# PengjieRen/CaSE_RG

Hardware: AMD Instinct MI355X
Metric: train tokens/sec (query+passage) CaSE model (higher is better)
Workload: dtype bf16; 1 GPU; CaSE train step fwd+bwd+allreduce+clip+Adam+EMA, d_model=512, 6 encoder layers, 10 passages x 384 tok, query 64, answer 40, vocab 30522, per-GPU batch 32, dropout on; global_batch=32, parallelism=dp1

## Files before the change

### case_rg_amd/CaSE/Model.py

```python
import torch
import torch.nn as nn

from .. import config, ops
from ..common.Constants import BOS_WORD, EOS_WORD, UNK_WORD
from ..common.Interaction import Interaction
from ..common.TransformerSeqEncoderDecoder import PointerDecoderCore, TransformerSeqEncoder, no_repeat_ngram_param, sampling_params
from ..common.Utils import to_sentence
from ..common.heads import block_stack, generation_nll, passage_bce, run_block_pair, run_blocks
from ..evaluation.rouge_ids import consensus_answers


class CaSETransformerSeqDecoder(PointerDecoderCore):

    def __init__(self, num_memories, num_layers, nhead, tgt_vocab_size, hidden_size, emb_matrix=None):
        super().__init__()
        H = hidden_size
        self._build(num_memories, num_layers, nhead, tgt_vocab_size, H, 2 * H, emb_matrix=emb_matrix)
        self.norm1 = nn.LayerNorm(H)
        self.norm2 = nn.LayerNorm(H)
        self.gen = nn.Sequential(nn.Linear(3 * H, H), nn.Dropout(0.1), nn.Linear(H, tgt_vocab_size, bias=False), nn.Softmax(dim=-1))
        self.mix = nn.Linear(3 * H, num_memories + 1)

    def extend(self, dec_outputs, gen_outputs, memory_weights, source_map):
        H = self.hidden_size
        d1, d2 = self._mix(dec_outputs[..., :H], [dec_outputs[..., H:2 * H], dec_outputs[..., 2 * H:]], gen_outputs,
                           memory_weights, source_map)
        return (d1, d2) if self.training else d1 + d2

    def _feature(self, answer_rep, T):
        feat = ops.layer_norm(answer_rep, self.norm2.weight, self.norm2.bias, self.norm2.eps)
        return ops.dropout(feat.unsqueeze(1).expand(-1, T, -1).contiguous(), 0.1, self.training)

    def _head_parts(self, dec_in, x, feat):
        dec_out = ops.layer_norm(x, self.norm1.weight, self.norm1.bias, self.norm1.eps)
        return dec_out, torch.cat([dec_in, dec_out, feat], dim=-1)

    train_returns_pair = True

    @property
    def gen_dropout(self):
        return self.gen[1].p

    def forward(self, encode_memories, BOS, UNK, source_map, groundtruth_index=None, additional_decoder_feature=None,
                encode_weights=None, encode_masks=None, init_decoder_state=None, max_target_length=None, beam_width=None, sampling=None,
                score_index=None, no_repeat_ngram=0):
        return self._run(encode_memories, encode_masks, encode_weights, source_map, BOS, groundtruth_index, max_target_length, beam_width, sampling,
                         score_index, feature_of=lambda T: self._feature(additional_decoder_feature, T), no_repeat_ngram=no_repeat_ngram)


class RelevantPassageSelection(nn.Module):

    def __init__(self, hidden_size, num_heads, query_encoder, passage_encoder):
        super().__init__()
        self.hidden_size = hidden_size
        self.query_encoder = query_encoder
        self.passage_encoder = passage_encoder
        self.num_heads = num_heads
        self.interaction = Interaction(hidden_size)
        self.query_blocks = block_stack(num_heads, hidden_size, 2)
        self.passage_blocks = block_stack(num_heads, hidden_size, 4)
        self.scorer = nn.Linear(hidden_size, 1)

    def action(self, query, passage, encode_query, encode_passage):
        eq, ep = encode_query[0][:, :, -1], encode_passage[0][:, :, -1]
        passage_mask, query_mask = passage.ne(0), query.ne(0)
        g_pq, g_qp = self.interaction(eq, ep, query_mask, passage_mask)
        query_reps, passage_reps = run_block_pair(self.query_blocks, g_pq, query_mask, self.passage_blocks, g_qp, passage_mask)
        cls = passage_reps[:, :, 0].contiguous()
        score = ops.linear(cls, self.scorer.weight, self.scorer.bias, out_dtype=torch.float32).squeeze(-1)
        return score, (query_reps, query_reps[:, :, 0]), (passage_reps, passage_reps[:, :, 0])


class SupportingTokenIdentification(nn.Module):

    def __init__(self, max_span_size, hidden_size, num_heads, query_encoder, passage_encoder, passage_selection):
        super().__init__()
        self.hidden_size = hidden_size
        self.num_heads = num_heads
        self.query_encoder = query_encoder
        self.passage_encoder = passage_encoder
        self.max_span_size = max_span_size
        self.passage_selection = passage_selection
        self.interaction = Interaction(hidden_size)
        self.query_blocks = block_stack(num_heads, hidden_size, 1)
        self.passage_blocks = block_stack(num_heads, hidden_size, 2)
        self.norm1 = nn.LayerNorm(hidden_size)
        self.norm2 = nn.LayerNorm(hidden_size)
        self.scorer = nn.Linear(hidden_size, 1)

    def action(self, query, passage, encode_query, encode_passage, passage_selection_result):
        passage_mask, query_mask = passage.ne(0), query.ne(0)
        _, query_rep, passage_rep = passage_selection_result
        g_pq, g_qp = self.interaction(query_rep[0], passage_rep[0], query_mask, passage_mask)
        query_reps, passage_reps = run_block_pair(self.query_blocks, g_pq, query_mask, self.passage_blocks, g_qp, passage_mask)
        token_score = ops.linear(passage_reps, self.scorer.weight, self.scorer.bias, out_dtype=torch.float32).squeeze(-1)
        token_score = token_score.masked_fill(~passage_mask, -1e6).clamp(min=-1e6, max=1e6)
        query_reps = ops.layer_norm(query_rep[0], self.norm1.weight, self.norm1.bias, self.norm1.eps, add=query_reps)
        passage_reps = ops.layer_norm(passage_rep[0], self.norm2.weight, self.norm2.bias, self.norm2.eps, add=passage_reps)
        return token_score, (query_reps, query_reps[:, :, 0]), (passage_reps, passage_reps[:, :, 0])


class ResponseGeneration(nn.Module):

    def __init__(self, BOS, UNK, vocab_size, hidden_size, num_heads, query_encoder, passage_encoder, passage_selection,
                 span_extraction, decoder):
        super().__init__()
        self.hidden_size = hidden_size
        self.vocab_size = vocab_size
        self.num_heads = num_heads
        self.query_encoder = query_encoder
        self.passage_encoder = passage_encoder
        self.passage_selection = passage_selection
        self.span_extraction = span_extraction
        self.BOS = BOS
        self.UNK = UNK
        self.decoder = decoder

    def action(self, query, passage, source_map, encode_query, encode_passage, passage_selection_result,
               span_extraction_result, output=None, max_target_length=None, beam_width=None, sampling=None, score_index=None, no_repeat_ngram=0):
        B = query.size(0)
        passage_score = passage_selection_result[0]
        token_score, query_rep, passage_rep = span_extraction_result
        H = passage_rep[0].size(-1)
        prior = (torch.sigmoid(passage_score).unsqueeze(-1) * torch.sigmoid(token_score)).reshape(B, -1)
        prior = prior / (1e-8 + prior.sum(dim=-1, keepdim=True))
        mem = passage_rep[0].reshape(B, -1, H)
        answer_rep = ops.bmm(ops.cast_to(prior.unsqueeze(1), mem.dtype), mem, b_is_kn=True).squeeze(1)
        prior_p = prior.reshape_as(token_score)
        prior_q = torch.ones(B, 1, query_rep[0].size(2), device=prior.device)
        return self.decoder([query_rep[0], passage_rep[0]], self.BOS, self.UNK, source_map,
                            additional_decoder_feature=answer_rep, groundtruth_index=output,
                            max_target_length=max_target_length, encode_masks=[query.ne(0), passage.ne(0)],
                            encode_weights=[prior_q, prior_p], beam_width=beam_width, sampling=sampling, score_index=score_index,
                            no_repeat_ngram=no_repeat_ngram)


class CaSE(nn.Module):
    def __init__(self, max_span_size, max_target_length, id2vocab, vocab2id, hidden_size, enc_layers=3, dec_layers=4, heads=8, early_stop=False):
        super().__init__()
        V = len(vocab2id)
        self.UNK = vocab2id[UNK_WORD]
        self.max_target_length = max_target_length
        self.query_encoder = TransformerSeqEncoder(enc_layers, heads, V, hidden_size)
        self.passage_encoder = self.query_encoder
        self.passage_selection = RelevantPassageSelection(hidden_size, heads, self.query_encoder, self.passage_encoder)
        self.span_extraction = SupportingTokenIdentification(max_span_size, hidden_size, heads, self.query_encoder,
                                                             self.passage_encoder, self.passage_selection)
        self.response_generation = ResponseGeneration(vocab2id[BOS_WORD], vocab2id[UNK_WORD], V, hidden_size, heads,
                                                      self.query_encoder, self.passage_encoder, self.passage_selection,
                                                      self.span_extraction,
                                                      CaSETransformerSeqDecoder(2, dec_layers, heads, V, hidden_size))
        self.id2vocab = id2vocab
        self.vocab_size = len(id2vocab)
        self.vocab2id = vocab2id
        self.beam_width = 4
        self.sampling = dict(num_samples=1, temperature=1.0, top_k=0, top_p=1.0, seed=None)
        self.consensus_samples = 8
        self.no_repeat_ngram = 0
        self.response_generation.decoder.beam_eos_id = vocab2id[EOS_WORD]
        if early_stop:
            self.response_generation.decoder.eos_id = vocab2id[EOS_WORD]

    def to_sentence(self, data, batch_indices):
        return to_sentence(batch_indices, self.id2vocab)

    def _encode_select_extract(self, data):
        if self.query_encoder is self.passage_encoder:
            eq, ep = self.query_encoder.forward_many([data['query'], data['passage']])
        else:
            eq, ep = self.query_encoder(data['query']), self.passage_encoder(data['passage'])
        ps = self.passage_selection.action(data['query'], data['passage'], encode_query=eq, encode_passage=ep)
        se = self.span_extraction.action(data['query'], data['passage'], encode_query=eq, encode_passage=ep,
                                         passage_selection_result=ps)
        return eq, ep, ps, se

    def do_train(self, data):
        eq, ep, ps, se = self._encode_select_extract(data)
        loss_ps = passage_bce(ps[0], data['passage_label'])
        valid = data['passage'].ne(0).float()
        bce = torch.nn.functional.binary_cross_entropy_with_logits(se[0], data['token_label'].detach(), reduction='none')
        loss_se = (valid * bce * data['token_weight'].detach()).sum() / valid.sum()
        rg = self.response_generation.action(data['query'], data['passage'], data['source_map'], encode_query=eq,
                                             encode_passage=ep, passage_selection_result=ps, span_extraction_result=se,
                                             output=data['response'])
        dist1, dist2 = rg[2]
        return [loss_ps, loss_se, generation_nll(ops.add(dist1, dist2), data['response'])]

    def _respond(self, data, **mode):
        eq, ep, ps, se = self._encode_select_extract(data)
        rg = self.response_generation.action(data['query'], data['passage'], data['source_map'], encode_query=eq,
                                             encode_passage=ep, passage_selection_result=ps, span_extraction_result=se,
                                             output=None, **mode)
        return rg, ps[0]

    def _ngram(self, no_repeat_ngram):
        return no_repeat_ngram_param(self.no_repeat_ngram if no_repeat_ngram is None else no_repeat_ngram, self.max_target_length)

    def do_test(self, data, no_repeat_ngram=None):
        rg, rank = self._respond(data, max_target_length=self.max_target_length, no_repeat_ngram=self._ngram(no_repeat_ngram))
        return {'answer': rg[3], 'rank': rank}

    do_infer = do_test

    def do_beam(self, data, width=None, no_repeat_ngram=None):
        rg, rank = self._respond(data, max_target_length=self.max_target_length, beam_width=self.beam_width if width is None else width,
                                 no_repeat_ngram=self._ngram(no_repeat_ngram))
        return {'answer': rg[3], 'rank': rank, 'beam_score': rg[5][:, 0], 'beam_answers': rg[4], 'beam_scores': rg[5]}

    def do_sample(self, data, num_samples=1, temperature=1.0, top_k=0, top_p=1.0, seed=None, uniforms=None, no_repeat_ngram=None):
        sampling = sampling_params(self.vocab2id, num_samples, temperature, top_k, top_p, seed, uniforms)
        rg, rank = self._respond(data, max_target_length=self.max_target_length, sampling=sampling, no_repeat_ngram=self._ngram(no_repeat_ngram))
        return {'answer': rg[3], 'rank': rank, 'samples': rg[4], 'sample_probs': rg[5], 'sample_scores': rg[6]}

    def do_consensus(self, data, pool="sample", candidates=None, valid=None, weights=None, no_repeat_ngram=None, **sampling):
        return consensus_answers(self, data, lambda d: self._encode_select_extract(d)[2][0], pool, candidates, valid, weights,
                                 no_repeat_ngram=no_repeat_ngram, **sampling)

    def do_score(self, data, answers=None):
        if self.training:
            raise ValueError("do_score runs in eval mode: call model.eval() first")
        out, rank = self._respond(data, score_index=data['response'] if answers is None else answers)
        out['rank'] = rank
        return out

    def forward(self, data, method='mle_train'):
        if method == 'train':
            return self.do_train(data)
        elif method == 'test':
            return self.do_test(data)
        elif method == 'beam':
            return self.do_beam(data)
        elif method == 'sample':
            return self.do_sample(data, **self.sampling)
        elif method == 'score':
            return self.do_score(data)
        elif method == 'consensus':
            return self.do_consensus(data)
```

### case_rg_amd/Masque/Model.py

```python
import torch
import torch.nn as nn

from .. import ops
from ..common.Constants import BOS_WORD, EOS_WORD, UNK_WORD
from ..common.Interaction import Interaction
from ..common.TransformerSeqEncoderDecoder import PointerDecoderCore, TransformerSeqEncoder, no_repeat_ngram_param, sampling_params
from ..common.Utils import to_sentence
from ..common.heads import block_stack, generation_nll, passage_bce, run_block_pair
from ..evaluation.rouge_ids import consensus_answers


class MasqueTransformerSeqDecoder(PointerDecoderCore):

    def __init__(self, num_memories, num_layers, nhead, tgt_vocab_size, hidden_size, emb_matrix=None):
        super().__init__()
        H = hidden_size
        self._build(num_memories, num_layers, nhead, tgt_vocab_size, H, H, emb_matrix=emb_matrix)
        self.norm = nn.LayerNorm(H)
        self.gen = nn.Sequential(nn.Linear(2 * H, H), nn.Linear(H, tgt_vocab_size, bias=False), nn.Softmax(dim=-1))
        self.mix = nn.Linear(3 * H, num_memories + 1)

    def extend(self, dec_outputs, gen_outputs, memory_weights, source_map):
        H = self.hidden_size
        d1, d2 = self._mix(dec_outputs[..., :H], [dec_outputs[..., H:2 * H], dec_outputs[..., 2 * H:]], gen_outputs,
                           memory_weights, source_map)
        return d1 + d2

    def _head_parts(self, dec_in, x, feat):
        dec_out = ops.layer_norm(x, self.norm.weight, self.norm.bias, self.norm.eps)
        return dec_out, torch.cat([dec_in, dec_out], dim=-1)

    def forward(self, encode_memories, BOS, UNK, source_map, encode_masks=None, encode_weights=None,
                groundtruth_index=None, init_decoder_state=None, max_target_length=None, beam_width=None, sampling=None, score_index=None,
                no_repeat_ngram=0):
        return self._run(encode_memories, encode_masks, encode_weights, source_map, BOS, groundtruth_index, max_target_length, beam_width, sampling,
                         score_index, no_repeat_ngram=no_repeat_ngram)


class PassageSelection(nn.Module):

    def __init__(self, hidden_size, num_heads, query_encoder, passage_encoder):
        super().__init__()
        self.hidden_size = hidden_size
        self.query_encoder = query_encoder
        self.passage_encoder = passage_encoder
        self.num_heads = num_heads
        self.interaction = Interaction(hidden_size)
        self.query_blocks = block_stack(num_heads, hidden_size, 2)
        self.passage_blocks = block_stack(num_heads, hidden_size, 4)
        self.scorer = nn.Linear(hidden_size, 1)

    def action(self, query, passage, encode_query=None, encode_passage=None):
        if encode_query is None:
            encode_query = self.query_encoder(query)[0][:, :, -1]
        if encode_passage is None:
            encode_passage = self.passage_encoder(passage)[0][:, :, -1]
        passage_mask, query_mask = passage.ne(0), query.ne(0)
        g_pq, g_qp = self.interaction(encode_query, encode_passage, query_mask, passage_mask)
        query_reps, passage_reps = run_block_pair(self.query_blocks, g_pq, query_mask, self.passage_blocks, g_qp, passage_mask)
        cls = passage_reps[:, :, 0].contiguous()
        score = ops.linear(cls, self.scorer.weight, self.scorer.bias, out_dtype=torch.float32).squeeze(-1)
        return score, query_reps, passage_reps


class ResponseGeneration(nn.Module):

    def __init__(self, BOS, UNK, vocab_size, hidden_size, num_heads, query_encoder, passage_encoder, passage_selection, decoder):
        super().__init__()
        self.hidden_size = hidden_size
        self.vocab_size = vocab_size
        self.num_heads = num_heads
        self.query_encoder = query_encoder
        self.passage_encoder = passage_encoder
        self.passage_selection = passage_selection
        self.BOS = BOS
        self.UNK = UNK
        self.decoder = decoder

    def action(self, query, passage, source_map, encode_query=None, encode_passage=None, passage_selection_result=None,
               output=None, max_target_length=None, beam_width=None, sampling=None, score_index=None, no_repeat_ngram=0):
        if encode_query is None:
            encode_query = self.query_encoder(query)[0][:, :, -1]
        if encode_passage is None:
            encode_passage = self.passage_encoder(passage)[0][:, :, -1]
        if passage_selection_result is None:
            passage_selection_result = self.passage_selection.action(query, passage, encode_query=encode_query,
                                                                     encode_passage=encode_passage)
        passage_score, query_rep, passage_rep = passage_selection_result
        B = query.size(0)
        prior_q = torch.ones(B, 1, query_rep.size(2), device=passage_score.device)
        prior_p = torch.sigmoid(passage_score).unsqueeze(-1).expand(-1, -1, passage_rep.size(2))
        return self.decoder([query_rep, passage_rep], self.BOS, self.UNK, source_map, groundtruth_index=output,
                            max_target_length=max_target_length, encode_masks=[query.ne(0), passage.ne(0)],
                            encode_weights=[prior_q, prior_p], beam_width=beam_width, sampling=sampling, score_index=score_index,
                            no_repeat_ngram=no_repeat_ngram)


class Masque(nn.Module):
    def __init__(self, max_target_length, id2vocab, vocab2id, hidden_size, enc_layers=3, dec_layers=4, heads=8, early_stop=False):
        super().__init__()
        V = len(vocab2id)
        self.UNK = vocab2id[UNK_WORD]
        self.max_target_length = max_target_length
        self.query_encoder = TransformerSeqEncoder(enc_layers, heads, V, hidden_size)
        self.passage_encoder = self.query_encoder
        self.passage_selection = PassageSelection(hidden_size, heads, self.query_encoder, self.passage_encoder)
        self.response_generation = ResponseGeneration(vocab2id[BOS_WORD], vocab2id[UNK_WORD], V, hidden_size, heads,
                                                      self.query_encoder, self.passage_encoder, self.passage_selection,
                                                      MasqueTransformerSeqDecoder(2, dec_layers, heads, V, hidden_size))
        self.id2vocab = id2vocab
        self.vocab_size = len(id2vocab)
        self.vocab2id = vocab2id
        self.beam_width = 4
        self.sampling = dict(num_samples=1, temperature=1.0, top_k=0, top_p=1.0, seed=None)
        self.consensus_samples = 8
        self.no_repeat_ngram = 0
        self.response_generation.decoder.beam_eos_id = vocab2id[EOS_WORD]
        if early_stop:
            self.response_generation.decoder.eos_id = vocab2id[EOS_WORD]

    def to_sentence(self, data, batch_indices):
        return to_sentence(batch_indices, self.id2vocab)

    def _encode_select(self, data):
        if self.query_encoder is self.passage_encoder:
            oq, op = self.query_encoder.forward_many([data['query'], data['passage']])
            eq, ep = oq[0][:, :, -1], op[0][:, :, -1]
        else:
            eq = self.query_encoder(data['query'])[0][:, :, -1]
            ep = self.passage_encoder(data['passage'])[0][:, :, -1]
        return eq, ep, self.passage_selection.action(data['query'], data['passage'], encode_query=eq, encode_passage=ep)

    def do_train(self, data):
        eq, ep, ps = self._encode_select(data)
        rg = self.response_generation.action(data['query'], data['passage'], data['source_map'], encode_query=eq,
                                             encode_passage=ep, passage_selection_result=ps, output=data['response'])
        return [0.25 * passage_bce(ps[0], data['passage_label']), generation_nll(rg[2], data['response'])]

    def do_ps_train(self, data):
        _, _, ps = self._encode_select(data)
        return [passage_bce(ps[0], data['passage_label'])]

    def _respond(self, data, **mode):
        eq, ep, ps = self._encode_select(data)
        rg = self.response_generation.action(data['query'], data['passage'], data['source_map'], encode_query=eq,
                                             encode_passage=ep, passage_selection_result=ps, output=None, **mode)
        return rg, ps[0]

    def _ngram(self, no_repeat_ngram):
        return no_repeat_ngram_param(self.no_repeat_ngram if no_repeat_ngram is None else no_repeat_ngram, self.max_target_length)

    def do_test(self, data, no_repeat_ngram=None):
        rg, rank = self._respond(data, max_target_length=self.max_target_length, no_repeat_ngram=self._ngram(no_repeat_ngram))
        return {'answer': rg[3], 'rank': rank}

    do_infer = do_test

    def do_beam(self, data, width=None, no_repeat_ngram=None):
        rg, rank = self._respond(data, max_target_length=self.max_target_length, beam_width=self.beam_width if width is None else width,
                                 no_repeat_ngram=self._ngram(no_repeat_ngram))
        return {'answer': rg[3], 'rank': rank, 'beam_score': rg[5][:, 0], 'beam_answers': rg[4], 'beam_scores': rg[5]}

    def do_sample(self, data, num_samples=1, temperature=1.0, top_k=0, top_p=1.0, seed=None, uniforms=None, no_repeat_ngram=None):
        sampling = sampling_params(self.vocab2id, num_samples, temperature, top_k, top_p, seed, uniforms)
        rg, rank = self._respond(data, max_target_length=self.max_target_length, sampling=sampling, no_repeat_ngram=self._ngram(no_repeat_ngram))
        return {'answer': rg[3], 'rank': rank, 'samples': rg[4], 'sample_probs': rg[5], 'sample_scores': rg[6]}

    def do_consensus(self, data, pool="sample", candidates=None, valid=None, weights=None, no_repeat_ngram=None, **sampling):
        return consensus_answers(self, data, lambda d: self._encode_select(d)[2][0], pool, candidates, valid, weights,
                                 no_repeat_ngram=no_repeat_ngram, **sampling)

    def do_score(self, data, answers=None):
        if self.training:
            raise ValueError("do_score runs in eval mode: call model.eval() first")
        out, rank = self._respond(data, score_index=data['response'] if answers is None else answers)
        out['rank'] = rank
        return out

    def forward(self, data, method='mle_train'):
        if method == 'train':
            return self.do_train(data)
        elif method == 'ps_train':
            return self.do_ps_train(data)
        elif method == 'test':
            return self.do_test(data)
        elif method == 'beam':
            return self.do_beam(data)
        elif method == 'sample':
            return self.do_sample(data, **self.sampling)
        elif method == 'score':
            return self.do_score(data)
        elif method == 'consensus':
            return self.do_consensus(data)
```

### case_rg_amd/_abi.py

```python
import ctypes as C
import os

import torch

_HERE = os.path.dirname(os.path.abspath(__file__))
LIB_PATH = os.environ.get("CASE_HIP_LIB") or os.path.join(_HERE, "csrc", "libcase_hip.so")

ABI_VERSION = 600
F32, BF16 = 0, 1
WS_ATTENTION_SPLITKV, WS_ATTENTION_BWD, WS_OPTIM_SUMSQ, WS_ENCODER_CHAIN_PACK, WS_GEMM_DW_SLABS = 1, 2, 3, 4, 5
(FEAT_GEMM_256, FEAT_GEMM_SMALL, FEAT_ENCODER_CHAIN, FEAT_ATTN_SCORES, FEAT_ATTN_DECODE, FEAT_OPTIM, FEAT_ATTN_RESIDENT, FEAT_RESERVED_CUS,
 FEAT_GEMM_DW_SLABS, FEAT_DECODER_CHAIN, FEAT_ATTN_DECODE_MQA, FEAT_POINTER_DECODE, FEAT_POINTER_HEAD, FEAT_GEMM_LN, FEAT_STEP_STATE,
 FEAT_INTERACTION, FEAT_ATTN_DECODE_APPEND, FEAT_LINEAR_SKINNY, FEAT_BEAM_DECODE, FEAT_SAMPLE_DECODE, FEAT_POINTER_SCORE, FEAT_CONSENSUS, FEAT_NGRAM_BAN) = (1 << i for i in range(23))
EPI_BIAS_COL, EPI_BIAS_ROW, EPI_GELU, EPI_RELU = 1, 2, 4, 8
EPI_RESIDUAL, EPI_MUL_DGELU, EPI_MUL_DRELU, EPI_ATOMIC, EPI_DROPOUT = 16, 32, 64, 128, 256

i32, i64, u64, f32, f64, ptr = C.c_int32, C.c_int64, C.c_uint64, C.c_float, C.c_double, C.c_void_p


class GemmDesc(C.Structure):
    _fields_ = [(n, i64) for n in ("M", "N", "K", "lda", "ldb", "ldc", "ld_aux", "batch1", "batch2",
                                   "sa1", "sa2", "sb1", "sb2", "sc1", "sc2", "saux1", "saux2")] + \
               [(n, i32) for n in ("a_kmajor", "b_kmajor", "in_dtype", "out_dtype", "epilogue", "split_k", "tile")] + \
               [("alpha", f32), ("drop_p", f32), ("seed", u64), ("offset", u64), ("state", ptr)]


class StepState(C.Structure):
    _fields_ = [("rng_base", u64), ("step_size", f32), ("bc2_sqrt", f32), ("lr", f32), ("step", i32), ("reserved", u64 * 5)]


class EncoderChainDesc(C.Structure):
    _fields_ = [("rows", i64), ("width", i32), ("variant", i32), ("eps_ln2", f32), ("eps_ln1_next", f32)]


class SoftmaxDesc(C.Structure):
    _fields_ = [("outer", i64), ("inner", i64), ("R", i64), ("C", i64), ("causal", i32), ("in_dtype", i32),
                ("out_dtype", i32), ("drop_p", f32), ("seed", u64), ("offset", u64), ("state", ptr)]


class AttnDesc(C.Structure):
    _fields_ = [(n, i64) for n in ("N", "heads", "Lq", "Lk", "head_dim", "ldq", "ldk", "ldv", "sq", "sk", "sv", "ldo", "so")] + \
               [("causal", i32), ("scale", f32), ("drop_p", f32), ("seed", u64), ("offset", u64), ("state", ptr)]


class InteractionDesc(C.Structure):
    _fields_ = [(n, i64) for n in ("n", "Lp", "Lq", "H", "eq_div")] + [("dtype", i32)]


class AttnProductDesc(C.Structure):
    _fields_ = [(n, i64) for n in ("N", "heads", "M", "Kc", "head_dim", "lda", "sa_seq", "sa_head", "ldb", "sb_seq", "sb_head",
                                   "ldc", "sc_seq", "sc_head")] + [("a_transposed", i32), ("alpha", f32)]


SIGNATURES = {
    "case_gemm": [C.POINTER(GemmDesc), ptr, ptr, ptr, ptr, ptr, ptr, ptr, ptr],
    "case_gemm_dw_bias": [C.POINTER(GemmDesc), ptr, ptr, ptr, ptr, ptr],
    "case_gemm_dw_slabs": [C.POINTER(GemmDesc), ptr, ptr, ptr, ptr, ptr, i64, ptr],
    "case_embed_pos_fwd": [ptr, ptr, ptr, ptr, i64, i64, i64, i64, f32, f32, u64, u64, ptr, i32, ptr],
    "case_embed_pos_bwd": [ptr, ptr, ptr, i64, i64, i64, f32, f32, u64, u64, ptr, i32, ptr],
    "case_scale_add_rows": [ptr, ptr, ptr, i64, i64, i64, f32, i32, ptr],
    "case_layernorm_fwd": [ptr, ptr, ptr, ptr, ptr, ptr, ptr, i64, i64, f32, i32, ptr],
    "case_layernorm_bwd": [ptr, ptr, ptr, ptr, ptr, ptr, ptr, ptr, ptr, ptr, i64, i64, i32, ptr],
    "case_layernorm_bwd_dropout": [ptr, ptr, ptr, ptr, ptr, ptr, ptr, ptr, ptr, i64, i64, f32, u64, u64, ptr, i32, ptr],
    "case_layernorm_bwd_concat5": [ptr] * 15 + [i64, i64, i32, ptr],
    "case_softmax_fwd": [C.POINTER(SoftmaxDesc), ptr, ptr, ptr, ptr, ptr, ptr],
    "case_softmax_bwd": [C.POINTER(SoftmaxDesc), ptr, ptr, ptr, ptr],
    "case_attention_supported": [i64],
    "case_attention_fwd": [C.POINTER(AttnDesc), ptr, ptr, ptr, ptr, ptr, ptr, ptr],
    "case_attention_splitkv_workspace": [C.POINTER(AttnDesc), i32, C.POINTER(i64)],
    "case_attention_fwd_splitkv": [C.POINTER(AttnDesc), ptr, ptr, ptr, ptr, ptr, ptr, ptr, i64, i32, ptr],
    "case_attention_bwd_supported": [i64],
    "case_attention_decode_supported": [i64],
    "case_attention_decode": [C.POINTER(AttnDesc), ptr, ptr, ptr, ptr, ptr, ptr],
    "case_attention_decode_append": [C.POINTER(AttnDesc), ptr, ptr, ptr, ptr, ptr, i64, i64, ptr, ptr, ptr],
    "case_attention_bwd": [C.POINTER(AttnDesc), ptr, ptr, ptr, ptr, ptr, ptr, ptr, ptr, ptr, ptr, ptr, ptr],
    "case_attention_scores_supported": [C.POINTER(AttnDesc)],
    "case_attention_scores_fwd": [C.POINTER(AttnDesc), ptr, ptr, ptr, ptr, ptr, ptr],
    "case_attention_scores_bwd": [C.POINTER(AttnDesc), ptr, ptr, ptr, ptr, ptr],
    "case_attention_product_supported": [C.POINTER(AttnProductDesc)],
    "case_attention_product": [C.POINTER(AttnProductDesc), ptr, ptr, ptr, ptr],
    "case_add": [ptr, ptr, ptr, i64, i32, ptr],
    "case_add_n": [C.POINTER(ptr), i32, ptr, i64, i32, ptr],
    "case_dropout": [ptr, ptr, i64, f32, u64, u64, ptr, i32, ptr],
    "case_mask_rows": [ptr, ptr, ptr, i64, i64, i32, ptr],
    "case_colsum": [ptr, ptr, i64, i64, i32, ptr],
    "case_cast": [ptr, ptr, i64, i32, i32, ptr],
    "case_scale_cols": [ptr, ptr, ptr, i64, i64, i32, ptr],
    "case_scale_cols_bwd": [ptr, ptr, ptr, ptr, ptr, i64, i64, i32, ptr],
    "case_rowdot_fwd": [ptr, ptr, ptr, ptr, i64, i64, i32, ptr],
    "case_linear_skinny": [ptr, ptr, i32, ptr, ptr, ptr, i64, i32, i32, ptr],
    "case_rowdot_bwd": [ptr, ptr, ptr, ptr, ptr, ptr, i64, i64, i32, ptr],
    "case_masked_mean_fwd": [ptr, ptr, ptr, i64, i64, i64, i32, ptr],
    "case_masked_mean_bwd": [ptr, ptr, ptr, i64, i64, i64, i32, ptr],
    "case_highway_gate_fwd": [ptr, ptr, i64, i64, i32, ptr],
    "case_highway_gate_bwd": [ptr, ptr, ptr, i64, i64, i32, ptr],
    "case_concat5_fwd": [ptr, ptr, ptr, ptr, ptr, i64, i64, i32, ptr],
    "case_concat5_bwd": [ptr, ptr, ptr, ptr, ptr, ptr, ptr, ptr, i64, i64, i32, ptr],
    "case_max_over_p_fwd": [ptr, ptr, ptr, i64, i64, i64, i32, ptr],
    "case_max_over_p_bwd": [ptr, ptr, ptr, i64, i64, i64, i32, ptr],
    "case_additive_scores_fwd": [ptr, ptr, ptr, ptr, i64, i64, i64, i64, i32, ptr],
    "case_additive_scores_bwd": [ptr, ptr, ptr, ptr, ptr, ptr, ptr, i64, i64, i64, i64, i32, ptr],
    "case_copy_scatter_fwd": [ptr, ptr, ptr, i64, i64, i64, i64, ptr],
    "case_copy_scatter_bwd": [ptr, ptr, ptr, i64, i64, i64, i64, ptr],
    "case_source_sort": [ptr, ptr, i64, i64, i64, ptr],
    "case_copy_scatter_sorted_fwd": [ptr, ptr, ptr, i64, i64, i64, i64, ptr],
    "case_nll_gather_fwd": [ptr, ptr, ptr, i64, i64, ptr],
    "case_nll_gather_bwd": [ptr, ptr, ptr, ptr, i64, i64, ptr],
    "case_row_argmax": [ptr, ptr, ptr, i64, i64, i64, ptr],
    "case_sentence_compact": [ptr, ptr, ptr, i64, i64, i64, i64, i64, ptr],
    "case_encoder_chain_pack": [ptr, ptr, ptr, ptr, ptr, ptr],
    "case_encoder_chain": [C.POINTER(EncoderChainDesc)] + [ptr] * 14,
    "case_set_reserved_cus": [i32],
    "case_attention_decode_mqa": [ptr, ptr, ptr, ptr, i64, i64, i64, i32, ptr, i64, ptr],
    "case_additive_key_exp": [ptr, ptr, i64, ptr],
    "case_pointer_attend_decode": [ptr] * 11 + [i64, i64, i64, ptr],
    "case_pointer_head_decode": [ptr] * 5 + [i32] + [ptr] * 4 + [i64, i64, i64, ptr],
    "case_pointer_head_beam": [ptr] * 5 + [i32] + [ptr] * 4 + [i64, i64, i64, i32, ptr],
    "case_pointer_head_sample": [ptr] * 5 + [i32] + [ptr] * 7 + [i64, i64, i64, f32, i32, f32, u64, u64, ptr, i64, i64, i64, i32, i32, ptr],
    "case_pointer_head_score": [ptr] * 3 + [i64, ptr, ptr, i32, ptr, i64, ptr, ptr, i64, i64, i64, ptr],
    "case_beam_advance": [ptr] * 12 + [i64, i64, i64, i32, i64, ptr],
    "case_pointer_head_decode_ban": [ptr] * 5 + [i32] + [ptr] * 4 + [i64, i64, i64, ptr, i64, i64, i32, i64, ptr],
    "case_pointer_head_beam_ban": [ptr] * 5 + [i32] + [ptr] * 4 + [i64, i64, i64, i32, ptr, i64, i64, i32, i64, ptr],
    "case_pointer_head_sample_ban": [ptr] * 5 + [i32] + [ptr] * 7 + [i64, i64, i64, f32, i32, f32, u64, u64, ptr, i64, i64, i64, i32, i32,
                                     ptr, i64, i64, i32, ptr],
    "case_beam_advance_ban": [ptr] * 12 + [i64, i64, i64, i32, i64, ptr, ptr, i64, ptr],
    "case_ngram_ban": [ptr, ptr, ptr, i64, i64, i64, i64, i32, i64, ptr],
    "case_remove_duplicate_ids": [ptr, ptr, i64, i64, i32, i64, ptr],
    "case_beam_gather": [ptr, ptr, i32, ptr, ptr, ptr, i64, i32, i64, i64, i64, ptr],
    "case_beam_backtrack": [ptr] * 8 + [i64, i32, i64, ptr],
    "case_lcs_pairs": [ptr] * 6 + [i64, i64, i64, i64, i64, ptr],
    "case_consensus_pick": [ptr] * 7 + [i64, i64, i64, ptr],
    "case_gemm_ln": [C.POINTER(GemmDesc), ptr, ptr, ptr, f32, ptr, ptr, ptr, ptr, ptr, ptr],
    "case_optim_sumsq": [ptr, ptr, i64, ptr, ptr, ptr],
    "case_optim_adam_ema": [ptr, ptr, i64, ptr, f32, f64, f64, f64, f64, ptr, ptr],
    "case_step_advance": [ptr, u64, f64, f64, ptr],
    "case_interaction_supported": [C.POINTER(InteractionDesc)],
    "case_interaction_fwd": [C.POINTER(InteractionDesc), ptr, ptr, ptr, ptr, ptr, ptr, ptr, ptr, ptr, ptr],
}


def _load():
    if not os.path.exists(LIB_PATH):
        raise ImportError(
            "case_rg_amd: %s is missing. Build it with `python -c 'import __graft_entry__ as g; g.build()'` "
            "(or `make -C case_rg_amd/csrc`). There is no CPU or eager fallback." % LIB_PATH)
    lib = C.CDLL(LIB_PATH)
    lib.case_version.restype = C.c_int
    if lib.case_version() != ABI_VERSION:
        raise ImportError("case_rg_amd: %s is ABI generation %d, this package binds %d -- rebuild it (make -C case_rg_amd/csrc)"
                          % (LIB_PATH, lib.case_version(), ABI_VERSION))
    for name, args in SIGNATURES.items():
        fn = getattr(lib, name)
        fn.argtypes = args
        fn.restype = C.c_int
    lib.case_optim_chunk_elems.restype = C.c_int
    lib.case_optim_chunk_elems.argtypes = []
    lib.case_encoder_chain_packed_bytes.restype = C.c_int64
    lib.case_encoder_chain_packed_bytes.argtypes = []
    lib.case_attention_bwd_scratch_floats.restype = C.c_int64
    lib.case_attention_bwd_scratch_floats.argtypes = [C.POINTER(AttnDesc)]
    lib.case_attention_decode_mqa_workspace.restype = C.c_int64
    lib.case_attention_decode_mqa_workspace.argtypes = [i64, i64, i32]
    lib.case_attention_decode_mqa_splits.restype = C.c_int32
    lib.case_attention_decode_mqa_splits.argtypes = [i64, i64]
    lib.case_abi_features.restype = C.c_uint32
    lib.case_abi_features.argtypes = []
    lib.case_get_reserved_cus.restype = C.c_int
    lib.case_get_reserved_cus.argtypes = []
    lib.case_sizeof_opt_tensor.restype = C.c_int
    lib.case_sizeof_opt_tensor.argtypes = []
    lib.case_sizeof_step_state.restype = C.c_int
    lib.case_sizeof_step_state.argtypes = []
    if lib.case_sizeof_step_state() != C.sizeof(StepState):
        raise ImportError("case_rg_amd: CaseStepState is %d bytes in %s, %d in this binding" % (lib.case_sizeof_step_state(), LIB_PATH, C.sizeof(StepState)))
    lib.case_gemm_dw_slab_bytes.restype = C.c_int64
    lib.case_gemm_dw_slab_bytes.argtypes = [C.POINTER(GemmDesc)]
    lib.case_workspace_bytes.restype = C.c_int64
    lib.case_workspace_bytes.argtypes = [i32, ptr, i64]
    lib.case_gemm_tile_for.restype = C.c_int
    lib.case_gemm_tile_for.argtypes = [C.POINTER(GemmDesc), ptr, ptr, ptr, ptr, ptr, ptr]
    lib.case_last_error.restype = C.c_char_p
    return lib


lib = _load()


def check(code, what):
    if code != 0:
        raise RuntimeError("%s failed (%d): %s" % (what, code, lib.case_last_error().decode()))


def call(name, *args):
    check(getattr(lib, name)(*args), name)
```

### case_rg_amd/common/TransformerSeqEncoderDecoder.py

```python
import operator
import os

import torch
import torch.nn as nn

from .. import config, ops
from .BilinearAttention import BilinearAttention
from .PositionalEmbedding import PositionalEmbedding
from .TransformerDecoder import TransformerDecoder, TransformerDecoderLayer
from .TransformerEncoder import TransformerEncoder, TransformerEncoderLayer
from .Utils import generate_square_subsequent_mask

MERGED_ENCODE = os.environ.get("CASE_MERGED_ENCODE", "1") != "0"
QUERY_SPLIT = os.environ.get("CASE_QUERY_SPLIT", "1") != "0"


def _embedding(vocab, width, max_len=1000, emb_matrix=None):
    if emb_matrix is not None:
        vocab, width = emb_matrix.shape
    table = nn.Embedding(vocab, width, padding_idx=0)
    if emb_matrix is not None:
        table.load_state_dict({"weight": emb_matrix})
        table.weight.requires_grad = False
    return nn.Sequential(table, PositionalEmbedding(width, dropout=0.1, max_len=max_len))
# ... 248 lines not shown
                            eu=self.attns[i].project_keys_exp(m) if fused else None))
        return out

    def _run_prefix(self, dec_ids, mems, valid, weights, feature):
        dec_in = _embed(self.embedding, dec_ids, self.training)
        tgt_valid = dec_ids.ne(0)
        x = dec_in
        ctxs, copies = [], []
        for i, mem in enumerate(mems):
            x = self.decs[i].forward_batch_first(x, mem, tgt_valid, valid[i], causal=True)
            q = x if feature is None else torch.cat([x, feature], dim=-1)
            ctx, p = self.attns[i].attend(q, mem, mem, row_valid=tgt_valid, col_valid=valid[i])
            ctxs.append(ctx)
            if weights is not None:
                p = weights[i].unsqueeze(1) * p
                p = p / (1e-8 + p.sum(dim=-1, keepdim=True))
            copies.append(p)
        return dec_in, x, ctxs, copies

    def _check_length(self, T):
        if T > self.embedding[1].pe.size(0):
            raise RuntimeError("max_target_length %d exceeds max_len %d" % (T, self.embedding[1].pe.size(0)))

    def _cache_setup(self, mems, max_target_length, feat):
        B, dev = mems[0].shape[0], mems[0].device
        inference = not self.training and not torch.is_grad_enabled()
        cache = self._memory_cache(mems, absorb=inference)
        self_kvs = [dec.new_self_cache(B, max_target_length, mems[0]) for dec in self.decs]
        hist_valid = torch.zeros(B, max_target_length, dtype=torch.bool, device=dev)
        self._check_length(max_target_length)
        splits = [self.attns[i].split_query(feat, self.hidden_size) if (QUERY_SPLIT and inference and feat is not None and cache[i]["eu"] is not None) else None
                  for i in range(len(mems))]
        return inference, cache, self_kvs, hist_valid, splits

    def _cached_layers(self, t, ids, mems, valid, weights, feat, cache, splits, self_kvs, hist_valid):
        table, pos = self.embedding[0].weight, self.embedding[1]
        tok_valid = ids.ne(0)
        hist_valid[:, t] = tok_valid[:, 0]
        dec_in = ops.embed_pos(ids, table, pos.pe[t:t + 1])
        x = dec_in
        ctxs, copies = [], []
        for i, mem in enumerate(mems):
            x = self.decs[i].step(x, t, self_kvs[i], hist_valid, cache[i]["kvs"], valid[i])
            q = x if (feat is None or splits[i] is not None) else torch.cat([x, feat], dim=-1)
            if cache[i]["eu"] is not None:
                ctx, p = self.attns[i].attend_decode(q, mem, tok_valid, valid[i], cache[i]["eu"], None if weights is None else weights[i],
                                                     split=splits[i])
            else:
                ctx, p = self.attns[i].attend(q, mem, mem, row_valid=tok_valid, col_valid=valid[i], uh=cache[i]["uh"])
                if weights is not None:
                    p = weights[i].unsqueeze(1) * p
                    p = p / (1e-8 + p.sum(dim=-1, keepdim=True))
            ctxs.append(ctx)
            copies.append(p)
        return dec_in, x, ctxs, copies

    @staticmethod
    def _per_item(n, mems, valid, weights, source_map, feat, keys=True, unit_too=False):
        if n == 1 and not unit_too:
            return mems, valid, weights, source_map, feat
        mems = [m.repeat_interleave(n, dim=0) for m in mems]
        valid = [v.repeat_interleave(n, dim=0) for v in valid]
        weights = None if weights is None else [w.repeat_interleave(n, dim=0) for w in weights]
        if keys:
            source_map = source_map.expand(n) if isinstance(source_map, ops.SortedSource) else source_map.repeat_interleave(n, dim=0)
        return mems, valid, weights, source_map, None if feat is None else feat.repeat_interleave(n, dim=0)

    def _decode(self, mode, mems, valid, weights, source_map, feat, BOS, max_target_length):
        R, dev, T = mems[0].shape[0], mems[0].device, max_target_length
        inference, cache, self_kvs, hist_valid, splits = self._cache_setup(mems, T, feat)
        ids = self._bos(R, BOS, dev)
        capturing = torch.cuda.is_current_stream_capturing()
        fused_head = inference and ops.pointer_head_supported(source_map, self.tgt_vocab_size, len(mems))
        mode.start(capturing, self_kvs, hist_valid)
        for t in range(T):
            dec_in, x, ctxs, copies = self._cached_layers(t, ids, mems, valid, weights, feat, cache, splits, self_kvs, hist_valid)
            if fused_head:
                dec_out, gen_in = self._head_parts(dec_in, x, feat)
                logits, mix_logits = self._head_logits(dec_out, gen_in, ctxs)
                ids = mode.fused_step(t, logits, mix_logits, source_map, [c.reshape(R, -1) for c in copies])
            else:
                dec_out, gen, dist = self._head(dec_in, x, ctxs, copies, feat, source_map)
                ids = mode.unfused_step(t, gen, dist)
            steps = t + 1
            if steps == T:
                break
            self_kvs, hist_valid = mode.after_step(t, self_kvs, hist_valid)
            if not capturing and steps % self.eos_check_every == 0 and mode.all_finished():
                break
        setattr(self, mode.counter, steps)
        return mode.result(dec_out)

    def _score(self, mems, valid, weights, source_map, BOS, answers, pad=0, feature_of=None):
        if self.training:
            raise ValueError("scoring runs in eval mode: call model.eval() first")
        if answers.dim() == 2:
            answers = answers.unsqueeze(1)
        if answers.dim() != 3 or answers.dtype != torch.int64 or answers.size(0) != mems[0].shape[0]:
            raise ValueError("scoring: answers must be int64 [B, T] or [B, N, T] with the batch's B")
        B, N, T = answers.shape
        dev, V, H = mems[0].device, self.tgt_vocab_size, self.hidden_size
        self._check_length(T)
        feat = None if feature_of is None else feature_of(T)
        mems, valid, weights, source_map, feat = self._per_item(N, mems, valid, weights, source_map, feat, keys=False)
        R = B * N
        tgt = answers.reshape(R, T).to(dev)
        dec_ids = torch.cat([self._bos(R, BOS, dev), tgt[:, :-1]], dim=-1)
        dec_in, x, ctxs, copies = self._run_prefix(dec_ids, mems, valid, weights, feat)
        rows, per = R * T, N * T
        dec_in, x = dec_in.reshape(rows, 1, H), x.reshape(rows, 1, H)
        feat = None if feat is None else feat.reshape(rows, 1, -1)
        ctxs = [c.reshape(rows, 1, -1) for c in ctxs]
        copies = [c.reshape(rows, -1) for c in copies]
        flat = tgt.reshape(rows)
        sorted_src = isinstance(source_map, ops.SortedSource)
        fused = sorted_src and ops.pointer_score_supported(source_map, len(mems))
        limit = max(1, int(self.score_chunk_rows))
        if per <= limit:
            step = limit // per * per
            chunks = [(r0, min(r0 + step, rows)) for r0 in range(0, rows, step)]
        else:
            chunks = [(b * per + o, min(b * per + o + limit, (b + 1) * per)) for b in range(B) for o in range(0, per, limit)]
        probs, ptrs = [], []
        for r0, r1 in chunks:
            n = r1 - r0
            dec_out, gen_in = self._head_parts(dec_in[r0:r1], x[r0:r1], None if feat is None else feat[r0:r1])
            cx, cp, y = [c[r0:r1] for c in ctxs], [c[r0:r1] for c in copies], flat[r0:r1]
            b0, b1 = r0 // per, (r1 + per - 1) // per
            if fused:
                logits, mix_logits = self._head_logits(dec_out, gen_in, cx)
                p, c = ops.pointer_head_score(logits, mix_logits, source_map.select(slice(b0, b1)), n // (b1 - b0), cp, y, pad)
            else:
                item = torch.arange(r0, r1, device=dev) // per
                src = source_map.select(item) if sorted_src else source_map.index_select(0, item)
                gen = self._generate(gen_in, 0.0)
                d1, d2 = self._mix(dec_out, cx, gen, [c.unsqueeze(1) for c in cp], src)
                inside = (y >= 0) & (y < V)
                at = y.clamp(0, V - 1).reshape(n, 1, 1)
                c = d2.gather(-1, at).reshape(n)
                p = d1.gather(-1, at).reshape(n) + c
                skip = y.eq(pad) if pad >= 0 else torch.zeros_like(inside)
                p = torch.where(skip, torch.ones_like(p), torch.where(inside, p, torch.zeros_like(p)))
                c = torch.where(skip | ~inside, torch.zeros_like(c), c)
            probs.append(p)
            ptrs.append(c)
        p, c = torch.cat(probs).view(B, N, T), torch.cat(ptrs).view(B, N, T)
        scored = (answers.to(dev).ne(pad) if pad >= 0 else torch.ones_like(answers, dtype=torch.bool, device=dev))
        count = scored.sum()
        scores = (-torch.log(p.clamp_min(1e-30)) * scored).sum(dim=-1) / scored.sum(dim=-1).clamp_min(1)
        loss = ((-torch.log(p + 1e-8) * scored).sum() / count.clamp_min(1)).reshape(1)
        return dict(token_probs=p, copy_probs=c, scores=scores, loss=loss, tokens=count)

    def _run(self, encode_memories, encode_masks, encode_weights, source_map, BOS, groundtruth_index, max_target_length, beam_width, sampling,
             score_index, feature_of=None, no_repeat_ngram=0):
        B, dev = source_map.size(0), encode_memories[0].device
        source_map = self._sorted(source_map)
        mems = [m.reshape(B, -1, self.hidden_size) for m in encode_memories]
        valid = [m.reshape(B, -1).contiguous() for m in encode_masks]
        weights = None if encode_weights is None else [w.reshape(B, -1) for w in encode_weights]
        if score_index is not None:
            return self._score(mems, valid, weights, source_map, BOS, score_index, feature_of=feature_of)
        T = groundtruth_index.size(1) if max_target_length is None else max_target_length
        if self.training and groundtruth_index is not None:
            dec_ids = torch.cat([self._bos(B, BOS, dev), groundtruth_index[:, :-1]], dim=-1)
            feat = None if feature_of is None else feature_of(dec_ids.size(1))
            dec_out, gen, dist = self._head(*self._run_prefix(dec_ids, mems, valid, weights, feat), feat, source_map)
            return dec_out, gen, dist, groundtruth_index
        if self.training:
            return None
        feat = None if feature_of is None else feature_of(1)
        ngram = no_repeat_ngram_param(no_repeat_ngram, T)
        if ngram and not ops.ngram_ban_supported():
            raise RuntimeError("no_repeat_ngram: this build of the library lacks the n-gram ban (CASE_FEAT_NGRAM_BAN)")
        if beam_width:
            W = int(beam_width)
            if not ops.beam_supported(W):
                raise RuntimeError("beam search: width %d is outside what the beam kernels are built for (1 .. 8)" % W)
            mode, n = _BeamMode(self, B, W, T, dev, ngram), W
        elif sampling:
            if not ops.sample_supported(self.tgt_vocab_size):
                raise RuntimeError("sampled decoding: the vocabulary (%d) is beyond what the sampling kernel holds in LDS (V <= 36000)"
                                   % self.tgt_vocab_size)
            mode, n = _SampleMode(B, T, dev, sampling, ngram), int(sampling["num_samples"])
        else:
            mode, n = _GreedyMode(self, B, T, dev, ngram), 1
        return self._decode(mode, *self._per_item(n, mems, valid, weights, source_map, feat, unit_too=bool(beam_width)), BOS, T)

    def _head_logits(self, dec_out, gen_in, ctxs):
        B, V = dec_out.shape[0], self.tgt_vocab_size
        h = ops.linear(gen_in, self.gen[0].weight, self.gen[0].bias)
        logits = ops.linear(h, self.gen[-2].weight, None, out_dtype=torch.float32)
        parts = [dec_out] + ctxs
        if ops.linear_skinny_supported(parts, self.mix.weight):
            mix_logits = ops.linear_skinny(parts, self.mix.weight, self.mix.bias)
        else:
            mix_logits = ops.linear(torch.cat(parts, dim=-1), self.mix.weight, self.mix.bias, out_dtype=torch.float32)
        return logits.reshape(B, V), mix_logits.reshape(B, -1)

    def _head(self, dec_in, x, ctxs, copies, feat, source_map):
        dec_out, gen_in = self._head_parts(dec_in, x, feat)
        gen = self._generate(gen_in, self.gen_dropout)
        d1, d2 = self._mix(dec_out, ctxs, gen, copies, source_map)
        return dec_out, gen, ((d1, d2) if self.training and self.train_returns_pair else ops.add(d1, d2))

    def _generate(self, gen_in, hidden_drop):
        h = ops.linear(gen_in, self.gen[0].weight, self.gen[0].bias, p_drop=config.drop_p(hidden_drop, self.training))
        logits = ops.linear(h, self.gen[-2].weight, None, out_dtype=torch.float32)
        return ops.masked_softmax(logits)

    def _mix(self, dec_out, ctxs, gen, copies, source_map):
        mix_in = torch.cat([dec_out] + ctxs, dim=-1)
        pm = ops.masked_softmax(ops.linear(mix_in, self.mix.weight, self.mix.bias, out_dtype=torch.float32))
        dist1 = pm[:, :, 0:1] * gen
        ptr = torch.cat([pm[:, :, k + 1:k + 2] * c for k, c in enumerate(copies)], dim=-1)
        return dist1, self._scatter(ptr, source_map, gen.shape[-1])

    @staticmethod
    def _scatter(ptr, source_map, V):
        if isinstance(source_map, ops.SortedSource) or (source_map.dtype == torch.int64 and source_map.dim() == 2):
            return ops.copy_scatter(source_map, ptr, V)
        return ops.copy_scatter(source_map.argmax(dim=-1), ptr * source_map.sum(dim=-1).unsqueeze(1), V)

    @staticmethod
    def _bos(batch_size, BOS, device):
        return torch.full((batch_size, 1), BOS, dtype=torch.long, device=device)


class TransformerSeqDecoder(PointerDecoderCore):

    def __init__(self, num_memories, num_layers, nhead, tgt_vocab_size, hidden_size, emb_matrix=None):
        super().__init__()
        H = hidden_size
        self._build(num_memories, num_layers, nhead, tgt_vocab_size, H, H, emb_matrix=emb_matrix, max_len=100 if emb_matrix is not None else 1000)
        self.norm = nn.LayerNorm(H)
        self.gen = nn.Sequential(nn.Linear(2 * H, H), nn.Linear(H, tgt_vocab_size, bias=False), nn.Softmax(dim=-1))
        self.mix = nn.Linear(H + num_memories * H, num_memories + 1)

    def _head_parts(self, dec_in, x, feat):
        dec_out = ops.layer_norm(x, self.norm.weight, self.norm.bias, self.norm.eps)
        return dec_out, torch.cat([dec_in, dec_out], dim=-1)

    def forward(self, encode_memories, BOS, UNK, source_maps, encode_masks=None, encode_weights=None,
                groundtruth_index=None, init_decoder_state=None, max_target_length=None, beam_width=None, sampling=None, score_index=None,
                no_repeat_ngram=0):
        if isinstance(source_maps, (list, tuple)):
            source_maps = torch.cat(source_maps, dim=-2 if source_maps[0].dim() == 3 else -1)
        return self._run(encode_memories, encode_masks, encode_weights, source_maps, BOS, groundtruth_index, max_target_length, beam_width, sampling,
                         score_index, no_repeat_ngram=no_repeat_ngram)
```

### case_rg_amd/common/heads.py

```python
import os

import torch
import torch.distributed as dist
import torch.nn as nn
import torch.nn.functional as F

from .. import ops
from .TransformerBlock import TransformerBlock


def block_stack(num_heads, hidden_size, extra):
    return nn.ModuleList([TransformerBlock(num_heads, 5 * hidden_size, hidden_size)] +
                         [TransformerBlock(num_heads, hidden_size, hidden_size) for _ in range(extra)])


def run_blocks(blocks, reps, mask):
    for block in blocks:
        reps = block(reps, mask)
    return reps


SIDE_STREAM = os.environ.get("CASE_SIDE_STREAM", "1") != "0"
SIDE_STREAM_INFERENCE = os.environ.get("CASE_SIDE_STREAM_INFERENCE", "0") == "1"
SIDE_STREAM_NOT_UNDER_DP = os.environ.get("CASE_SIDE_STREAM_UNDER_DP", "0") != "1"
SIDE_STREAM_MIN_ELEMS = 100_000_000
_side = {}


def run_block_pair(query_blocks, g_pq, query_mask, passage_blocks, g_qp, passage_mask):
    if not (SIDE_STREAM and g_pq.is_cuda and g_qp.numel() >= SIDE_STREAM_MIN_ELEMS and (torch.is_grad_enabled() or SIDE_STREAM_INFERENCE)
            and not torch.cuda.is_current_stream_capturing() and not (SIDE_STREAM_NOT_UNDER_DP and dist.is_available() and dist.is_initialized())):
        return run_blocks(query_blocks, g_pq, query_mask), run_blocks(passage_blocks, g_qp, passage_mask)
    cur = torch.cuda.current_stream()
    side = _side.get(g_pq.device)
    if side is None:
        side = _side[g_pq.device] = torch.cuda.Stream(device=g_pq.device)
    ops.AUX_STREAMS[side.cuda_stream] = side
    ops.AUX_STREAMS[cur.cuda_stream] = cur
    side.wait_stream(cur)
    with torch.cuda.stream(side):
        g_pq.record_stream(side)
        if torch.is_tensor(query_mask):
            query_mask.record_stream(side)
        query_reps = run_blocks(query_blocks, g_pq, query_mask)
    passage_reps = run_blocks(passage_blocks, g_qp, passage_mask)
    cur.wait_stream(side)
    query_reps.record_stream(cur)
    return query_reps, passage_reps


def passage_bce(passage_score, passage_label):
    target = torch.zeros_like(passage_score).scatter_(1, passage_label.unsqueeze(-1), 1.0)
    return F.binary_cross_entropy_with_logits(passage_score.float(), target.float()).unsqueeze(0)


def generation_nll(dist, response):
    V = dist.size(-1)
    rows = ops.nll_rows(dist.reshape(-1, V), response.reshape(-1))
    count = response.ne(0).sum().clamp(min=1)
    return (rows.sum() / count).unsqueeze(0)
```

### case_rg_amd/csrc/api.hip

```cpp
#include <stdarg.h>
#include <stdio.h>
#include <stdlib.h>

#include "common.h"

static thread_local char g_err[512] = "";

int case_set_error(int code, const char* fmt, ...) {
  va_list ap;
  va_start(ap, fmt);
  vsnprintf(g_err, sizeof(g_err), fmt, ap);
  va_end(ap);
  return code;
}

int case_check_launch(const char* what) {
  const hipError_t e = hipGetLastError();
  if (e == hipSuccess) return CASE_OK;
  return case_set_error(CASE_E_LAUNCH, "%s: %s", what, hipGetErrorString(e));
}

extern "C" int case_version(void) { return CASE_ABI_VERSION; }
extern "C" uint32_t case_abi_features(void) {
  return CASE_FEAT_GEMM_256 | CASE_FEAT_GEMM_SMALL | CASE_FEAT_ENCODER_CHAIN | CASE_FEAT_ATTN_SCORES | CASE_FEAT_ATTN_DECODE | CASE_FEAT_OPTIM |
         CASE_FEAT_ATTN_RESIDENT | CASE_FEAT_RESERVED_CUS | CASE_FEAT_GEMM_DW_SLABS | CASE_FEAT_ATTN_DECODE_MQA | CASE_FEAT_POINTER_DECODE | CASE_FEAT_POINTER_HEAD | CASE_FEAT_GEMM_LN | CASE_FEAT_STEP_STATE | CASE_FEAT_INTERACTION | CASE_FEAT_ATTN_DECODE_APPEND | CASE_FEAT_LINEAR_SKINNY |
         CASE_FEAT_BEAM_DECODE | CASE_FEAT_SAMPLE_DECODE | CASE_FEAT_POINTER_SCORE | CASE_FEAT_CONSENSUS | CASE_FEAT_NGRAM_BAN;
}
extern "C" const char* case_last_error(void) { return g_err; }

static int g_reserved_cus = [] {
  const char* e = getenv("CASE_RESERVE_CUS");
  return e ? atoi(e) : 0;
}();
extern "C" int case_set_reserved_cus(int n) {
  if (n < 0 || n > 128) return case_set_error(CASE_E_ARG, "case_set_reserved_cus: %d out of range (0 .. 128)", n);
  g_reserved_cus = n;
  return CASE_OK;
}
extern "C" int case_get_reserved_cus(void) { return g_reserved_cus; }
int case_device_cus() {
  static int cus = 0;
  if (!cus) {
    int dev = 0, n = 0;
    (void)hipGetDevice(&dev);
    (void)hipDeviceGetAttribute(&n, hipDeviceAttributeMultiprocessorCount, dev);
    cus = n > 0 ? n : 256;
  }
  return cus;
}
int case_persistent_cus() {
  int c = case_device_cus() - g_reserved_cus;
  c = c / 8 * 8;
  return c > 8 ? c : 8;
}
extern "C" int case_sizeof_opt_tensor(void) { return (int)sizeof(CaseOptTensor); }
```

### case_rg_amd/csrc/attn_pointer.hip

```cpp
#include "common.h"

namespace {

template <bool FAST>
__device__ __forceinline__ float tanh_t(float x) {
  if constexpr (FAST) {
    const float e = __expf(2.f * x);
    return 1.f - __fdividef(2.f, e + 1.f);
  } else {
    return tanhf(x);
  }
}

constexpr float TANH_PRESCALE = 2.8853900817779268f;
constexpr float EXP2_CLAMP = 62.f;
__device__ __forceinline__ float exp2_factor(float xs) { return __builtin_amdgcn_exp2f(fminf(fmaxf(xs, -EXP2_CLAMP), EXP2_CLAMP)); }
__device__ __forceinline__ float half_sigmoid_prod(float ew, float eu) { return __builtin_amdgcn_rcpf(fmaf(ew, eu, 1.f)); }

constexpr int AJ = 64;
constexpr int AH = 64;
constexpr int ATW = 8;

template <typename T, bool FAST>
__global__ __launch_bounds__(256) void additive_fwd_kernel(const float* __restrict__ wq, const T* __restrict__ uh,
// ... 800 lines not shown
  return x;
}

template <bool BAN>
__global__ __launch_bounds__(PH_THREADS) void pointer_head_sample_kernel(const HeadArgs a, const SampleArgs s, const BanArgs nb) {
  extern __shared__ __attribute__((aligned(16))) float ph_smem[];
  float* row = ph_smem;
  uint32_t* tk = reinterpret_cast<uint32_t*>(ph_smem + ((a.V + 3) & ~(int64_t)3));
  float* tv = reinterpret_cast<float*>(tk + PH_THREADS + 4);
  float* red = tv + PH_THREADS;
  unsigned long long* hist = reinterpret_cast<unsigned long long*>(tk);
  __shared__ unsigned long long sel[3];
  __shared__ uint32_t wcnt[SM_WAVES];
  __shared__ float wsum[SM_WAVES];
  __shared__ int wmin[SM_WAVES], wmax[SM_WAVES];
  __shared__ int tie_id;
  const int64_t b = blockIdx.x;
  const int V = (int)a.V, tid = threadIdx.x, lane = tid & 63, wave = tid >> 6;
  if (a.logits) {
    pointer_head_build_row(a, row, tk, tv, red, b);
  } else {
    for (int i = tid; i < V; i += PH_THREADS) row[i] = s.dist_in[b * a.V + i];
    __syncthreads();
  }
  if constexpr (BAN) {
    if (!s.ended[b]) ngram_ban_row(row, a.V, nb.hist + b * nb.Tmax, nb.t, nb.n, s.eos, reinterpret_cast<int*>(tv));
  }
  float pmax = 0.f;
  for (int i = tid; i < V; i += PH_THREADS) {
    const float x = row[i];
    if (a.dist) a.dist[b * a.V + i] = x;
    pmax = fmaxf(pmax, x);
  }
  pmax = block_max(pmax, red);

  SampleView v;
  v.row = row;
  const int chunk = (((V + SM_WAVES - 1) / SM_WAVES) + 255) & ~255;
  v.w0 = min(V, wave * chunk);
  v.w1 = min(V, v.w0 + chunk);
  v.lane = lane;
  v.unit = s.temperature == 1.f;
  v.inv_tau = 1.f / s.temperature;
  v.l2max = v.unit ? 0.f : __builtin_amdgcn_logf(pmax);
  {
    int e = 0;
    frexpf(v.unit ? pmax : 1.f, &e);
    v.scale = ldexpf(1.f, min(40 - e, 120));
  }
  v.cbits = 0;
  v.cid = V - 1;

  if (s.top_k > 0 && s.top_k < V) {
    const uint32_t bits = sample_radix<false>(v, hist, sel, (unsigned long long)s.top_k, 0.0);
    const unsigned long long r = sel[1] - sel[0];
    const int id = sample_nth_tie(v, bits, r, wcnt, &tie_id, V);
    v.cbits = bits;
    v.cid = id;
  }
  if (s.top_p < 1.f) {
    const uint32_t bits = sample_radix<true>(v, hist, sel, 0ull, (double)s.top_p);
    const unsigned long long m = (unsigned long long)(__uint_as_float(bits) * v.scale), lack = sel[1] - sel[0];
    const unsigned long long r = m > 0 ? (lack + m - 1) / m : 1ull;
    const int id = sample_nth_tie(v, bits, r < 1 ? 1ull : r, wcnt, &tie_id, V);
    v.cbits = bits;
    v.cid = id;
  }

  float carry = 0.f;
  for (int base = v.w0; base < v.w1; base += 256) {
    float x[4];
    v.quad(base, x);
    const float mine = ((x[0] + x[1]) + x[2]) + x[3];
    const float inc = sample_scan64(mine, lane);
    float before = __shfl_up(inc, 1, 64);
    if (lane == 0) before = 0.f;
    carry += __shfl(before + mine, 63, 64);
  }
  if (lane == 0) wsum[wave] = carry;
  __syncthreads();
  float off = 0.f, Z = 0.f;
  for (int w = 0; w < SM_WAVES; ++w) {
    if (w == wave) off = Z;
    Z += wsum[w];
  }
  const float u = s.uniforms ? s.uniforms[b] : rng_uniform24(s.seed, rng_base_of(s.state) + s.offset + (uint64_t)b);
  const float thr = u * Z;
  int mn = 0x7fffffff, mx = -1;
  carry = 0.f;
  for (int base = v.w0; base < v.w1; base += 256) {
    float x[4];
    v.quad(base, x);
    const float mine = ((x[0] + x[1]) + x[2]) + x[3];
    const float inc = sample_scan64(mine, lane);
    float before = __shfl_up(inc, 1, 64);
    if (lane == 0) before = 0.f;
    float run = 0.f;
#pragma unroll
    for (int e = 0; e < 4; ++e) {
      run = e == 0 ? x[0] : run + x[e];
      const int i = base + 4 * lane + e;
      if (x[e] > 0.f) {
        mx = i;
        if (off + (carry + (before + run)) > thr && i < mn) mn = i;
      }
    }
    carry += __shfl(before + mine, 63, 64);
  }
#pragma unroll
  for (int o = 32; o > 0; o >>= 1) {
    mn = min(mn, __shfl_xor(mn, o, 64));
    mx = max(mx, __shfl_xor(mx, o, 64));
  }
  if (lane == 0) {
    wmin[wave] = mn;
    wmax[wave] = mx;
  }
  __syncthreads();
  if (tid == 0) {
    for (int w = 0; w < SM_WAVES; ++w) {
      mn = min(mn, wmin[w]);
      mx = max(mx, wmax[w]);
    }
    const int x = mn < V ? mn : (mx >= 0 ? mx : 0);
    const bool e = s.ended[b] != 0, this_end = (int64_t)x == s.eos;
    int64_t emit;
    if (s.first) emit = this_end ? s.unk : (int64_t)x;
    else if (s.last) emit = e ? s.pad : s.eos;
    else emit = e ? s.pad : (int64_t)x;
    s.ids[b] = emit;
    if constexpr (BAN) nb.hist[b * nb.Tmax + nb.t] = (int32_t)emit;
    s.prob[b] = e ? 1.f : row[x];
    s.ended[b] = (uint8_t)(e || this_end);
  }
}

__global__ __launch_bounds__(64) void ngram_ban_kernel(float* __restrict__ dist, const uint8_t* __restrict__ ended, const int64_t V, const BanArgs nb) {
  __shared__ int stage[NB_MAX_T];
  const int64_t b = blockIdx.x;
  if (ended && ended[b]) return;
  ngram_ban_row(dist + b * V, V, nb.hist + b * nb.Tmax, nb.t, nb.n, nb.eos, stage);
}

constexpr int PS_THREADS = 256;
struct ScoreArgs {
  const float* logits;
  const float* mix_logits;
  const uint32_t* keys;
  const float* copy[PH_MAX_MEM];
  int64_t len[PH_MAX_MEM];
  const int64_t* targets;
  float* prob;
  float* ptr;
  int64_t V, S, rows_per_source, pad;
  int nmem;
};

typedef float ps_f32x4 __attribute__((ext_vector_type(4)));
#ifndef CASE_STREAM_DEFAULT_POLICY
#define PS_LOAD1(P) __builtin_nontemporal_load(P)
#define PS_LOAD4(P) __builtin_nontemporal_load(reinterpret_cast<const ps_f32x4*>(P))
#else
#define PS_LOAD1(P) (*(P))
#define PS_LOAD4(P) (*reinterpret_cast<const ps_f32x4*>(P))
#endif

__device__ __forceinline__ void ps_merge(float& m, float& s, const float om, const float os) {
  const float M = fmaxf(m, om);
  const float ref = M == -INFINITY ? 0.f : M;
  s = s * __expf(m - ref) + os * __expf(om - ref);
  m = M;
}

__global__ __launch_bounds__(PS_THREADS) void pointer_head_score_kernel(const ScoreArgs a) {
  __shared__ float red_m[PS_THREADS / 64], red_s[PS_THREADS / 64];
  const int64_t r = blockIdx.x, V = a.V;
  const int tid = threadIdx.x, lane = tid & 63;
  const int64_t y = a.targets[r];
  const bool is_pad = a.pad >= 0 && y == a.pad;
  if (is_pad || y < 0 || y >= V) {
    if (tid == 0) {
      a.prob[r] = is_pad ? 1.f : 0.f;
      if (a.ptr) a.ptr[r] = 0.f;
    }
    return;
  }
  const float* lg = a.logits + r * V;
  int64_t head = (int64_t)(((16u - (uint32_t)(reinterpret_cast<uintptr_t>(lg) & 15u)) & 15u) >> 2);
  if (head > V) head = V;
  const int64_t n4 = (V - head) >> 2, tail = head + 4 * n4;
  float m = -INFINITY, s = 0.f;
  if (tid < head) ps_merge(m, s, PS_LOAD1(lg + tid), 1.f);
  const float* body = lg + head;
#pragma unroll 2
  for (int64_t i = tid; i < n4; i += PS_THREADS) {
    const ps_f32x4 x = PS_LOAD4(body + 4 * i);
    const float m4 = fmaxf(fmaxf(x[0], x[1]), fmaxf(x[2], x[3]));
    if (m4 > m) {
      s *= __expf(m - m4);
      m = m4;
    }
    s += (__expf(x[0] - m) + __expf(x[1] - m)) + (__expf(x[2] - m) + __expf(x[3] - m));
  }
  if (tail + tid < V) ps_merge(m, s, PS_LOAD1(lg + tail + tid), 1.f);
#pragma unroll
  for (int o = 32; o > 0; o >>= 1) {
    const float om = __shfl_xor(m, o, 64), os = __shfl_xor(s, o, 64);
    ps_merge(m, s, om, os);
  }
  if (lane == 0) {
    red_m[tid >> 6] = m;
    red_s[tid >> 6] = s;
  }
  __syncthreads();
  if (tid >= 64) return;
  m = red_m[0];
  s = red_s[0];
#pragma unroll
  for (int w = 1; w < PS_THREADS / 64; ++w) ps_merge(m, s, red_m[w], red_s[w]);
  const float gen_y = __expf(lg[y] - m) / s;
  float pm[1 + PH_MAX_MEM];
  {
    float mm = -INFINITY, ss = 0.f;
#pragma unroll
    for (int k = 0; k <= PH_MAX_MEM; ++k) pm[k] = k <= a.nmem ? a.mix_logits[r * (a.nmem + 1) + k] : -INFINITY;
#pragma unroll
    for (int k = 0; k <= PH_MAX_MEM; ++k) mm = fmaxf(mm, pm[k]);
#pragma unroll
    for (int k = 0; k <= PH_MAX_MEM; ++k) {
      pm[k] = __expf(pm[k] - mm);
      ss += pm[k];
    }
#pragma unroll
    for (int k = 0; k <= PH_MAX_MEM; ++k) pm[k] /= ss;
  }
  const uint32_t* keys = a.keys + (r / a.rows_per_source) * a.S;
  const uint32_t want = (uint32_t)y << 15;
  int64_t lo = 0, hi = a.S;
  while (lo < hi) {
    const int64_t mid = (lo + hi) >> 1;
    if (keys[mid] < want) lo = mid + 1;
    else hi = mid;
  }
  float acc = 0.f;
  for (int64_t i = lo + lane; i < a.S; i += 64) {
    const uint32_t key = keys[i];
    if (key == 0xFFFFFFFFu || (key >> 15) != (uint32_t)y) break;
    int64_t pos = key & 0x7FFFu;
    bool done = false;
#pragma unroll
    for (int k = 0; k < PH_MAX_MEM; ++k) {
      if (k < a.nmem && !done) {
        if (pos < a.len[k]) {
          acc += pm[k + 1] * a.copy[k][r * a.len[k] + pos];
          done = true;
        }
        pos -= a.len[k];
      }
    }
  }
  acc = wave_sum(acc);
  if (lane == 0) {
    a.prob[r] = pm[0] * gen_y + acc;
    if (a.ptr) a.ptr[r] = acc;
  }
}

__global__ void copy_scatter_fwd_kernel(const int64_t* __restrict__ src, const float* __restrict__ w,
                                        float* __restrict__ dist, int64_t B, int64_t Tn, int64_t S, int64_t V) {
  const int64_t n = B * Tn * S;
  for (int64_t i = (int64_t)blockIdx.x * blockDim.x + threadIdx.x; i < n; i += (int64_t)gridDim.x * blockDim.x) {
    const int64_t sidx = i % S, bt = i / S, b = bt / Tn;
    const int64_t tok = src[b * S + sidx];
    const float val = w[i];
    if (tok >= 0 && tok < V && val != 0.f) atomicAdd(dist + bt * V + tok, val);
  }
}

__global__ void copy_scatter_bwd_kernel(const int64_t* __restrict__ src, const float* __restrict__ d_dist,
                                        float* __restrict__ d_w, int64_t B, int64_t Tn, int64_t S, int64_t V) {
  const int64_t n = B * Tn * S;
  for (int64_t i = (int64_t)blockIdx.x * blockDim.x + threadIdx.x; i < n; i += (int64_t)gridDim.x * blockDim.x) {
    const int64_t sidx = i % S, bt = i / S, b = bt / Tn;
    const int64_t tok = src[b * S + sidx];
    d_w[i] = (tok >= 0 && tok < V) ? d_dist[bt * V + tok] : 0.f;
  }
}

__global__ __launch_bounds__(1024) void source_sort_kernel(const int64_t* __restrict__ src, uint32_t* __restrict__ keys, int64_t S,
                                                            int64_t V, int n) {
  extern __shared__ uint32_t sk[];
  const int64_t b = blockIdx.x;
  for (int i = threadIdx.x; i < n; i += 1024) {
    uint32_t k = 0xFFFFFFFFu;
    if (i < S) {
      const int64_t tok = src[b * S + i];
      if (tok >= 0 && tok < V) k = ((uint32_t)tok << 15) | (uint32_t)i;
    }
    sk[i] = k;
  }
  __syncthreads();
  for (int k = 2; k <= n; k <<= 1) {
    for (int j = k >> 1; j > 0; j >>= 1) {
      for (int i = threadIdx.x; i < n; i += 1024) {
        const int p = i ^ j;
        if (p > i) {
          const uint32_t x = sk[i], y = sk[p];
          if ((x > y) == ((i & k) == 0)) {
            sk[i] = y;
            sk[p] = x;
          }
        }
      }
      __syncthreads();
    }
  }
  for (int i = threadIdx.x; i < S; i += 1024) keys[b * S + i] = sk[i];
}

__global__ __launch_bounds__(256) void copy_scatter_sorted_kernel(const uint32_t* __restrict__ keys, const float* __restrict__ w,
                                                                  float* __restrict__ dist, int64_t Tn, int64_t S, int64_t V) {
  __shared__ uint32_t tk[257];
  __shared__ float tv[256];
  const int64_t bt = blockIdx.x, b = bt / Tn;
  const uint32_t* k = keys + b * S;
  const float* wr = w + bt * S;
  float* d = dist + bt * V;
  for (int64_t base = 0; base < S; base += 256) {
    const int64_t i = base + threadIdx.x;
    const uint32_t key = i < S ? k[i] : 0xFFFFFFFFu;
    const bool valid = key != 0xFFFFFFFFu;
    tk[threadIdx.x] = valid ? (key >> 15) : 0xFFFFFFFFu;
    tv[threadIdx.x] = valid ? wr[key & 0x7FFFu] : 0.f;
    if (threadIdx.x == 0) tk[256] = 0xFFFFFFFEu;
    __syncthreads();
    const uint32_t tok = tk[threadIdx.x];
    if (valid && tok != tk[threadIdx.x + 1]) {
      int j = threadIdx.x;
      while (j > 0 && tk[j - 1] == tok) --j;
      float sum = 0.f;
      for (; j <= (int)threadIdx.x; ++j) sum += tv[j];
      if (sum != 0.f) d[tok] += sum;
    }
    __threadfence_block();
    __syncthreads();
  }
}

__global__ void nll_fwd_kernel(const float* __restrict__ dist, const int64_t* __restrict__ target,
                               float* __restrict__ per_row, int64_t rows, int64_t V) {
  for (int64_t r = (int64_t)blockIdx.x * blockDim.x + threadIdx.x; r < rows; r += (int64_t)gridDim.x * blockDim.x) {
    const int64_t y = target[r];
    per_row[r] = (y > 0 && y < V) ? -logf(dist[r * V + y] + 1e-8f) : 0.f;
  }
}

__global__ void nll_bwd_kernel(const float* __restrict__ dist, const int64_t* __restrict__ target,
                               const float* __restrict__ g_row, float* __restrict__ d_dist, int64_t rows, int64_t V) {
  for (int64_t r = (int64_t)blockIdx.x * blockDim.x + threadIdx.x; r < rows; r += (int64_t)gridDim.x * blockDim.x) {
    const int64_t y = target[r];
    if (y > 0 && y < V) d_dist[r * V + y] = -g_row[r] / (dist[r * V + y] + 1e-8f);
  }
}

__global__ __launch_bounds__(256) void row_argmax_kernel(const float* __restrict__ x, int64_t* __restrict__ idx,
                                                         float* __restrict__ val, int64_t rows, int64_t cols, int64_t ld) {
  __shared__ float sv[4];
  __shared__ int64_t si[4];
  for (int64_t r = blockIdx.x; r < rows; r += gridDim.x) {
    float best = -INFINITY;
    int64_t bi = cols;
    for (int64_t c = threadIdx.x; c < cols; c += 256) {
      const float vv = x[r * ld + c];
      if (vv > best || (vv == best && c < bi)) {
        best = vv;
        bi = c;
      }
    }
#pragma unroll
    for (int o = 32; o > 0; o >>= 1) {
      const float ob = __shfl_xor(best, o, 64);
      const int64_t oi = __shfl_xor(bi, o, 64);
      if (ob > best || (ob == best && oi < bi)) {
        best = ob;
        bi = oi;
      }
    }
    __syncthreads();
    if ((threadIdx.x & 63) == 0) {
      sv[threadIdx.x >> 6] = best;
      si[threadIdx.x >> 6] = bi;
    }
    __syncthreads();
    if (threadIdx.x == 0) {
      for (int w = 1; w < 4; ++w)
        if (sv[w] > best || (sv[w] == best && si[w] < bi)) {
          best = sv[w];
          bi = si[w];
        }
      idx[r] = bi < cols ? bi : 0;
      if (val) val[r] = best;
    }
  }
}

}

extern "C" int case_additive_scores_fwd(const float* wq, const void* uh, const float* v, float* s, int64_t B, int64_t T,
                                        int64_t S, int64_t H, int32_t dtype, case_stream_t stream) {
  CASE_REQUIRE(wq && uh && v && s && B > 0 && T > 0 && S > 0 && H > 0 && B < 65536, "case_additive_scores_fwd: bad argument");
  hipStream_t st = (hipStream_t)stream;
  const int ev = dtype == CASE_F32 ? 4 : 8;
  if (T <= 2 && H % ev == 0 && H <= 2 * 64 * ev && (uintptr_t)uh % 16 == 0) {
    const dim3 g((unsigned)((S + 15) / 16 < 64 ? (S + 15) / 16 : 64), (unsigned)B);
    const bool one = H <= 64 * ev;
#define ROWWISE(TY, FAST, TT, NCH) hipLaunchKernelGGL((additive_fwd_rowwise_kernel<TY, FAST, TT, NCH>), g, dim3(256), 0, st, wq, (const TY*)uh, v, s, T, S, H)
    if (dtype == CASE_F32) {
// ... 140 lines not shown
  a.ids = ids;
  a.top = top;
  static bool attr = false;
  rc = pointer_head_reserve(reinterpret_cast<const void*>(&pointer_head_decode_kernel<BAN>), attr, who);
  if (rc != CASE_OK) return rc;
  hipLaunchKernelGGL(pointer_head_decode_kernel<BAN>, dim3((unsigned)B), dim3(PH_THREADS), pointer_head_lds(V), (hipStream_t)stream, a, nb);
  return case_check_launch(who);
}

extern "C" int case_pointer_head_decode(const float* logits, const float* mix_logits, const uint32_t* keys, const float* const* copies,
                                        const int64_t* lens, int32_t nmem, float* gen, float* dist, int64_t* ids, float* top, int64_t B, int64_t V,
                                        int64_t S, case_stream_t stream) {
  return pointer_head_decode_launch<false>("case_pointer_head_decode", logits, mix_logits, keys, copies, lens, nmem, gen, dist, ids, top, B, V, S,
                                           BanArgs(), stream);
}

extern "C" int case_pointer_head_decode_ban(const float* logits, const float* mix_logits, const uint32_t* keys, const float* const* copies,
                                            const int64_t* lens, int32_t nmem, float* gen, float* dist, int64_t* ids, float* top, int64_t B,
                                            int64_t V, int64_t S, int32_t* hist, int64_t Tmax, int64_t t, int32_t n, int64_t eos,
                                            case_stream_t stream) {
  BanArgs nb;
  const int rc = pointer_head_ban(nb, "case_pointer_head_decode_ban", hist, Tmax, t, n, eos);
  if (rc != CASE_OK) return rc;
  return pointer_head_decode_launch<true>("case_pointer_head_decode_ban", logits, mix_logits, keys, copies, lens, nmem, gen, dist, ids, top, B, V, S,
                                          nb, stream);
}

template <bool BAN>
static int pointer_head_beam_launch(const char* who, const float* logits, const float* mix_logits, const uint32_t* keys, const float* const* copies,
                                    const int64_t* lens, int32_t nmem, float* gen, float* dist, float* cand_p, int64_t* cand_id, int64_t R, int64_t V,
                                    int64_t S, int32_t W, const BanArgs& nb, case_stream_t stream) {
  CASE_REQUIRE(cand_p && cand_id, "%s: bad argument", who);
  if (W < 1 || W > PH_MAX_W || W > V) return case_set_error(CASE_E_UNSUPPORTED, "%s: width %d outside 1 .. min(%d, V)", who, W, PH_MAX_W);
  HeadArgs a;
  int rc = pointer_head_args(a, who, logits, mix_logits, keys, copies, lens, nmem, gen, dist, R, V, S);
  if (rc != CASE_OK) return rc;
  static bool attr = false;
  rc = pointer_head_reserve(reinterpret_cast<const void*>(&pointer_head_beam_kernel<BAN>), attr, who);
  if (rc != CASE_OK) return rc;
  hipLaunchKernelGGL(pointer_head_beam_kernel<BAN>, dim3((unsigned)R), dim3(PH_THREADS), pointer_head_lds(V), (hipStream_t)stream, a, cand_p, cand_id,
                     (int)W, nb);
  return case_check_launch(who);
}

extern "C" int case_pointer_head_beam(const float* logits, const float* mix_logits, const uint32_t* keys, const float* const* copies,
                                      const int64_t* lens, int32_t nmem, float* gen, float* dist, float* cand_p, int64_t* cand_id, int64_t R,
                                      int64_t V, int64_t S, int32_t W, case_stream_t stream) {
  return pointer_head_beam_launch<false>("case_pointer_head_beam", logits, mix_logits, keys, copies, lens, nmem, gen, dist, cand_p, cand_id, R, V, S, W,
                                         BanArgs(), stream);
}

extern "C" int case_pointer_head_beam_ban(const float* logits, const float* mix_logits, const uint32_t* keys, const float* const* copies,
                                          const int64_t* lens, int32_t nmem, float* gen, float* dist, float* cand_p, int64_t* cand_id, int64_t R,
                                          int64_t V, int64_t S, int32_t W, const int32_t* hist, int64_t Tmax, int64_t t, int32_t n, int64_t eos,
                                          case_stream_t stream) {
  BanArgs nb;
  const int rc = pointer_head_ban(nb, "case_pointer_head_beam_ban", hist, Tmax, t, n, eos);
  if (rc != CASE_OK) return rc;
  return pointer_head_beam_launch<true>("case_pointer_head_beam_ban", logits, mix_logits, keys, copies, lens, nmem, gen, dist, cand_p, cand_id, R, V, S,
                                        W, nb, stream);
}

template <bool BAN>
static int pointer_head_sample_launch(const char* who, const float* logits, const float* mix_logits, const uint32_t* keys, const float* const* copies,
                                      const int64_t* lens, int32_t nmem, const float* dist_in, float* gen, float* dist, int64_t* ids, float* prob,
                                      uint8_t* ended, const float* uniforms, int64_t R, int64_t V, int64_t S, float temperature, int32_t top_k,
                                      float top_p, uint64_t seed, uint64_t offset, const CaseStepState* state, int64_t eos, int64_t unk, int64_t pad,
                                      int32_t first, int32_t last, const BanArgs& nb, case_stream_t stream) {
  CASE_REQUIRE(ids && prob && ended && R > 0 && V > 0 && R < (1ll << 31), "%s: bad argument", who);
  CASE_REQUIRE(temperature > 0.f && top_k >= 0 && top_p > 0.f && top_p <= 1.f, "%s: temperature must be > 0, top_k >= 0 and top_p in (0, 1]", who);
  CASE_REQUIRE((logits != nullptr) != (dist_in != nullptr), "%s: give either the logits or a ready distribution", who);
  HeadArgs a;
  if (logits) {
    const int rc = pointer_head_args(a, who, logits, mix_logits, keys, copies, lens, nmem, gen, dist, R, V, S);
    if (rc != CASE_OK) return rc;
  } else {
    if (V > PH_MAX_V) return case_set_error(CASE_E_UNSUPPORTED, "%s: built for V <= %lld", who, (long long)PH_MAX_V);
    a = HeadArgs();
    a.dist = dist;
    a.V = V;
  }
  SampleArgs s;
  s.dist_in = dist_in;
  s.uniforms = uniforms;
  s.state = state;
  s.seed = seed;
  s.offset = offset;
  s.ended = ended;
  s.ids = ids;
  s.prob = prob;
  s.eos = eos;
  s.unk = unk;
  s.pad = pad;
  s.temperature = temperature;
  s.top_p = top_p;
  s.top_k = top_k;
  s.first = first;
  s.last = last;
  static bool attr = false;
  const int rc = pointer_head_reserve(reinterpret_cast<const void*>(&pointer_head_sample_kernel<BAN>), attr, who);
  if (rc != CASE_OK) return rc;
  hipLaunchKernelGGL(pointer_head_sample_kernel<BAN>, dim3((unsigned)R), dim3(PH_THREADS), pointer_head_lds(V), (hipStream_t)stream, a, s, nb);
  return case_check_launch(who);
}

extern "C" int case_pointer_head_sample(const float* logits, const float* mix_logits, const uint32_t* keys, const float* const* copies,
                                        const int64_t* lens, int32_t nmem, const float* dist_in, float* gen, float* dist, int64_t* ids, float* prob,
                                        uint8_t* ended, const float* uniforms, int64_t R, int64_t V, int64_t S, float temperature, int32_t top_k,
                                        float top_p, uint64_t seed, uint64_t offset, const CaseStepState* state, int64_t eos, int64_t unk,
                                        int64_t pad, int32_t first, int32_t last, case_stream_t stream) {
  return pointer_head_sample_launch<false>("case_pointer_head_sample", logits, mix_logits, keys, copies, lens, nmem, dist_in, gen, dist, ids, prob,
                                           ended, uniforms, R, V, S, temperature, top_k, top_p, seed, offset, state, eos, unk, pad, first, last,
                                           BanArgs(), stream);
}

extern "C" int case_pointer_head_sample_ban(const float* logits, const float* mix_logits, const uint32_t* keys, const float* const* copies,
                                            const int64_t* lens, int32_t nmem, const float* dist_in, float* gen, float* dist, int64_t* ids,
                                            float* prob, uint8_t* ended, const float* uniforms, int64_t R, int64_t V, int64_t S, float temperature,
                                            int32_t top_k, float top_p, uint64_t seed, uint64_t offset, const CaseStepState* state, int64_t eos,
                                            int64_t unk, int64_t pad, int32_t first, int32_t last, int32_t* hist, int64_t Tmax, int64_t t, int32_t n,
                                            case_stream_t stream) {
  BanArgs nb;
  const int rc = pointer_head_ban(nb, "case_pointer_head_sample_ban", hist, Tmax, t, n, eos);
  if (rc != CASE_OK) return rc;
  return pointer_head_sample_launch<true>("case_pointer_head_sample_ban", logits, mix_logits, keys, copies, lens, nmem, dist_in, gen, dist, ids, prob,
                                          ended, uniforms, R, V, S, temperature, top_k, top_p, seed, offset, state, eos, unk, pad, first, last, nb,
                                          stream);
}

extern "C" int case_ngram_ban(float* dist, const int32_t* hist, const uint8_t* ended, int64_t R, int64_t V, int64_t Tmax, int64_t t, int32_t n,
                              int64_t eos, case_stream_t stream) {
  CASE_REQUIRE(dist && R > 0 && R < (1ll << 31) && V > 0, "case_ngram_ban: bad argument");
  BanArgs nb;
  const int rc = pointer_head_ban(nb, "case_ngram_ban", hist, Tmax, t, n, eos);
  if (rc != CASE_OK) return rc;
  hipLaunchKernelGGL(ngram_ban_kernel, dim3((unsigned)R), dim3(64), 0, (hipStream_t)stream, dist, ended, V, nb);
  return case_check_launch("case_ngram_ban");
}

extern "C" int case_pointer_head_score(const float* logits, const float* mix_logits, const uint32_t* keys, int64_t rows_per_source,
                                       const float* const* copies, const int64_t* lens, int32_t nmem, const int64_t* targets, int64_t pad,
                                       float* prob, float* copy, int64_t R, int64_t V, int64_t S, case_stream_t stream) {
  CASE_REQUIRE(targets && prob, "case_pointer_head_score: bad argument");
  CASE_REQUIRE(rows_per_source >= 1 && R % rows_per_source == 0, "case_pointer_head_score: %lld rows are no multiple of rows_per_source %lld",
               (long long)R, (long long)rows_per_source);
  ScoreArgs a;
  const int rc = pointer_head_fill(a, "case_pointer_head_score", logits, mix_logits, keys, copies, lens, nmem, R, V, S, PS_MAX_V, "");
  if (rc != CASE_OK) return rc;
  a.targets = targets;
  a.prob = prob;
  a.ptr = copy;
  a.rows_per_source = rows_per_source;
  a.pad = pad;
  hipLaunchKernelGGL(pointer_head_score_kernel, dim3((unsigned)R), dim3(PS_THREADS), 0, (hipStream_t)stream, a);
  return case_check_launch("case_pointer_head_score");
}

extern "C" int case_copy_scatter_fwd(const int64_t* src, const float* w, float* dist, int64_t B, int64_t T, int64_t S,
                                     int64_t V, case_stream_t stream) {
  CASE_REQUIRE(src && w && dist && B > 0 && T > 0 && S > 0 && V > 0, "case_copy_scatter_fwd: bad argument");
  hipLaunchKernelGGL(copy_scatter_fwd_kernel, dim3(grid_for(B * T * S, 256, 2)), dim3(256), 0, (hipStream_t)stream, src, w,
                     dist, B, T, S, V);
  return case_check_launch("case_copy_scatter_fwd");
}

extern "C" int case_copy_scatter_bwd(const int64_t* src, const float* d_dist, float* d_w, int64_t B, int64_t T, int64_t S,
                                     int64_t V, case_stream_t stream) {
  CASE_REQUIRE(src && d_dist && d_w && B > 0 && T > 0 && S > 0 && V > 0, "case_copy_scatter_bwd: bad argument");
  hipLaunchKernelGGL(copy_scatter_bwd_kernel, dim3(grid_for(B * T * S, 256, 2)), dim3(256), 0, (hipStream_t)stream, src,
                     d_dist, d_w, B, T, S, V);
  return case_check_launch("case_copy_scatter_bwd");
}

extern "C" int case_source_sort(const int64_t* src, uint32_t* keys, int64_t B, int64_t S, int64_t V, case_stream_t stream) {
  CASE_REQUIRE(src && keys && B > 0 && S > 0 && V > 0, "case_source_sort: bad argument");
  CASE_REQUIRE(S <= 32768 && V <= 131071, "case_source_sort: S <= 32768 and V <= 131071 (token << 15 | position must fit 32 bits)");
  int n = 2;
  while (n < S) n <<= 1;
  if (n > 16384 && hipFuncSetAttribute((const void*)source_sort_kernel, hipFuncAttributeMaxDynamicSharedMemorySize, 32768 * 4) != hipSuccess)
    return case_set_error(CASE_E_LAUNCH, "case_source_sort: cannot reserve 128 KiB of LDS");
  hipLaunchKernelGGL(source_sort_kernel, dim3((unsigned)B), dim3(1024), (size_t)n * 4, (hipStream_t)stream, src, keys, S, V, n);
  return case_check_launch("case_source_sort");
}

extern "C" int case_copy_scatter_sorted_fwd(const uint32_t* keys, const float* w, float* dist, int64_t B, int64_t T, int64_t S,
                                            int64_t V, case_stream_t stream) {
  CASE_REQUIRE(keys && w && dist && B > 0 && T > 0 && S > 0 && V > 0 && B * T < (1ll << 31), "case_copy_scatter_sorted_fwd: bad argument");
  CASE_REQUIRE(S <= 32768 && V <= 131071, "case_copy_scatter_sorted_fwd: S <= 32768 and V <= 131071");
  hipLaunchKernelGGL(copy_scatter_sorted_kernel, dim3((unsigned)(B * T)), dim3(256), 0, (hipStream_t)stream, keys, w, dist, T, S, V);
  return case_check_launch("case_copy_scatter_sorted_fwd");
}

extern "C" int case_nll_gather_fwd(const float* dist, const int64_t* target, float* per_row, int64_t rows, int64_t V,
                                   case_stream_t stream) {
  CASE_REQUIRE(dist && target && per_row && rows > 0 && V > 0, "case_nll_gather_fwd: bad argument");
  hipLaunchKernelGGL(nll_fwd_kernel, dim3(grid_for(rows, 256)), dim3(256), 0, (hipStream_t)stream, dist, target, per_row, rows, V);
  return case_check_launch("case_nll_gather_fwd");
}

extern "C" int case_nll_gather_bwd(const float* dist, const int64_t* target, const float* g_row, float* d_dist,
                                   int64_t rows, int64_t V, case_stream_t stream) {
  CASE_REQUIRE(dist && target && g_row && d_dist && rows > 0 && V > 0, "case_nll_gather_bwd: bad argument");
  hipLaunchKernelGGL(nll_bwd_kernel, dim3(grid_for(rows, 256)), dim3(256), 0, (hipStream_t)stream, dist, target, g_row, d_dist, rows, V);
  return case_check_launch("case_nll_gather_bwd");
}

namespace {
__global__ void sentence_compact_kernel(const int64_t* __restrict__ ids, int64_t* __restrict__ out, int32_t* __restrict__ len,
                                        int64_t B, int64_t T, int64_t bos, int64_t pad, int64_t eos) {
  const int64_t b = (int64_t)blockIdx.x * blockDim.x + threadIdx.x;
  if (b >= B) return;
  int n = 0;
  bool open = true;
  for (int64_t t = 0; t < T; ++t) {
    const int64_t id = ids[b * T + t];
    if (open && id == eos) open = false;
    if (open && id != bos && id != pad) out[b * T + n++] = id;
  }
  len[b] = n;
  for (int64_t t = n; t < T; ++t) out[b * T + t] = pad;
}

constexpr int RD_MAX_T = 256;
__global__ __launch_bounds__(64) void remove_duplicate_kernel(int64_t* __restrict__ out, int32_t* __restrict__ len, const int64_t T, const int n,
                                                              const int64_t pad) {
  __shared__ int64_t tok[RD_MAX_T];
  const int64_t b = blockIdx.x;
  const int lane = threadIdx.x;
  int64_t* row = out + b * T;
  int L = len[b];
  L = L < 0 ? 0 : (L > (int)T ? (int)T : L);
  const int L0 = L;
  for (int i = lane; i < L0; i += 64) tok[i] = row[i];
  __syncthreads();
  int first[4];
#pragma unroll
  for (int e = 0; e < 4; ++e) {
    const int p = 4 * lane + e;
    first[e] = p;
    if (p < L0) {
      const int64_t mine = tok[p];
      for (int q = 0; q < p; ++q)
        if (tok[q] == mine) {
          first[e] = q;
          break;
        }
    }
  }
  while (L > n) {
    int s[4];
#pragma unroll
    for (int e = 3; e >= 0; --e) {
      const int p = 4 * lane + e;
      const int x = p < L ? first[e] : -1;
      s[e] = e == 3 ? x : max(x, s[e + 1]);
    }
    int tot = s[0];
#pragma unroll
    for (int o = 1; o < 64; o <<= 1) {
      const int other = __shfl_down(tot, o, 64);
      if (lane + o < 64) tot = max(tot, other);
    }
    int after = __shfl_down(tot, 1, 64);
    if (lane == 63) after = -1;
    int best = 0;
#pragma unroll
    for (int e = 0; e < 4; ++e) {
      const int i = 4 * lane + e;
      if (i >= 1 && i <= L - n && max(s[e], after) < i) best = i;
    }
#pragma unroll
    for (int o = 32; o > 0; o >>= 1) best = max(best, __shfl_xor(best, o, 64));
    if (best < 1) break;
    L = best;
  }
  for (int i = L + lane; i < L0; i += 64) row[i] = pad;
  if (lane == 0) len[b] = L;
}
}

extern "C" int case_sentence_compact(const int64_t* ids, int64_t* out, int32_t* len, int64_t B, int64_t T, int64_t bos, int64_t pad,
                                     int64_t eos, case_stream_t stream) {
  CASE_REQUIRE(ids && out && len && B > 0 && T > 0, "case_sentence_compact: bad argument");
  hipLaunchKernelGGL(sentence_compact_kernel, dim3((unsigned)((B + 63) / 64)), dim3(64), 0, (hipStream_t)stream, ids, out, len, B, T, bos,
                     pad, eos);
  return case_check_launch("case_sentence_compact");
}

extern "C" int case_remove_duplicate_ids(int64_t* out, int32_t* len, int64_t B, int64_t T, int32_t n, int64_t pad, case_stream_t stream) {
  CASE_REQUIRE(out && len && B > 0 && B < (1ll << 31) && T > 0 && n >= 1, "case_remove_duplicate_ids: bad argument");
  if (T > RD_MAX_T) return case_set_error(CASE_E_UNSUPPORTED, "case_remove_duplicate_ids: rows of up to %d positions (got %lld)", RD_MAX_T, (long long)T);
  hipLaunchKernelGGL(remove_duplicate_kernel, dim3((unsigned)B), dim3(64), 0, (hipStream_t)stream, out, len, T, (int)n, pad);
  return case_check_launch("case_remove_duplicate_ids");
}

extern "C" int case_row_argmax(const float* x, int64_t* idx, float* val, int64_t rows, int64_t cols, int64_t ld,
                               case_stream_t stream) {
  CASE_REQUIRE(x && idx && rows > 0 && cols > 0 && ld >= cols, "case_row_argmax: bad argument");
  hipLaunchKernelGGL(row_argmax_kernel, dim3(grid_for(rows, 1)), dim3(256), 0, (hipStream_t)stream, x, idx, val, rows, cols, ld);
  return case_check_launch("case_row_argmax");
}
```

### case_rg_amd/ops.py

```python
import math
import ctypes as C
import os

import torch
from torch.autograd import Function

from . import _abi as A
from . import config, paramcache

_DT = {torch.float32: A.F32, torch.bfloat16: A.BF16}


def _code(t):
    try:
        return _DT[t.dtype]
    except KeyError:
        raise TypeError("case_rg_amd: unsupported activation dtype %s" % t.dtype)


_raw_stream, _cur_device = getattr(torch._C, "_cuda_getCurrentRawStream", None), getattr(torch._C, "_cuda_getDevice", None)


def _stream():
    if _raw_stream is not None and _cur_device is not None:
        return _raw_stream(_cur_device())
    return torch.cuda.current_stream().cuda_stream


def _ptr(t, offset_elems=0):
    if t is None:
        return None
    if not t.is_cuda:
        raise RuntimeError("case_rg_amd ops run on the GPU only (got a %s tensor); there is no CPU path" % t.device)
    return t.data_ptr() + offset_elems * t.element_size()


def _drop4(drop):
    if drop is None:
        return 0.0, 0, 0, None
    return tuple(drop) if len(drop) == 4 else tuple(drop) + (None,)


def _u8(mask):
    if mask is None:
        return None
    m = mask.contiguous()
    return m.view(torch.uint8) if m.dtype == torch.bool else m


def invalidate_param_cache():
    paramcache.rewritten()


def cast_param(p, dtype):
    if p.dtype == dtype:
        return p.detach().contiguous()
    base = getattr(p, "_base", None)
    owner = p if isinstance(p, torch.nn.Parameter) else (base if isinstance(base, torch.nn.Parameter) else None)
    if owner is None:
        return cast(p.detach(), dtype)
    owners, tag = (owner,), paramcache.cast_tag(p, dtype)
    hit = paramcache.peek(owners, tag)
    if hit is not None:
        return hit
    if owner is not p and p.is_contiguous() and owner.is_contiguous():
        whole = paramcache.peek(owners, paramcache.cast_tag(owner, dtype))
        if whole is not None:
            return whole.as_strided(p.shape, p.stride(), p.storage_offset() - owner.storage_offset())
    return paramcache.derived(owners, tag, lambda: cast(p.detach(), dtype))


def cast(x, dtype):
    if x.dtype == dtype:
        return x
    x = x.contiguous()
    out = torch.empty(x.shape, dtype=dtype, device=x.device)
    A.call("case_cast", _ptr(x), _ptr(out), x.numel(), _code(x), _DT[dtype], _stream())
    return out


ENCODER_CHAIN = "auto"


def encoder_chain_supported(x, width, ffn_width, needs_grad):
    return (ENCODER_CHAIN == "auto" and x.is_cuda and x.dtype == torch.bfloat16 and width == 512 and ffn_width == 512
            and not needs_grad)


def _chain_pack(mats):
    def build():
        low = [None if m is None else cast_param(m, torch.bfloat16) for m in mats]
        packed = torch.empty(A.lib.case_encoder_chain_packed_bytes() // 2, dtype=torch.bfloat16, device=next(m for m in mats if m is not None).device)
        A.call("case_encoder_chain_pack", _ptr(low[0]), _ptr(low[1]), _ptr(low[2]), _ptr(low[3]), _ptr(packed), _stream())
        return packed

    return paramcache.derived(mats, "chain", build)


def encoder_chain(variant, x_in, resid, layer, next_layer):
    M = x_in.shape[0] * x_in.shape[1]
    dev = x_in.device
    f32 = lambda p: None if p is None else p.detach()
    lay = None if variant == "head" else layer
    nxt = None if variant == "tail" else next_layer
    packed = _chain_pack((None if lay is None else lay.self_attn.out_proj.weight, None if lay is None else lay.linear1.weight,
                          None if lay is None else lay.linear2.weight, None if nxt is None else nxt.self_attn.in_proj_weight))
    d = A.EncoderChainDesc()
    d.rows, d.width, d.variant = M, 512, {"full": 0, "tail": 1, "head": 2}[variant]
    d.eps_ln2 = 0.0 if lay is None else lay.norm2.eps
    d.eps_ln1_next = 0.0 if nxt is None else nxt.norm1.eps
    s_out = torch.empty(x_in.shape, dtype=torch.bfloat16, device=dev)
    qkv = None if nxt is None else torch.empty(x_in.shape[0], x_in.shape[1], 1536, dtype=torch.bfloat16, device=dev)
    x_in = x_in if x_in.is_contiguous() else x_in.contiguous()
    if resid is not None and not resid.is_contiguous():
        resid = resid.contiguous()
    A.call("case_encoder_chain", d, _ptr(x_in), _ptr(resid), _ptr(packed),
           _ptr(None if lay is None else f32(lay.self_attn.out_proj.bias)), _ptr(None if lay is None else f32(lay.linear1.bias)),
           _ptr(None if lay is None else f32(lay.linear2.bias)), _ptr(None if nxt is None else f32(nxt.self_attn.in_proj_bias)),
           _ptr(None if lay is None else f32(lay.norm2.weight)), _ptr(None if lay is None else f32(lay.norm2.bias)),
           _ptr(None if nxt is None else f32(nxt.norm1.weight)), _ptr(None if nxt is None else f32(nxt.norm1.bias)),
           _ptr(s_out), _ptr(qkv), _stream())
    return s_out, qkv


GEMM_TILE = 0
AUX_STREAMS = {}


TILE_TRACE = None
DECODE_MIN_PAIRS = 192
FUSE_BIAS_GRAD = True


def gemm(a, b, c, M, N, K, lda, ldb, ldc, *, a_off=0, b_off=0, c_off=0, a_kmajor=False, b_kmajor=False,
         batch1=1, batch2=1, sa=(0, 0), sb=(0, 0), sc=(0, 0), alpha=1.0, epilogue=0, bias_col=None, bias_row=None,
         aux=None, aux_out=None, ld_aux=0, saux=(0, 0), split_k=1, drop=None, rowsum_out=None):
    d = A.GemmDesc()
    d.M, d.N, d.K, d.lda, d.ldb, d.ldc, d.ld_aux = M, N, K, lda, ldb, ldc, ld_aux
    d.batch1, d.batch2 = batch1, batch2
    d.sa1, d.sa2 = sa
    d.sb1, d.sb2 = sb
    d.sc1, d.sc2 = sc
    d.saux1, d.saux2 = saux
    d.a_kmajor, d.b_kmajor = int(a_kmajor), int(b_kmajor)
    d.in_dtype, d.out_dtype = _code(a), _code(c)
    d.tile = GEMM_TILE
    if b.dtype != a.dtype:
        raise TypeError("gemm operands differ in dtype: %s vs %s" % (a.dtype, b.dtype))
    for name, t in (("aux", aux), ("aux_out", aux_out)):
        if t is not None and t.dtype != a.dtype:
            raise TypeError("gemm %s must have the operand dtype %s, got %s" % (name, a.dtype, t.dtype))
    for name, t in (("bias_col", bias_col), ("bias_row", bias_row)):
        if t is not None and t.dtype != torch.float32:
            raise TypeError("gemm %s must be float32, got %s" % (name, t.dtype))
    if drop is not None and drop[0] > 0.0:
        epilogue |= A.EPI_DROPOUT
        d.drop_p, d.seed, d.offset, d.state = _drop4(drop)
    d.epilogue, d.split_k, d.alpha = epilogue, split_k, alpha
    if TILE_TRACE is not None:
        TILE_TRACE.append(A.lib.case_gemm_tile_for(d, _ptr(a, a_off), _ptr(b, b_off), _ptr(c, c_off), _ptr(bias_col), _ptr(aux),
                                                   _ptr(aux_out)))
    if rowsum_out is not None:
        if not (a_kmajor and epilogue == A.EPI_ATOMIC and lda == M and batch1 * batch2 == 1 and a_off == 0):
            raise ValueError("rowsum_out needs an unbatched k-major contiguous A and the bare ATOMIC epilogue")
        if FUSE_BIAS_GRAD and a.dtype == torch.bfloat16 and A.lib.case_gemm_tile_for(d, _ptr(a), _ptr(b, b_off), _ptr(c, c_off), None, None, None) == 256:
            if not _dw_slabs(d, a, b, b_off, c, c_off, rowsum_out):
                A.call("case_gemm_dw_bias", d, _ptr(a), _ptr(b, b_off), _ptr(c, c_off), _ptr(rowsum_out), _stream())
            return c
        A.call("case_colsum", _ptr(a), _ptr(rowsum_out), K, M, _code(a), _stream())
    elif (epilogue == A.EPI_ATOMIC and split_k >= DW_SLAB_MIN_SPLIT and a.dtype == torch.bfloat16 and batch1 * batch2 == 1 and a_off == 0
          and A.lib.case_gemm_tile_for(d, _ptr(a), _ptr(b, b_off), _ptr(c, c_off), None, None, None) == 256 and _dw_slabs(d, a, b, b_off, c, c_off, None)):
        return c
    A.call("case_gemm", d, _ptr(a, a_off), _ptr(b, b_off), _ptr(c, c_off), _ptr(bias_col), _ptr(bias_row), _ptr(aux),
           _ptr(aux_out), _stream())
    return c


DW_SLAB_MIN_SPLIT = int(os.environ.get("CASE_DW_SLAB_MIN_SPLIT", "8"))
DW_SLAB_MAX_BYTES = 256 << 20


def _dw_slabs(d, a, b, b_off, c, c_off, rowsum_out):
    if DW_SLAB_MIN_SPLIT <= 0 or d.split_k < DW_SLAB_MIN_SPLIT or d.ldc != d.N:
        return False
    need = A.lib.case_gemm_dw_slab_bytes(d)
    if need <= 0 or need > DW_SLAB_MAX_BYTES:
        return False
    ws = torch.empty(need, dtype=torch.uint8, device=c.device)
    A.call("case_gemm_dw_slabs", d, _ptr(a), _ptr(b, b_off), _ptr(c, c_off), _ptr(rowsum_out), _ptr(ws), need, _stream())
    return True


def _split_for(out_rows, out_cols, k_len, elem_bytes):
    k_tiles = max(1, (k_len * elem_bytes + 127) // 128)
    tiles256 = (out_rows // 256) * (out_cols // 256)
    if (elem_bytes == 2 and out_rows % 256 == 0 and out_cols % 256 == 0 and k_len % 64 == 0 and k_tiles >= 64
            and tiles256 * min(64, k_tiles // 8) >= 230):
        tiles = tiles256
        cus = max(8, (256 - int(A.lib.case_get_reserved_cus())) // 8 * 8)
        best, best_score = 1, -1.0
        for split in range(1, 65):
            if split > 1 and k_tiles // split < 8:
                break
            wgs = tiles * split
            eff = wgs / float(((wgs + cus - 1) // cus) * cus)
            score = eff - (0.012 if tiles >= 64 else 0.004) * split - (0.5 if wgs < 0.9 * cus else 0.0)
            if score > best_score:
                best, best_score = split, score
        return best
    tiles = ((out_rows + 127) // 128) * ((out_cols + 127) // 128)
    if elem_bytes == 2 and out_rows % 64 == 0 and out_cols % 64 == 0 and k_len % 64 == 0 and tiles < 128:
        t64 = (out_rows // 64) * (out_cols // 64)
        need = (k_tiles + 9) // 10
        want = max(need, (256 + t64 - 1) // t64)
        split = min(want, k_tiles, max(need, 512 // t64))
        if (k_tiles + split - 1) // split <= 10 and t64 * split <= 512:
            return max(1, split)
    min_k_tiles = 8 if tiles >= 128 else 2
    best, best_eff = 1, 0.0
    for split in range(1, 65):
        if split > 1 and k_tiles // split < min_k_tiles:
            break
# ... 1441 lines not shown

LINEAR_SKINNY = os.environ.get("CASE_LINEAR_SKINNY", "auto")


def linear_skinny_supported(xs, w):
    return (LINEAR_SKINNY != "off" and 1 <= len(xs) <= 4 and 1 <= w.shape[0] <= 8 and not torch.is_grad_enabled()
            and all(x.is_cuda and x.dtype == xs[0].dtype and x.shape[:-1] == xs[0].shape[:-1] for x in xs)
            and xs[0].dtype in (torch.float32, torch.bfloat16) and sum(x.shape[-1] for x in xs) == w.shape[1]
            and bool(A.lib.case_abi_features() & A.FEAT_LINEAR_SKINNY))


def linear_skinny(xs, w, b=None):
    xs = [x if x.is_contiguous() else x.contiguous() for x in xs]
    n = len(xs)
    rows = xs[0].numel() // xs[0].shape[-1]
    ptrs = (C.c_void_p * n)(*[x.data_ptr() for x in xs])
    widths = (C.c_int64 * n)(*[x.shape[-1] for x in xs])
    w32 = w.detach().float().contiguous()
    b32 = None if b is None else b.detach().float().contiguous()
    y = torch.empty(*xs[0].shape[:-1], w.shape[0], dtype=torch.float32, device=xs[0].device)
    A.call("case_linear_skinny", C.cast(ptrs, C.c_void_p), C.cast(widths, C.c_void_p), n, _ptr(w32), _ptr(b32), _ptr(y), rows, w.shape[0], _code(xs[0]),
           _stream())
    return y


def _head_operands(logits, mix_logits, source_map, copies):
    logits = logits if logits.is_contiguous() else logits.contiguous()
    mix_logits = mix_logits.float().contiguous()
    cs = [c.float().contiguous() for c in copies]
    n = len(cs)
    ptrs = (C.c_void_p * n)(*[c.data_ptr() for c in cs])
    lens = (C.c_int64 * n)(*[c.shape[-1] for c in cs])
    return logits, mix_logits, cs, C.cast(ptrs, C.c_void_p), C.cast(lens, C.c_void_p), n, source_map.keys.shape[1]


def _ban_operands(ban, rows, who):
    hist, t, n, eos = ban
    if hist.dtype != torch.int32 or hist.dim() != 2 or hist.shape[0] != rows or not hist.is_contiguous():
        raise TypeError("%s: the history must be a contiguous int32 [%d, Tmax]" % (who, rows))
    if int(n) < 1 or not 0 <= int(t) < hist.shape[1] or int(t) > NGRAM_MAX_T:
        raise ValueError("%s: n >= 1 and 0 <= t < min(Tmax, %d + 1) (got n %r, t %r, Tmax %d)" % (who, NGRAM_MAX_T, n, t, hist.shape[1]))
    return _ptr(hist), hist.shape[1], int(t), int(n), -1 if eos is None else int(eos)


def pointer_head_decode(logits, mix_logits, source_map, copies, want_gen=True, want_dist=True, ban=None):
    B, V = logits.shape
    logits, mix_logits, cs, ptrs, lens, n, S = _head_operands(logits, mix_logits, source_map, copies)
    gen = torch.empty(B, V, dtype=torch.float32, device=logits.device) if want_gen else None
    dist = torch.empty(B, V, dtype=torch.float32, device=logits.device) if want_dist else None
    ids = torch.empty(B, dtype=torch.int64, device=logits.device)
    head = (_ptr(logits), _ptr(mix_logits), _ptr(source_map.keys), ptrs, lens, n, _ptr(gen), _ptr(dist), _ptr(ids), None, B, V, S)
    if ban is None:
        A.call("case_pointer_head_decode", *head, _stream())
    else:
        A.call("case_pointer_head_decode_ban", *head, *_ban_operands(ban, B, "pointer_head_decode"), _stream())
    return gen, dist, ids


def beam_supported(width):
    return 1 <= width <= 8 and bool(A.lib.case_abi_features() & A.FEAT_BEAM_DECODE)


def pointer_head_topk(logits, mix_logits, source_map, copies, width, want_gen=False, want_dist=False, ban=None):
    R, V = logits.shape
    logits, mix_logits, cs, ptrs, lens, n, S = _head_operands(logits, mix_logits, source_map, copies)
    gen = torch.empty(R, V, dtype=torch.float32, device=logits.device) if want_gen else None
    dist = torch.empty(R, V, dtype=torch.float32, device=logits.device) if want_dist else None
    cand_p = torch.empty(R, width, dtype=torch.float32, device=logits.device)
    cand_id = torch.empty(R, width, dtype=torch.int64, device=logits.device)
    head = (_ptr(logits), _ptr(mix_logits), _ptr(source_map.keys), ptrs, lens, n, _ptr(gen), _ptr(dist), _ptr(cand_p), _ptr(cand_id), R, V, S, width)
    if ban is None:
        A.call("case_pointer_head_beam", *head, _stream())
    else:
        A.call("case_pointer_head_beam_ban", *head, *_ban_operands(ban, R, "pointer_head_topk"), _stream())
    return gen, dist, cand_p, cand_id


def sample_supported(V):
    return V <= 36000 and bool(A.lib.case_abi_features() & A.FEAT_SAMPLE_DECODE)


def pointer_head_sample(logits, mix_logits, source_map, copies, ended, t_first, t_last, eos, unk, pad, temperature, top_k, top_p, rng=None,
                        uniforms=None, dist_in=None, want_gen=False, want_dist=False, ban=None):
    if not (float(temperature) > 0.0) or int(top_k) < 0 or not (0.0 < float(top_p) <= 1.0):
        raise ValueError("pointer_head_sample: temperature must be > 0, top_k >= 0 and top_p in (0, 1]")
    if (logits is None) == (dist_in is None):
        raise ValueError("pointer_head_sample: give either the logits or dist_in")
    if uniforms is None and rng is None:
        raise ValueError("pointer_head_sample: give rng=(seed, offset, state) or uniforms")
    src = dist_in if logits is None else logits
    if src.dtype != torch.float32 or src.dim() != 2:
        raise TypeError("pointer_head_sample: the row source must be f32 [R, V]")
    R, V = src.shape
    dev = src.device
    src = src if src.is_contiguous() else src.contiguous()
    if ended.dtype != torch.uint8 or tuple(ended.shape) != (R,) or not ended.is_contiguous():
        raise TypeError("pointer_head_sample: ended must be a contiguous uint8 [R]")
    if uniforms is not None:
        if uniforms.dtype != torch.float32 or tuple(uniforms.shape) != (R,):
            raise TypeError("pointer_head_sample: uniforms must be f32 [R]")
        uniforms = uniforms if uniforms.is_contiguous() else uniforms.contiguous()
    seed, offset, state = rng if rng is not None else (0, 0, None)
    gen = torch.empty(R, V, dtype=torch.float32, device=dev) if (want_gen and logits is not None) else None
    dist = torch.empty(R, V, dtype=torch.float32, device=dev) if want_dist else None
    ids = torch.empty(R, dtype=torch.int64, device=dev)
    prob = torch.empty(R, dtype=torch.float32, device=dev)
    tail = (_ptr(gen), _ptr(dist), _ptr(ids), _ptr(prob), _ptr(ended), _ptr(uniforms), R, V)
    draw = (float(temperature), min(int(top_k), 2 ** 31 - 1), float(top_p), int(seed), int(offset), state, int(eos), int(unk), int(pad),
            int(bool(t_first)), int(bool(t_last)))
    if ban is None:
        entry, draw = "case_pointer_head_sample", draw + (_stream(),)
    else:
        entry, draw = "case_pointer_head_sample_ban", draw + _ban_operands(tuple(ban) + (None,), R, "pointer_head_sample")[:4] + (_stream(),)
    if logits is None:
        A.call(entry, None, None, None, None, None, 0, _ptr(src), *tail, 0, *draw)
    else:
        src, mix_logits, cs, ptrs, lens, n, S = _head_operands(src, mix_logits, source_map, copies)
        A.call(entry, _ptr(src), _ptr(mix_logits), _ptr(source_map.keys), ptrs, lens, n, None, *tail, S, *draw)
    return gen, dist, ids, prob


POINTER_SCORE = os.environ.get("CASE_POINTER_SCORE", "auto")


def pointer_score_supported(source_map, nmem):
    return (POINTER_SCORE != "off" and isinstance(source_map, SortedSource) and 1 <= nmem <= 4
            and not torch.is_grad_enabled()
            and bool(A.lib.case_abi_features() & A.FEAT_POINTER_SCORE))


def pointer_head_score(logits, mix_logits, source_map, rows_per_source, copies, targets, pad=0):
    if logits.dtype != torch.float32 or logits.dim() != 2:
        raise TypeError("pointer_head_score: logits must be f32 [R, V]")
    R, V = logits.shape
    rows_per_source = int(rows_per_source)
    keys = source_map.keys
    if rows_per_source < 1 or R % rows_per_source or keys.shape[0] * rows_per_source != R:
        raise ValueError("pointer_head_score: %d rows, %d key rows, rows_per_source %d" % (R, keys.shape[0], rows_per_source))
    if targets.dtype != torch.int64 or targets.numel() != R:
        raise TypeError("pointer_head_score: targets must be int64 [R]")
    if tuple(mix_logits.shape) != (R, len(copies) + 1):
        raise ValueError("pointer_head_score: mix_logits must be [R, 1 + nmem]")
    if any(c.dim() != 2 or c.shape[0] != R for c in copies):
        raise ValueError("pointer_head_score: every copies[k] must be [R, len_k]")
    logits, mix_logits, cs, ptrs, lens, n, S = _head_operands(logits, mix_logits, source_map, copies)
    targets = targets.reshape(R).contiguous()
    prob = torch.empty(R, dtype=torch.float32, device=logits.device)
    copy = torch.empty(R, dtype=torch.float32, device=logits.device)
    A.call("case_pointer_head_score", _ptr(logits), _ptr(mix_logits), _ptr(keys), rows_per_source, ptrs, lens, n, _ptr(targets), int(pad), _ptr(prob),
           _ptr(copy), R, V, S, _stream())
    return prob, copy


NGRAM_MAX_T = 256


def ngram_ban_supported():
    return bool(A.lib.case_abi_features() & A.FEAT_NGRAM_BAN)


def ngram_ban_(dist, hist, t, n, eos=None, ended=None):
    if dist.dtype != torch.float32 or dist.dim() != 2 or not dist.is_contiguous():
        raise TypeError("ngram_ban_: dist must be a contiguous f32 [R, V]")
    R, V = dist.shape
    if ended is not None and (ended.dtype != torch.uint8 or tuple(ended.shape) != (R,) or not ended.is_contiguous()):
        raise TypeError("ngram_ban_: ended must be a contiguous uint8 [R]")
    hp, Tmax, t, n, eos = _ban_operands((hist, t, n, eos), R, "ngram_ban_")
    A.call("case_ngram_ban", _ptr(dist), hp, _ptr(ended), R, V, Tmax, t, n, eos, _stream())
    return dist


def remove_duplicate_ids(out, len, n=3, pad=0):
    if out.dtype != torch.int64 or out.dim() != 2 or not out.is_contiguous():
        raise TypeError("remove_duplicate_ids: out must be a contiguous int64 [B, T]")
    B, T = out.shape
    if len.dtype != torch.int32 or tuple(len.shape) != (B,) or not len.is_contiguous():
        raise TypeError("remove_duplicate_ids: len must be a contiguous int32 [B]")
    if int(n) != n or n < 1:
        raise ValueError("remove_duplicate_ids: n must be an integer >= 1, not %r" % (n,))
    if T > NGRAM_MAX_T:
        raise ValueError("remove_duplicate_ids: rows of up to %d positions (got %d)" % (NGRAM_MAX_T, T))
    A.call("case_remove_duplicate_ids", _ptr(out), _ptr(len), B, T, int(n), int(pad), _stream())
    return out, len


class BeamState(object):

    def __init__(self, B, W, T, device, flat=False):
        self.B, self.W, self.T = B, W, T
        self.flat = torch.zeros(2, B, W, T, dtype=torch.int32, device=device) if flat else None
        self.alive = torch.zeros(B, W, dtype=torch.uint8, device=device)
        self.alive[:, 0] = 1
        self.cum = torch.zeros(B, W, dtype=torch.float32, device=device)
        self.len = torch.ones(B, W, dtype=torch.int32, device=device)
        self.parent = torch.zeros(B, W, dtype=torch.int32, device=device)
        self.token = torch.zeros(B, W, dtype=torch.int64, device=device)
        self.hist_parent = torch.zeros(T, B, W, dtype=torch.int32, device=device)
        self.hist_token = torch.zeros(T, B, W, dtype=torch.int64, device=device)
        self.fin_key = torch.full((B, W), float("inf"), dtype=torch.float32, device=device)
        self.fin_step = torch.full((B, W), -1, dtype=torch.int32, device=device)
        self.fin_slot = torch.zeros(B, W, dtype=torch.int32, device=device)


    def flat_rows(self, t):
        return self.flat[t % 2].view(self.B * self.W, self.T)


def beam_advance(state, cand_p, cand_id, t, eos):
    B, W = state.B, state.W
    if tuple(cand_p.shape) != (B * W, W) or tuple(cand_id.shape) != (B * W, W) or cand_p.dtype != torch.float32 or cand_id.dtype != torch.int64:
        raise TypeError("beam_advance: candidates must be f32 / int64 [B * W, W]")
    cand_p = cand_p if cand_p.is_contiguous() else cand_p.contiguous()
    cand_id = cand_id if cand_id.is_contiguous() else cand_id.contiguous()
    args = (_ptr(cand_p), _ptr(cand_id), _ptr(state.alive), _ptr(state.cum), _ptr(state.len), _ptr(state.parent), _ptr(state.token),
            _ptr(state.hist_parent), _ptr(state.hist_token), _ptr(state.fin_key), _ptr(state.fin_step), _ptr(state.fin_slot), t, state.T, B, W,
            -1 if eos is None else eos)
    if state.flat is None:
        A.call("case_beam_advance", *args, _stream())
    else:
        A.call("case_beam_advance_ban", *args, _ptr(state.flat[t % 2]), _ptr(state.flat[(t + 1) % 2]), state.T, _stream())


def beam_gather(src, dst, parent, t, valid_src=None, valid_dst=None):
    B, W = parent.shape
    n = len(src)
    first = src[0]
    for s, d in zip(src, dst):
        if not (s.is_contiguous() and d.is_contiguous() and s.shape == first.shape == d.shape and s.dtype == first.dtype == d.dtype
                and s.shape[0] == B * W):
            raise TypeError("beam_gather: every cache must be a contiguous [B * W, Tmax, 2E] tensor of one shape and dtype")
    if parent.dtype != torch.int32 or not parent.is_contiguous():
        raise TypeError("beam_gather: parent must be a contiguous int32 [B, W]")
    sp = (C.c_void_p * n)(*[x.data_ptr() for x in src])
    dp = (C.c_void_p * n)(*[x.data_ptr() for x in dst])
    Tmax = first.shape[1]
    A.call("case_beam_gather", C.cast(sp, C.c_void_p), C.cast(dp, C.c_void_p), n, _ptr(parent), _ptr(_u8(valid_src)), _ptr(_u8(valid_dst)), B, W, Tmax,
           first.shape[2] * first.element_size(), t, _stream())


def beam_backtrack(state):
    B, W, T = state.B, state.W, state.T
    dev = state.fin_key.device
    answer = torch.empty(B, T, dtype=torch.int64, device=dev)
    beam_answers = torch.empty(B, W, T, dtype=torch.int64, device=dev)
    beam_scores = torch.empty(B, W, dtype=torch.float32, device=dev)
    A.call("case_beam_backtrack", _ptr(state.hist_parent), _ptr(state.hist_token), _ptr(state.fin_key), _ptr(state.fin_step), _ptr(state.fin_slot),
           _ptr(answer), _ptr(beam_answers), _ptr(beam_scores), B, W, T, _stream())
    return answer, beam_answers, beam_scores


class SortedSource(object):
    MAX_S, MAX_V = 32768, 131071

    def __init__(self, ids, V):
        self.ids = ids.contiguous()
        self.V = V
        B, S = self.ids.shape
        self.keys = torch.empty(B, S, dtype=torch.int32, device=ids.device)
        A.call("case_source_sort", _ptr(self.ids), _ptr(self.keys), B, S, V, _stream())

    def expand(self, width):
        out = object.__new__(SortedSource)
        out.ids, out.V, out.keys = self.ids.repeat_interleave(width, dim=0), self.V, self.keys.repeat_interleave(width, dim=0)
        return out

    def select(self, rows):
        out = object.__new__(SortedSource)
        if isinstance(rows, slice):
            out.ids, out.V, out.keys = self.ids[rows], self.V, self.keys[rows]
        else:
            out.ids, out.V, out.keys = self.ids.index_select(0, rows), self.V, self.keys.index_select(0, rows)
        return out

    @classmethod
    def fits(cls, ids, V):
        return ids.dtype == torch.int64 and ids.dim() == 2 and ids.size(1) <= cls.MAX_S and V <= cls.MAX_V


class CopyScatterFn(Function):
    @staticmethod
    def forward(ctx, src_ids, w, V, base, keys=None):
        B, T, S = w.shape
        w = w.float().contiguous()
        dist = torch.zeros(B, T, V, dtype=torch.float32, device=w.device) if base is None else base.float().clone()
        if keys is not None:
            A.call("case_copy_scatter_sorted_fwd", _ptr(keys), _ptr(w), _ptr(dist), B, T, S, V, _stream())
        else:
            A.call("case_copy_scatter_fwd", _ptr(src_ids), _ptr(w), _ptr(dist), B, T, S, V, _stream())
        ctx.save_for_backward(src_ids)
        ctx.meta = (B, T, S, V, base is not None)
        return dist

    @staticmethod
    def backward(ctx, g):
        (src_ids,) = ctx.saved_tensors
        B, T, S, V, has_base = ctx.meta
        g = g.float().contiguous()
        d_w = torch.empty(B, T, S, dtype=torch.float32, device=g.device)
        A.call("case_copy_scatter_bwd", _ptr(src_ids), _ptr(g), _ptr(d_w), B, T, S, V, _stream())
        return None, d_w, None, (g if has_base else None), None


def copy_scatter(src_ids, w, V, base=None):
    if isinstance(src_ids, SortedSource):
        if src_ids.V != V:
            raise ValueError("source map was sorted for a vocabulary of %d, scatter asks for %d" % (src_ids.V, V))
# ... 93 lines not shown
```

### case_rg_amd/optim.py

```python
import ctypes as C
import math

import torch

from . import _abi as A
from . import ops, paramcache


class _Entry(C.Structure):
    _fields_ = [("p", C.c_void_p), ("g", C.c_void_p), ("m", C.c_void_p), ("v", C.c_void_p), ("shadow", C.c_void_p),
                ("p_bf16", C.c_void_p), ("numel", C.c_int64), ("step_size", C.c_float), ("bc2_sqrt", C.c_float)]


if C.sizeof(_Entry) != A.lib.case_sizeof_opt_tensor():
    raise ImportError("case_rg_amd.optim: CaseOptTensor is %d bytes in libcase_hip.so, %d here" % (A.lib.case_sizeof_opt_tensor(), C.sizeof(_Entry)))


class FusedAdam(torch.optim.Optimizer):
    def __init__(self, params, lr=1e-3, betas=(0.9, 0.999), eps=1e-8, low_precision=None):
        if lr < 0.0 or eps < 0.0 or not 0.0 <= betas[0] < 1.0 or not 0.0 <= betas[1] < 1.0:
            raise ValueError("invalid Adam hyper-parameters")
        super().__init__(params, dict(lr=lr, betas=betas, eps=eps))
        self.low_precision = low_precision
        self._chunks = {}
        self._table = None
        self._stage = []
        self._stage_next = 0
        self._low = {}
        self._norm_ws = None
        self._graph_stage = None
        self._graph_keep = []
        self.generation = 0
        self.last_stepped = []

    def load_state_dict(self, state_dict):
        super().load_state_dict(state_dict)
        self.generation += 1

    def next_step_number(self):
        steps = [int(st["step"]) for st in self.state.values() if "step" in st]
        return 1 + (max(steps) if steps else 0)

    def stage_step(self, state):
        g0 = self.param_groups[0]
        if any(g["lr"] != g0["lr"] or g["betas"] != g0["betas"] for g in self.param_groups):
            raise RuntimeError("FusedAdam: the device-resident step state carries ONE learning rate / beta pair; the groups differ")
        state.stage_adam(g0["lr"], g0["betas"][0], g0["betas"][1], self.next_step_number())

    def prepare_capture(self):
        n = max(4096, 0 if self._table is None else self._table.numel())
        self._graph_stage = torch.empty(n, dtype=torch.uint8).pin_memory()
        self._graph_keep.append(self._graph_stage)
        self.refresh_low_copies()
        paramcache.rewritten(keep=self.low_copies())

    def low_copies(self):
        for group in self.param_groups:
            for p in group["params"]:
                if id(p) in self._low:
                    yield p, self._low[id(p)]

    def refresh_low_copies(self):
        for p, lp in self.low_copies():
            A.call("case_cast", p.data_ptr(), lp.data_ptr(), p.numel(), A.F32, ops._DT[lp.dtype], ops._stream())
            paramcache.install((p,), paramcache.cast_tag(p, lp.dtype), lp)

    def advance_host_steps(self, params):
        for p in params:
            self.state[p]["step"] = int(self.state[p]["step"]) + 1

    def _chunk_list(self, numels, device):
        key = (tuple(numels), str(device))
        if key not in self._chunks:
            per = A.lib.case_optim_chunk_elems()
            pairs = [(i, c) for i, n in enumerate(numels) for c in range((n + per - 1) // per)]
            self._chunks = {key: torch.tensor(pairs, dtype=torch.int32).to(device)}
        return self._chunks[key]

    @torch.no_grad()
    def step(self, closure=None, clip_norm=None, ema=None, state=None):
        capturing = torch.cuda.is_current_stream_capturing()
        if capturing and (state is None or self._graph_stage is None):
            raise RuntimeError("FusedAdam.step() under stream capture needs prepare_capture() and a device-resident step state")
        self.last_stepped = []
        loss = None
        if closure is not None:
            with torch.enable_grad():
                loss = closure()
        shadow_of = {}
        if ema is not None:
            names = {id(p): n for n, p in ema.model.named_parameters()}
            shadow_of = {pid: ema.shadow[n] for pid, n in names.items() if n in ema.shadow}
        rows, runs, fresh, stepped = [], [], [], []
        dev = None
        for group in self.param_groups:
            params = [p for p in group["params"] if p.grad is not None]
            idle = [p for p in group["params"] if p.grad is None and p.requires_grad and id(p) in shadow_of]
            if not params and not idle:
                continue
            if not (params or idle)[0].is_cuda:
                raise RuntimeError("case_rg_amd.optim.FusedAdam runs on the GPU only; there is no CPU path")
            if dev is None:
                dev = (params or idle)[0].device
            elif (params or idle)[0].device != dev:
                raise RuntimeError("FusedAdam: every parameter group must live on one device")
            beta1, beta2 = group["betas"]
            lr = float(group["lr"])
            first = len(rows)
            dev_state = state
            for p in params:
                if p.dtype != torch.float32 or p.grad.dtype != torch.float32 or not p.is_contiguous():
                    raise TypeError("FusedAdam expects contiguous float32 parameters and gradients")
                st = self.state[p]
                if not st:
                    st["step"] = 0
                    st["exp_avg"] = torch.zeros_like(p, memory_format=torch.preserve_format)
                    st["exp_avg_sq"] = torch.zeros_like(p, memory_format=torch.preserve_format)
                step = st["step"] = int(st["step"]) + 1
                if state is not None and (step != state.staged_step or lr != state.staged_lr):
                    if capturing:
                        raise RuntimeError("FusedAdam: a captured step needs every updated parameter at the same step count (got %d, state %d)"
                                           % (step, state.staged_step))
                    dev_state = None
                g = p.grad if p.grad.is_contiguous() else p.grad.contiguous()
                sh = shadow_of.get(id(p))
                lp = None
                if self.low_precision is not None and p.dim() > 1:
                    lp = self._low.get(id(p))
                    if lp is None or lp.shape != p.shape or lp.device != dev:
                        lp = self._low[id(p)] = torch.empty(p.shape, dtype=self.low_precision, device=dev)
                    fresh.append((p, lp))
                rows.append((_Entry(p.data_ptr(), g.data_ptr(), st["exp_avg"].data_ptr(), st["exp_avg_sq"].data_ptr(),
                                           0 if sh is None else sh.data_ptr(), 0 if lp is None else lp.data_ptr(), p.numel(),
                                           lr / (1.0 - beta1 ** step), math.sqrt(1.0 - beta2 ** step)), p.numel()))
                st["_g"] = g
            for p in idle:
                rows.append((_Entry(p.data_ptr(), 0, 0, 0, shadow_of[id(p)].data_ptr(), 0, p.numel(), 0.0, 1.0), p.numel()))
            runs.append((first, len(rows), beta1, beta2, group["eps"], dev_state))
            stepped += params
        if not rows:
            return loss
        entries = (_Entry * len(rows))(*[e for e, _ in rows])
        raw = bytes(entries)
        if capturing:
            if self._table is None or self._table.numel() < len(raw) or self._table.device != dev or len(raw) > self._graph_stage.numel():
                raise RuntimeError("FusedAdam: run the step eagerly once before capturing it (the entry table is sized by the first step)")
            self._graph_stage[:len(raw)].copy_(torch.frombuffer(bytearray(raw), dtype=torch.uint8))
            self._table[:len(raw)].copy_(self._graph_stage[:len(raw)], non_blocking=True)
        else:
            if self._table is None or self._table.numel() < len(raw) or self._table.device != dev:
                self._table = torch.empty(max(len(raw), 4096), dtype=torch.uint8, device=dev)
                self._stage = [(torch.empty(self._table.numel(), dtype=torch.uint8).pin_memory(), None) for _ in range(3)]
            stage, ev = self._stage[self._stage_next]
            if ev is not None:
                ev.synchronize()
            stage[:len(raw)].copy_(torch.frombuffer(bytearray(raw), dtype=torch.uint8))
            self._table[:len(raw)].copy_(stage[:len(raw)], non_blocking=True)
            ev = torch.cuda.Event()
            ev.record()
            self._stage[self._stage_next] = (stage, ev)
            self._stage_next = (self._stage_next + 1) % len(self._stage)
        table = self._table
        chunks = self._chunk_list([n for _, n in rows], dev)
        per = A.lib.case_optim_chunk_elems()
        chunk_at = [0]
        for _, n in rows:
            chunk_at.append(chunk_at[-1] + (n + per - 1) // per)
        stream = torch.cuda.current_stream().cuda_stream
        sumsq = None
        if clip_norm is not None:
            if self._norm_ws is None or self._norm_ws.numel() != chunks.shape[0] + 1 or self._norm_ws.device != dev:
                self._norm_ws = torch.empty(chunks.shape[0] + 1, dtype=torch.float32, device=dev)
            sumsq = self._norm_ws
            A.call("case_optim_sumsq", table.data_ptr(), chunks.data_ptr(), chunks.shape[0], sumsq.data_ptr() + 4, sumsq.data_ptr(),
                   stream)
        for first, end, beta1, beta2, eps, dev_state in runs:
            c0, c1 = chunk_at[first], chunk_at[end]
            A.call("case_optim_adam_ema", table.data_ptr(), chunks.data_ptr() + c0 * chunks.stride(0) * chunks.element_size(), c1 - c0,
                   None if sumsq is None else sumsq.data_ptr(), float(clip_norm or 0.0), beta1, beta2, eps,
                   0.0 if ema is None else 1.0 - ema.decay, None if dev_state is None else dev_state.address, stream)
        if capturing:
            self._graph_keep += [table, chunks, sumsq]
        self.last_stepped = stepped
        for p in stepped:
            self.state[p].pop("_g", None)
        paramcache.rewritten(keep=fresh)
        return loss
```

### case_rg_amd/paramcache.py

```python
import weakref

_entries = {}
EPOCH = 0
_nobody = lambda: None


def cast_tag(t, dtype):
    return ("cast", t.storage_offset(), t.shape, t.stride(), dtype)


def peek(owners, tag):
    hit = _entries.get((tag, *map(id, owners)))
    if hit is None:
        return None
    for ref, stamp, p in zip(hit[0], hit[1], owners):
        if ref() is not p or (p is not None and stamp != (p._version, p.data_ptr(), p.device)):
            return None
    return hit[2]


def install(owners, tag, value):
    _entries[(tag, *map(id, owners))] = (tuple(_nobody if p is None else weakref.ref(p) for p in owners),
                                                 tuple(None if p is None else (p._version, p.data_ptr(), p.device) for p in owners), value)
    return value


def derived(owners, tag, build):
    value = peek(owners, tag)
    if value is None:
        for key in [k for k, (refs, _, _) in _entries.items() if any(r is not _nobody and r() is None for r in refs)]:
            del _entries[key]
        value = install(owners, tag, build())
    return value


def rewritten(keep=()):
    global EPOCH
    _entries.clear()
    EPOCH += 1
    for p, low in keep:
        install((p,), cast_tag(p, low.dtype), low)


def entries(kind=None):
    for key, (refs, _, value) in list(_entries.items()):
        if kind is None or kind == (key[0][0] if isinstance(key[0], tuple) else key[0]):
            yield tuple(r() for r in refs), key[0], value
```

### include/case_hip.h

```cpp
#ifndef CASE_HIP_H
#define CASE_HIP_H

#include <stddef.h>
#include <stdint.h>

#ifdef __cplusplus
extern "C" {
#endif

typedef void* case_stream_t;

typedef enum { CASE_F32 = 0, CASE_BF16 = 1 } case_dtype_t;

enum {
  CASE_OK = 0,
  CASE_E_ARG = -1,
  CASE_E_UNSUPPORTED = -2,
  CASE_E_LAUNCH = -3
};

#define CASE_ABI_VERSION 600
int case_version(void);
enum {
  CASE_FEAT_GEMM_256 = 1u << 0,
  CASE_FEAT_GEMM_SMALL = 1u << 1,
  CASE_FEAT_ENCODER_CHAIN = 1u << 2,
  CASE_FEAT_ATTN_SCORES = 1u << 3,
  CASE_FEAT_ATTN_DECODE = 1u << 4,
  CASE_FEAT_OPTIM = 1u << 5,
  CASE_FEAT_ATTN_RESIDENT = 1u << 6,
  CASE_FEAT_RESERVED_CUS = 1u << 7,
  CASE_FEAT_GEMM_DW_SLABS = 1u << 8,
  CASE_FEAT_DECODER_CHAIN = 1u << 9,
  CASE_FEAT_ATTN_DECODE_MQA = 1u << 10,
  CASE_FEAT_POINTER_DECODE = 1u << 11,
  CASE_FEAT_POINTER_HEAD = 1u << 12,
  CASE_FEAT_GEMM_LN = 1u << 13,
  CASE_FEAT_STEP_STATE = 1u << 14,
  CASE_FEAT_INTERACTION = 1u << 15,
  CASE_FEAT_ATTN_DECODE_APPEND = 1u << 16,
  CASE_FEAT_LINEAR_SKINNY = 1u << 17,
  CASE_FEAT_BEAM_DECODE = 1u << 18,
  CASE_FEAT_SAMPLE_DECODE = 1u << 19,
  CASE_FEAT_POINTER_SCORE = 1u << 20,
  CASE_FEAT_CONSENSUS = 1u << 21,
  CASE_FEAT_NGRAM_BAN = 1u << 22
};
uint32_t case_abi_features(void);
const char* case_last_error(void);

typedef struct {
  uint64_t rng_base;
  float step_size;
  float bc2_sqrt;
  float lr;
  int32_t step;
  uint64_t reserved[5];
} CaseStepState;
int case_sizeof_step_state(void);
int case_step_advance(CaseStepState* state, uint64_t rng_stride, double beta1, double beta2, case_stream_t stream);

int case_set_reserved_cus(int n);
int case_get_reserved_cus(void);

typedef enum { CASE_WS_ATTENTION_SPLITKV = 1, CASE_WS_ATTENTION_BWD = 2, CASE_WS_OPTIM_SUMSQ = 3, CASE_WS_ENCODER_CHAIN_PACK = 4, CASE_WS_GEMM_DW_SLABS = 5 } case_workspace_kind_t;
int64_t case_workspace_bytes(int32_t kind, const void* desc, int64_t arg);

enum {
  CASE_EPI_BIAS_COL = 1,
  CASE_EPI_BIAS_ROW = 2,
  CASE_EPI_GELU = 4,
  CASE_EPI_RELU = 8,
  CASE_EPI_RESIDUAL = 16,
  CASE_EPI_MUL_DGELU = 32,
  CASE_EPI_MUL_DRELU = 64,
  CASE_EPI_ATOMIC = 128,
  CASE_EPI_DROPOUT = 256
};

typedef struct {
  int64_t M, N, K;
  int64_t lda, ldb, ldc, ld_aux;
  int64_t batch1, batch2;
  int64_t sa1, sa2, sb1, sb2, sc1, sc2, saux1, saux2;
  int32_t a_kmajor, b_kmajor;
  int32_t in_dtype;
  int32_t out_dtype;
  int32_t epilogue;
  int32_t split_k;
  int32_t tile;
  float alpha;
  float drop_p;
  uint64_t seed, offset;
  const CaseStepState* state;
} CaseGemmDesc;

int case_gemm(const CaseGemmDesc* d, const void* A, const void* B, void* C, const float* bias_col,
              const float* bias_row, const void* aux, void* aux_out, case_stream_t stream);
int case_gemm_ln(const CaseGemmDesc* d, const void* A, const float* gamma, const float* beta, float eps, void* ln_out, const void* B, void* C,
                 const float* bias_col, const void* aux, case_stream_t stream);

int case_gemm_dw_bias(const CaseGemmDesc* d, const void* A, const void* B, void* C, float* d_bias, case_stream_t stream);
int case_gemm_dw_slabs(const CaseGemmDesc* d, const void* A, const void* B, void* C, float* d_bias, void* slabs, int64_t slab_bytes,
                       case_stream_t stream);
int64_t case_gemm_dw_slab_bytes(const CaseGemmDesc* d);

int case_gemm_tile_for(const CaseGemmDesc* d, const void* A, const void* B, const void* C, const float* bias_col,
                       const void* aux, const void* aux_out);

int case_embed_pos_fwd(const int64_t* ids, const float* table, const float* pe, void* out, int64_t rows,
                       int64_t seq_len, int64_t H, int64_t vocab, float scale, float drop_p, uint64_t seed,
                       uint64_t offset, const CaseStepState* state, int32_t dtype, case_stream_t stream);
int case_embed_pos_bwd(const int64_t* ids, const void* d_out, float* d_table, int64_t rows, int64_t H,
                       int64_t vocab, float scale, float drop_p, uint64_t seed, uint64_t offset, const CaseStepState* state,
                       int32_t dtype, case_stream_t stream);

int case_scale_add_rows(const void* x, const float* pe, void* y, int64_t rows, int64_t seq_len, int64_t H, float scale,
                        int32_t dtype, case_stream_t stream);

int case_layernorm_fwd(const void* x, const void* x2, const float* gamma, const float* beta, void* y, float* mean,
                       float* rstd, int64_t rows, int64_t cols, float eps, int32_t dtype, case_stream_t stream);
int case_layernorm_bwd(const void* dy, const void* x, const void* x2, const float* gamma, const float* mean,
                       const float* rstd, void* dx, const void* dx_add, float* d_gamma, float* d_beta, int64_t rows,
                       int64_t cols, int32_t dtype, case_stream_t stream);
int case_layernorm_bwd_dropout(const void* dy, const void* x, const float* gamma, const float* mean, const float* rstd, void* dx,
                               void* dx_dropped, float* d_gamma, float* d_beta, int64_t rows, int64_t cols, float p, uint64_t seed,
                               uint64_t offset, const CaseStepState* state, int32_t dtype, case_stream_t stream);
int case_layernorm_bwd_concat5(const void* dy, const void* x, const float* gamma, const float* mean, const float* rstd, const void* dx_add,
                               const void* e, const void* a1, const void* a2, const uint8_t* row_valid, void* de, void* da1, void* da2,
                               float* d_gamma, float* d_beta, int64_t rows, int64_t H, int32_t dtype, case_stream_t stream);

typedef struct {
  int64_t outer, inner, R, C;
  int32_t causal;
  int32_t in_dtype, out_dtype;
  float drop_p;
  uint64_t seed, offset;
  const CaseStepState* state;
} CaseSoftmaxDesc;

int case_softmax_fwd(const CaseSoftmaxDesc* d, const void* x, const uint8_t* col_valid, const uint8_t* row_valid,
                     void* p_out, void* y_out, case_stream_t stream);
int case_softmax_bwd(const CaseSoftmaxDesc* d, const void* dy, const void* p, void* dx, case_stream_t stream);

typedef struct {
  int64_t N, heads, Lq, Lk, head_dim;
  int64_t ldq, ldk, ldv, sq, sk, sv;
  int64_t ldo, so;
  int32_t causal;
  float scale, drop_p;
  uint64_t seed, offset;
  const CaseStepState* state;
} CaseAttnDesc;

int case_attention_supported(int64_t head_dim);
int case_attention_fwd(const CaseAttnDesc* d, const void* q, const void* k, const void* v, const uint8_t* key_valid,
                       void* out, float* lse, case_stream_t stream);
int case_attention_splitkv_workspace(const CaseAttnDesc* d, int32_t ksplit, int64_t* bytes);
int case_attention_fwd_splitkv(const CaseAttnDesc* d, const void* q, const void* k, const void* v, const uint8_t* key_valid,
                               void* out, float* lse, void* workspace, int64_t workspace_bytes, int32_t ksplit,
                               case_stream_t stream);
int case_attention_decode_supported(int64_t head_dim);
int case_attention_decode(const CaseAttnDesc* d, const void* q, const void* k, const void* v, const uint8_t* key_valid,
                          void* out, case_stream_t stream);
int case_attention_decode_append(const CaseAttnDesc* d, const void* q, void* k_cache, void* v_cache, const void* new_k, const void* new_v,
                                 int64_t new_stride, int64_t pos, const uint8_t* key_valid, void* out, case_stream_t stream);
int64_t case_attention_decode_mqa_workspace(int64_t B, int64_t S, int32_t nsplit);
int case_attention_decode_mqa_splits(int64_t B, int64_t S);
int case_attention_decode_mqa(const void* qp, const void* mem, const uint8_t* key_valid, void* out, int64_t B, int64_t S, int64_t ldo,
                              int32_t nsplit, void* workspace, int64_t workspace_bytes, case_stream_t stream);
int case_attention_bwd_supported(int64_t head_dim);
int64_t case_attention_bwd_scratch_floats(const CaseAttnDesc* d);
int case_attention_bwd(const CaseAttnDesc* d, const void* q, const void* k, const void* v, const uint8_t* key_valid,
                       const void* out, const float* lse, const void* dout, float* delta, void* dq, void* dk, void* dv,
                       case_stream_t stream);

int case_attention_scores_supported(const CaseAttnDesc* d);
int case_attention_scores_fwd(const CaseAttnDesc* d, const void* q, const void* k, const uint8_t* key_valid, void* p,
                              void* p_dropped, case_stream_t stream);
int case_attention_scores_bwd(const CaseAttnDesc* d, const void* dout, const void* v, const void* p, void* ds,
                              case_stream_t stream);
typedef struct {
  int64_t N, heads, M, Kc, head_dim;
  int64_t lda, sa_seq, sa_head;
  int64_t ldb, sb_seq, sb_head;
  int64_t ldc, sc_seq, sc_head;
  int32_t a_transposed;
  float alpha;
} CaseAttnProductDesc;
int case_attention_product_supported(const CaseAttnProductDesc* d);
int case_attention_product(const CaseAttnProductDesc* d, const void* a, const void* b, void* c, case_stream_t stream);

int case_add(const void* a, const void* b, void* out, int64_t n, int32_t dtype, case_stream_t stream);
int case_add_n(const void* const* srcs, int32_t count, void* out, int64_t n, int32_t dtype, case_stream_t stream);
int case_dropout(const void* x, void* y, int64_t n, float p, uint64_t seed, uint64_t offset, const CaseStepState* state,
                 int32_t dtype, case_stream_t stream);
int case_mask_rows(const void* x, const uint8_t* row_valid, void* y, int64_t rows, int64_t cols, int32_t dtype,
                   case_stream_t stream);
int case_colsum(const void* x, float* out, int64_t rows, int64_t cols, int32_t dtype, case_stream_t stream);
int case_cast(const void* x, void* y, int64_t n, int32_t src_dtype, int32_t dst_dtype, case_stream_t stream);
int case_scale_cols(const void* x, const float* w, void* y, int64_t rows, int64_t cols, int32_t dtype,
                    case_stream_t stream);
int case_scale_cols_bwd(const void* dy, const void* x, const float* w, void* dx, float* dw, int64_t rows,
                        int64_t cols, int32_t dtype, case_stream_t stream);
int case_rowdot_fwd(const void* x, const float* w, const float* b, float* y, int64_t rows, int64_t cols, int32_t dtype,
                    case_stream_t stream);
int case_rowdot_bwd(const float* g, const void* x, const float* w, void* dx, float* dw, float* db, int64_t rows,
                    int64_t cols, int32_t dtype, case_stream_t stream);
int case_linear_skinny(const void* const* xs, const int64_t* widths, int32_t nseg, const float* w, const float* b, float* y, int64_t rows,
                       int32_t nout, int32_t dtype, case_stream_t stream);
int case_masked_mean_fwd(const void* x, const uint8_t* valid, void* out, int64_t n, int64_t L, int64_t H,
                         int32_t dtype, case_stream_t stream);
int case_masked_mean_bwd(const void* d_out, const uint8_t* valid, void* dx, int64_t n, int64_t L, int64_t H,
                         int32_t dtype, case_stream_t stream);
int case_highway_gate_fwd(const void* gnl, void* y, int64_t rows, int64_t cols, int32_t dtype, case_stream_t stream);
int case_highway_gate_bwd(const void* dy, const void* gnl, void* d_gnl, int64_t rows, int64_t cols, int32_t dtype,
                          case_stream_t stream);

typedef struct {
  int64_t n, Lp, Lq, H, eq_div;
  int32_t dtype;
} CaseInteractionDesc;
int case_interaction_supported(const CaseInteractionDesc* d);
int case_interaction_fwd(const CaseInteractionDesc* d, const void* eq, const void* ep, const uint8_t* q_valid, const uint8_t* p_valid, const float* w,
                         void* a, void* bt, void* g_q_p, void* g_p_q, case_stream_t stream);
int case_concat5_fwd(const void* e, const void* a1, const void* a2, const uint8_t* row_valid, void* out,
                     int64_t rows, int64_t H, int32_t dtype, case_stream_t stream);
int case_concat5_bwd(const void* d_out, const void* e, const void* a1, const void* a2, const uint8_t* row_valid,
                     void* de, void* da1, void* da2, int64_t rows, int64_t H, int32_t dtype, case_stream_t stream);
int case_max_over_p_fwd(const void* x, void* out, int32_t* argmax, int64_t B, int64_t P, int64_t inner, int32_t dtype,
                        case_stream_t stream);
int case_max_over_p_bwd(const void* d_out, const int32_t* argmax, void* dx, int64_t B, int64_t P, int64_t inner,
                        int32_t dtype, case_stream_t stream);

int case_additive_scores_fwd(const float* wq, const void* uh, const float* v, float* s, int64_t B, int64_t T,
                             int64_t S, int64_t H, int32_t dtype, case_stream_t stream);
int case_additive_scores_bwd(const float* ds, const float* wq, const void* uh, const float* v, float* d_wq,
                             float* d_uh, float* d_v, int64_t B, int64_t T, int64_t S, int64_t H, int32_t dtype,
                             case_stream_t stream);

int case_additive_key_exp(const float* uh, void* eu, int64_t n, case_stream_t stream);
int case_pointer_head_decode(const float* logits, const float* mix_logits, const uint32_t* keys, const float* const* copies,
                             const int64_t* lens, int32_t nmem, float* gen, float* dist, int64_t* ids, float* top, int64_t B, int64_t V,
                             int64_t S, case_stream_t stream);
int case_pointer_head_beam(const float* logits, const float* mix_logits, const uint32_t* keys, const float* const* copies, const int64_t* lens,
                           int32_t nmem, float* gen, float* dist, float* cand_p, int64_t* cand_id, int64_t R, int64_t V, int64_t S, int32_t W,
                           case_stream_t stream);
int case_beam_advance(const float* cand_p, const int64_t* cand_id, uint8_t* alive, float* cum, int32_t* len, int32_t* parent, int64_t* token,
                      int32_t* hist_parent, int64_t* hist_token, float* fin_key, int32_t* fin_step, int32_t* fin_slot, int64_t t, int64_t T,
                      int64_t B, int32_t W, int64_t eos, case_stream_t stream);
int case_beam_gather(const void* const* src, void* const* dst, int32_t nlayers, const int32_t* parent, const uint8_t* valid_src,
                     uint8_t* valid_dst, int64_t B, int32_t W, int64_t Tmax, int64_t row_bytes, int64_t t, case_stream_t stream);
int case_beam_backtrack(const int32_t* hist_parent, const int64_t* hist_token, const float* fin_key, const int32_t* fin_step,
                        const int32_t* fin_slot, int64_t* answer, int64_t* beam_answers, float* beam_scores, int64_t B, int32_t W, int64_t T,
                        case_stream_t stream);
int case_pointer_head_sample(const float* logits, const float* mix_logits, const uint32_t* keys, const float* const* copies, const int64_t* lens,
                             int32_t nmem, const float* dist_in, float* gen, float* dist, int64_t* ids, float* prob, uint8_t* ended,
                             const float* uniforms, int64_t R, int64_t V, int64_t S, float temperature, int32_t top_k, float top_p, uint64_t seed,
                             uint64_t offset, const CaseStepState* state, int64_t eos, int64_t unk, int64_t pad, int32_t first, int32_t last,
                             case_stream_t stream);
int case_pointer_head_decode_ban(const float* logits, const float* mix_logits, const uint32_t* keys, const float* const* copies,
                                 const int64_t* lens, int32_t nmem, float* gen, float* dist, int64_t* ids, float* top, int64_t B, int64_t V,
                                 int64_t S, int32_t* hist, int64_t Tmax, int64_t t, int32_t n, int64_t eos, case_stream_t stream);
int case_pointer_head_beam_ban(const float* logits, const float* mix_logits, const uint32_t* keys, const float* const* copies, const int64_t* lens,
                               int32_t nmem, float* gen, float* dist, float* cand_p, int64_t* cand_id, int64_t R, int64_t V, int64_t S, int32_t W,
                               const int32_t* hist, int64_t Tmax, int64_t t, int32_t n, int64_t eos, case_stream_t stream);
int case_pointer_head_sample_ban(const float* logits, const float* mix_logits, const uint32_t* keys, const float* const* copies, const int64_t* lens,
                                 int32_t nmem, const float* dist_in, float* gen, float* dist, int64_t* ids, float* prob, uint8_t* ended,
                                 const float* uniforms, int64_t R, int64_t V, int64_t S, float temperature, int32_t top_k, float top_p, uint64_t seed,
                                 uint64_t offset, const CaseStepState* state, int64_t eos, int64_t unk, int64_t pad, int32_t first, int32_t last,
                                 int32_t* hist, int64_t Tmax, int64_t t, int32_t n, case_stream_t stream);
int case_beam_advance_ban(const float* cand_p, const int64_t* cand_id, uint8_t* alive, float* cum, int32_t* len, int32_t* parent, int64_t* token,
                          int32_t* hist_parent, int64_t* hist_token, float* fin_key, int32_t* fin_step, int32_t* fin_slot, int64_t t, int64_t T,
                          int64_t B, int32_t W, int64_t eos, const int32_t* flat_old, int32_t* flat_new, int64_t Tmax, case_stream_t stream);
int case_ngram_ban(float* dist, const int32_t* hist, const uint8_t* ended, int64_t R, int64_t V, int64_t Tmax, int64_t t, int32_t n, int64_t eos,
                   case_stream_t stream);
int case_pointer_head_score(const float* logits, const float* mix_logits, const uint32_t* keys, int64_t rows_per_source,
                            const float* const* copies, const int64_t* lens, int32_t nmem, const int64_t* targets, int64_t pad, float* prob,
                            float* copy, int64_t R, int64_t V, int64_t S, case_stream_t stream);
int case_pointer_attend_decode(const float* wq, const float* wq_add, const void* eu, const float* v, const void* value, const uint8_t* col_valid,
                               const uint8_t* row_valid, const float* prior, void* ctx, float* p, float* copy, int64_t B, int64_t S, int64_t H,
                               case_stream_t stream);
int case_copy_scatter_fwd(const int64_t* src, const float* w, float* dist, int64_t B, int64_t T, int64_t S,
                          int64_t V, case_stream_t stream);
int case_copy_scatter_bwd(const int64_t* src, const float* d_dist, float* d_w, int64_t B, int64_t T, int64_t S,
                          int64_t V, case_stream_t stream);
int case_source_sort(const int64_t* src, uint32_t* keys, int64_t B, int64_t S, int64_t V, case_stream_t stream);
int case_copy_scatter_sorted_fwd(const uint32_t* keys, const float* w, float* dist, int64_t B, int64_t T, int64_t S,
                                 int64_t V, case_stream_t stream);

int case_nll_gather_fwd(const float* dist, const int64_t* target, float* per_row, int64_t rows, int64_t V,
                        case_stream_t stream);
int case_nll_gather_bwd(const float* dist, const int64_t* target, const float* g_row, float* d_dist, int64_t rows,
                        int64_t V, case_stream_t stream);
int case_row_argmax(const float* x, int64_t* idx, float* val, int64_t rows, int64_t cols, int64_t ld,
                    case_stream_t stream);

typedef struct {
  void* p;
  const void* g;
  void* m;
  void* v;
  void* shadow;
  void* p_bf16;
  int64_t numel;
  float step_size;
  float bc2_sqrt;
} CaseOptTensor;
int case_optim_chunk_elems(void);
int case_sizeof_opt_tensor(void);
int case_optim_sumsq(const CaseOptTensor* table, const int32_t* chunks, int64_t nchunks, float* partials, float* sumsq,
                     case_stream_t stream);
int case_optim_adam_ema(const CaseOptTensor* table, const int32_t* chunks, int64_t nchunks, const float* sumsq, float max_norm,
                        double beta1, double beta2, double eps, double ema_w, const CaseStepState* state, case_stream_t stream);

typedef struct {
  int64_t rows;
  int32_t width;
  int32_t variant;
  float eps_ln2, eps_ln1_next;
} CaseEncoderChainDesc;
int64_t case_encoder_chain_packed_bytes(void);
int case_encoder_chain_pack(const void* wo, const void* w1, const void* w2, const void* wqkv, void* packed, case_stream_t stream);
int case_encoder_chain(const CaseEncoderChainDesc* d, const void* x_in, const void* resid, const void* packed, const float* bo,
                       const float* b1, const float* b2, const float* bqkv, const float* ln2_g, const float* ln2_b,
                       const float* ln1n_g, const float* ln1n_b, void* s_out, void* qkv_out, case_stream_t stream);


int case_sentence_compact(const int64_t* ids, int64_t* out, int32_t* len, int64_t B, int64_t T, int64_t bos, int64_t pad,
                          int64_t eos, case_stream_t stream);

int case_remove_duplicate_ids(int64_t* out, int32_t* len, int64_t B, int64_t T, int32_t n, int64_t pad, case_stream_t stream);

int case_lcs_pairs(const int64_t* a, const int32_t* a_len, const int64_t* b, const int32_t* b_len, int32_t* lcs, float* f, int64_t B,
                   int64_t N, int64_t M, int64_t Ta, int64_t Tb, case_stream_t stream);
int case_consensus_pick(const float* f, const float* w, const uint8_t* valid, const int64_t* cand, float* utility, int64_t* index,
                        int64_t* answer, int64_t B, int64_t N, int64_t T, case_stream_t stream);

#ifdef __cplusplus
}
#endif
#endif
```

Before: 1.336 million tokens/s.

## Fuse pointer-generator training head into target-only probability kernels

```diff
diff --git a/case_rg_amd/CaSE/Model.py b/case_rg_amd/CaSE/Model.py
--- a/case_rg_amd/CaSE/Model.py
+++ b/case_rg_amd/CaSE/Model.py
@@ -6,7 +6,7 @@
 from ..common.Interaction import Interaction
 from ..common.TransformerSeqEncoderDecoder import PointerDecoderCore, TransformerSeqEncoder, no_repeat_ngram_param, sampling_params
 from ..common.Utils import to_sentence
-from ..common.heads import block_stack, generation_nll, passage_bce, run_block_pair, run_blocks
+from ..common.heads import block_stack, generation_nll, passage_bce, run_block_pair, run_blocks, target_nll
 from ..evaluation.rouge_ids import consensus_answers
 
 
@@ -43,9 +43,10 @@
 
     def forward(self, encode_memories, BOS, UNK, source_map, groundtruth_index=None, additional_decoder_feature=None,
                 encode_weights=None, encode_masks=None, init_decoder_state=None, max_target_length=None, beam_width=None, sampling=None,
-                score_index=None, no_repeat_ngram=0):
+                score_index=None, no_repeat_ngram=0, target_probs=False):
         return self._run(encode_memories, encode_masks, encode_weights, source_map, BOS, groundtruth_index, max_target_length, beam_width, sampling,
-                         score_index, feature_of=lambda T: self._feature(additional_decoder_feature, T), no_repeat_ngram=no_repeat_ngram)
+                         score_index, feature_of=lambda T: self._feature(additional_decoder_feature, T), no_repeat_ngram=no_repeat_ngram,
+                         target_probs=target_probs)
 
 
 class RelevantPassageSelection(nn.Module):
@@ -117,7 +118,8 @@
         self.decoder = decoder
 
     def action(self, query, passage, source_map, encode_query, encode_passage, passage_selection_result,
-               span_extraction_result, output=None, max_target_length=None, beam_width=None, sampling=None, score_index=None, no_repeat_ngram=0):
+               span_extraction_result, output=None, max_target_length=None, beam_width=None, sampling=None, score_index=None, no_repeat_ngram=0,
+               target_probs=False):
         B = query.size(0)
         passage_score = passage_selection_result[0]
         token_score, query_rep, passage_rep = span_extraction_result
@@ -132,7 +134,7 @@
                             additional_decoder_feature=answer_rep, groundtruth_index=output,
                             max_target_length=max_target_length, encode_masks=[query.ne(0), passage.ne(0)],
                             encode_weights=[prior_q, prior_p], beam_width=beam_width, sampling=sampling, score_index=score_index,
-                            no_repeat_ngram=no_repeat_ngram)
+                            no_repeat_ngram=no_repeat_ngram, target_probs=target_probs)
 
 
 class CaSE(nn.Module):
@@ -182,7 +184,9 @@
         loss_se = (valid * bce * data['token_weight'].detach()).sum() / valid.sum()
         rg = self.response_generation.action(data['query'], data['passage'], data['source_map'], encode_query=eq,
                                              encode_passage=ep, passage_selection_result=ps, span_extraction_result=se,
-                                             output=data['response'])
+                                             output=data['response'], target_probs=True)
+        if rg[1] is None:
+            return [loss_ps, loss_se, target_nll(rg[2], data['response'])]
         dist1, dist2 = rg[2]
         return [loss_ps, loss_se, generation_nll(ops.add(dist1, dist2), data['response'])]
 
diff --git a/case_rg_amd/Masque/Model.py b/case_rg_amd/Masque/Model.py
--- a/case_rg_amd/Masque/Model.py
+++ b/case_rg_amd/Masque/Model.py
@@ -6,7 +6,7 @@
 from ..common.Interaction import Interaction
 from ..common.TransformerSeqEncoderDecoder import PointerDecoderCore, TransformerSeqEncoder, no_repeat_ngram_param, sampling_params
 from ..common.Utils import to_sentence
-from ..common.heads import block_stack, generation_nll, passage_bce, run_block_pair
+from ..common.heads import block_stack, generation_nll, passage_bce, run_block_pair, target_nll
 from ..evaluation.rouge_ids import consensus_answers
 
 
@@ -32,9 +32,9 @@
 
     def forward(self, encode_memories, BOS, UNK, source_map, encode_masks=None, encode_weights=None,
                 groundtruth_index=None, init_decoder_state=None, max_target_length=None, beam_width=None, sampling=None, score_index=None,
-                no_repeat_ngram=0):
+                no_repeat_ngram=0, target_probs=False):
         return self._run(encode_memories, encode_masks, encode_weights, source_map, BOS, groundtruth_index, max_target_length, beam_width, sampling,
-                         score_index, no_repeat_ngram=no_repeat_ngram)
+                         score_index, no_repeat_ngram=no_repeat_ngram, target_probs=target_probs)
 
 
 class PassageSelection(nn.Module):
@@ -78,7 +78,7 @@
         self.decoder = decoder
 
     def action(self, query, passage, source_map, encode_query=None, encode_passage=None, passage_selection_result=None,
-               output=None, max_target_length=None, beam_width=None, sampling=None, score_index=None, no_repeat_ngram=0):
+               output=None, max_target_length=None, beam_width=None, sampling=None, score_index=None, no_repeat_ngram=0, target_probs=False):
         if encode_query is None:
             encode_query = self.query_encoder(query)[0][:, :, -1]
         if encode_passage is None:
@@ -93,7 +93,7 @@
         return self.decoder([query_rep, passage_rep], self.BOS, self.UNK, source_map, groundtruth_index=output,
                             max_target_length=max_target_length, encode_masks=[query.ne(0), passage.ne(0)],
                             encode_weights=[prior_q, prior_p], beam_width=beam_width, sampling=sampling, score_index=score_index,
-                            no_repeat_ngram=no_repeat_ngram)
+                            no_repeat_ngram=no_repeat_ngram, target_probs=target_probs)
 
 
 class Masque(nn.Module):
@@ -134,8 +134,9 @@
     def do_train(self, data):
         eq, ep, ps = self._encode_select(data)
         rg = self.response_generation.action(data['query'], data['passage'], data['source_map'], encode_query=eq,
-                                             encode_passage=ep, passage_selection_result=ps, output=data['response'])
-        return [0.25 * passage_bce(ps[0], data['passage_label']), generation_nll(rg[2], data['response'])]
+                                             encode_passage=ep, passage_selection_result=ps, output=data['response'], target_probs=True)
+        nll = target_nll(rg[2], data['response']) if rg[1] is None else generation_nll(rg[2], data['response'])
+        return [0.25 * passage_bce(ps[0], data['passage_label']), nll]
 
     def do_ps_train(self, data):
         _, _, ps = self._encode_select(data)
diff --git a/case_rg_amd/_abi.py b/case_rg_amd/_abi.py
--- a/case_rg_amd/_abi.py
+++ b/case_rg_amd/_abi.py
@@ -11,7 +11,8 @@
 WS_ATTENTION_SPLITKV, WS_ATTENTION_BWD, WS_OPTIM_SUMSQ, WS_ENCODER_CHAIN_PACK, WS_GEMM_DW_SLABS = 1, 2, 3, 4, 5
 (FEAT_GEMM_256, FEAT_GEMM_SMALL, FEAT_ENCODER_CHAIN, FEAT_ATTN_SCORES, FEAT_ATTN_DECODE, FEAT_OPTIM, FEAT_ATTN_RESIDENT, FEAT_RESERVED_CUS,
  FEAT_GEMM_DW_SLABS, FEAT_DECODER_CHAIN, FEAT_ATTN_DECODE_MQA, FEAT_POINTER_DECODE, FEAT_POINTER_HEAD, FEAT_GEMM_LN, FEAT_STEP_STATE,
- FEAT_INTERACTION, FEAT_ATTN_DECODE_APPEND, FEAT_LINEAR_SKINNY, FEAT_BEAM_DECODE, FEAT_SAMPLE_DECODE, FEAT_POINTER_SCORE, FEAT_CONSENSUS, FEAT_NGRAM_BAN) = (1 << i for i in range(23))
+ FEAT_INTERACTION, FEAT_ATTN_DECODE_APPEND, FEAT_LINEAR_SKINNY, FEAT_BEAM_DECODE, FEAT_SAMPLE_DECODE, FEAT_POINTER_SCORE, FEAT_CONSENSUS, FEAT_NGRAM_BAN,
+ FEAT_POINTER_TRAIN) = (1 << i for i in range(24))
 EPI_BIAS_COL, EPI_BIAS_ROW, EPI_GELU, EPI_RELU = 1, 2, 4, 8
 EPI_RESIDUAL, EPI_MUL_DGELU, EPI_MUL_DRELU, EPI_ATOMIC, EPI_DROPOUT = 16, 32, 64, 128, 256
 
@@ -118,6 +119,8 @@
     "case_pointer_head_beam": [ptr] * 5 + [i32] + [ptr] * 4 + [i64, i64, i64, i32, ptr],
     "case_pointer_head_sample": [ptr] * 5 + [i32] + [ptr] * 7 + [i64, i64, i64, f32, i32, f32, u64, u64, ptr, i64, i64, i64, i32, i32, ptr],
     "case_pointer_head_score": [ptr] * 3 + [i64, ptr, ptr, i32, ptr, i64, ptr, ptr, i64, i64, i64, ptr],
+    "case_pointer_head_train_fwd": [ptr, i64, ptr, ptr, i64, ptr, ptr, i32, ptr, i64, ptr, ptr, ptr, i64, i64, i64, ptr],
+    "case_pointer_head_train_bwd": [ptr, ptr, i64, ptr, ptr, ptr, ptr, i64, ptr, ptr, i32, ptr, i64, ptr, i32, ptr, ptr, i64, i64, i64, ptr],
     "case_beam_advance": [ptr] * 12 + [i64, i64, i64, i32, i64, ptr],
     "case_pointer_head_decode_ban": [ptr] * 5 + [i32] + [ptr] * 4 + [i64, i64, i64, ptr, i64, i64, i32, i64, ptr],
     "case_pointer_head_beam_ban": [ptr] * 5 + [i32] + [ptr] * 4 + [i64, i64, i64, i32, ptr, i64, i64, i32, i64, ptr],
diff --git a/case_rg_amd/common/TransformerSeqEncoderDecoder.py b/case_rg_amd/common/TransformerSeqEncoderDecoder.py
--- a/case_rg_amd/common/TransformerSeqEncoderDecoder.py
+++ b/case_rg_amd/common/TransformerSeqEncoderDecoder.py
@@ -424,7 +424,7 @@
         return dict(token_probs=p, copy_probs=c, scores=scores, loss=loss, tokens=count)
 
     def _run(self, encode_memories, encode_masks, encode_weights, source_map, BOS, groundtruth_index, max_target_length, beam_width, sampling,
-             score_index, feature_of=None, no_repeat_ngram=0):
+             score_index, feature_of=None, no_repeat_ngram=0, target_probs=False):
         B, dev = source_map.size(0), encode_memories[0].device
         source_map = self._sorted(source_map)
         mems = [m.reshape(B, -1, self.hidden_size) for m in encode_memories]
@@ -436,7 +436,11 @@
         if self.training and groundtruth_index is not None:
             dec_ids = torch.cat([self._bos(B, BOS, dev), groundtruth_index[:, :-1]], dim=-1)
             feat = None if feature_of is None else feature_of(dec_ids.size(1))
-            dec_out, gen, dist = self._head(*self._run_prefix(dec_ids, mems, valid, weights, feat), feat, source_map)
+            prefix = self._run_prefix(dec_ids, mems, valid, weights, feat)
+            if target_probs and ops.pointer_train_supported(source_map, len(mems), self.tgt_vocab_size):
+                dec_out, prob = self._head_train(*prefix, feat, source_map, groundtruth_index)
+                return dec_out, None, prob, groundtruth_index
+            dec_out, gen, dist = self._head(*prefix, feat, source_map)
             return dec_out, gen, dist, groundtruth_index
         if self.training:
             return None
@@ -475,6 +479,12 @@
         d1, d2 = self._mix(dec_out, ctxs, gen, copies, source_map)
         return dec_out, gen, ((d1, d2) if self.training and self.train_returns_pair else ops.add(d1, d2))
 
+    def _head_train(self, dec_in, x, ctxs, copies, feat, source_map, targets):
+        dec_out, gen_in = self._head_parts(dec_in, x, feat)
+        h = ops.linear(gen_in, self.gen[0].weight, self.gen[0].bias, p_drop=config.drop_p(self.gen_dropout, self.training))
+        mix_logits = ops.linear(torch.cat([dec_out] + ctxs, dim=-1), self.mix.weight, self.mix.bias, out_dtype=torch.float32)
+        return dec_out, ops.pointer_head_train(h, self.gen[-2].weight, mix_logits, copies, source_map, targets)
+
     def _generate(self, gen_in, hidden_drop):
         h = ops.linear(gen_in, self.gen[0].weight, self.gen[0].bias, p_drop=config.drop_p(hidden_drop, self.training))
         logits = ops.linear(h, self.gen[-2].weight, None, out_dtype=torch.float32)
diff --git a/case_rg_amd/common/heads.py b/case_rg_amd/common/heads.py
--- a/case_rg_amd/common/heads.py
+++ b/case_rg_amd/common/heads.py
@@ -59,3 +59,9 @@
     rows = ops.nll_rows(dist.reshape(-1, V), response.reshape(-1))
     count = response.ne(0).sum().clamp(min=1)
     return (rows.sum() / count).unsqueeze(0)
+
+
+def target_nll(prob, response):
+    scored = response.ne(0)
+    count = scored.sum().clamp(min=1)
+    return ((-torch.log(prob + 1e-8) * scored).sum() / count).unsqueeze(0)
diff --git a/case_rg_amd/csrc/api.hip b/case_rg_amd/csrc/api.hip
--- a/case_rg_amd/csrc/api.hip
+++ b/case_rg_amd/csrc/api.hip
@@ -24,7 +24,7 @@
 extern "C" uint32_t case_abi_features(void) {
   return CASE_FEAT_GEMM_256 | CASE_FEAT_GEMM_SMALL | CASE_FEAT_ENCODER_CHAIN | CASE_FEAT_ATTN_SCORES | CASE_FEAT_ATTN_DECODE | CASE_FEAT_OPTIM |
          CASE_FEAT_ATTN_RESIDENT | CASE_FEAT_RESERVED_CUS | CASE_FEAT_GEMM_DW_SLABS | CASE_FEAT_ATTN_DECODE_MQA | CASE_FEAT_POINTER_DECODE | CASE_FEAT_POINTER_HEAD | CASE_FEAT_GEMM_LN | CASE_FEAT_STEP_STATE | CASE_FEAT_INTERACTION | CASE_FEAT_ATTN_DECODE_APPEND | CASE_FEAT_LINEAR_SKINNY |
-         CASE_FEAT_BEAM_DECODE | CASE_FEAT_SAMPLE_DECODE | CASE_FEAT_POINTER_SCORE | CASE_FEAT_CONSENSUS | CASE_FEAT_NGRAM_BAN;
+         CASE_FEAT_BEAM_DECODE | CASE_FEAT_SAMPLE_DECODE | CASE_FEAT_POINTER_SCORE | CASE_FEAT_CONSENSUS | CASE_FEAT_NGRAM_BAN | CASE_FEAT_POINTER_TRAIN;
 }
 extern "C" const char* case_last_error(void) { return g_err; }
 
diff --git a/case_rg_amd/csrc/attn_pointer.hip b/case_rg_amd/csrc/attn_pointer.hip
--- a/case_rg_amd/csrc/attn_pointer.hip
+++ b/case_rg_amd/csrc/attn_pointer.hip
@@ -976,7 +976,10 @@
   const int64_t* targets;
   float* prob;
   float* ptr;
+  float* row_max;
+  float* row_sum;
   int64_t V, S, rows_per_source, pad;
+  int64_t ld;
   int nmem;
 };
 
@@ -1006,10 +1009,12 @@
     if (tid == 0) {
       a.prob[r] = is_pad ? 1.f : 0.f;
       if (a.ptr) a.ptr[r] = 0.f;
+      if (a.row_max) a.row_max[r] = 0.f;
+      if (a.row_sum) a.row_sum[r] = 1.f;
     }
     return;
   }
-  const float* lg = a.logits + r * V;
+  const float* lg = a.logits + r * a.ld;
   int64_t head = (int64_t)(((16u - (uint32_t)(reinterpret_cast<uintptr_t>(lg) & 15u)) & 15u) >> 2);
   if (head > V) head = V;
   const int64_t n4 = (V - head) >> 2, tail = head + 4 * n4;
@@ -1087,6 +1092,134 @@
   if (lane == 0) {
     a.prob[r] = pm[0] * gen_y + acc;
     if (a.ptr) a.ptr[r] = acc;
+    if (a.row_max) a.row_max[r] = m;
+    if (a.row_sum) a.row_sum[r] = s;
+  }
+}
+
+struct TrainBwdArgs {
+  const float* logits;
+  const float* mix_logits;
+  const uint32_t* keys;
+  const float* copy[PH_MAX_MEM];
+  int64_t len[PH_MAX_MEM];
+  float* d_copy[PH_MAX_MEM];
+  const float* c;
+  const float* row_max;
+  const float* row_sum;
+  const int64_t* targets;
+  void* g;
+  float* d_mix;
+  int64_t V, S, rows_per_source, pad, ld;
+  int nmem;
+};
+
+template <typename OutT>
+__device__ __forceinline__ void pt_store8(OutT* p, const float (&v)[8]);
+template <>
+__device__ __forceinline__ void pt_store8<bf16_t>(bf16_t* p, const float (&v)[8]) { Vec16<bf16_t>::store(p, v); }
+template <>
+__device__ __forceinline__ void pt_store8<float>(float* p, const float (&v)[8]) {
+  *reinterpret_cast<float4*>(p) = make_float4(v[0], v[1], v[2], v[3]);
+  *reinterpret_cast<float4*>(p + 4) = make_float4(v[4], v[5], v[6], v[7]);
+}
+
+template <typename OutT>
+__global__ __launch_bounds__(PS_THREADS) void pointer_head_train_bwd_kernel(const TrainBwdArgs a) {
+  const int64_t r = blockIdx.x, V = a.V, n8 = a.ld >> 3;
+  const int tid = threadIdx.x, lane = tid & 63;
+  const int64_t y = a.targets[r];
+  const float c = a.c[r];
+  OutT* g = reinterpret_cast<OutT*>(a.g) + r * a.ld;
+#pragma unroll
+  for (int k = 0; k < PH_MAX_MEM; ++k) {
+    if (k < a.nmem) {
+      float* d = a.d_copy[k] + r * a.len[k];
+      for (int64_t i = tid; i < a.len[k]; i += PS_THREADS) d[i] = 0.f;
+    }
+  }
+  if ((a.pad >= 0 && y == a.pad) || y < 0 || y >= V || c == 0.f) {
+    const float zero[8] = {0.f, 0.f, 0.f, 0.f, 0.f, 0.f, 0.f, 0.f};
+    for (int64_t i = tid; i < n8; i += PS_THREADS) pt_store8<OutT>(g + 8 * i, zero);
+    if (tid <= a.nmem) a.d_mix[r * (a.nmem + 1) + tid] = 0.f;
+    return;
+  }
+  const float* lg = a.logits + r * a.ld;
+  const float m = a.row_max[r], s = a.row_sum[r];
+  const float gen_y = __expf(lg[y] - m) / s;
+  float pm[1 + PH_MAX_MEM];
+  {
+    float mm = -INFINITY, ss = 0.f;
+#pragma unroll
+    for (int k = 0; k <= PH_MAX_MEM; ++k) pm[k] = k <= a.nmem ? a.mix_logits[r * (a.nmem + 1) + k] : -INFINITY;
+#pragma unroll
+    for (int k = 0; k <= PH_MAX_MEM; ++k) mm = fmaxf(mm, pm[k]);
+#pragma unroll
+    for (int k = 0; k <= PH_MAX_MEM; ++k) {
+      pm[k] = __expf(pm[k] - mm);
+      ss += pm[k];
+    }
+#pragma unroll
+    for (int k = 0; k <= PH_MAX_MEM; ++k) pm[k] /= ss;
+  }
+  __syncthreads();
+  if (tid < 64) {
+    const uint32_t* keys = a.keys + (r / a.rows_per_source) * a.S;
+    const uint32_t want = (uint32_t)y << 15;
+    int64_t lo = 0, hi = a.S;
+    while (lo < hi) {
+      const int64_t mid = (lo + hi) >> 1;
+      if (keys[mid] < want) lo = mid + 1;
+      else hi = mid;
+    }
+    float mass[PH_MAX_MEM] = {0.f, 0.f, 0.f, 0.f};
+    for (int64_t i = lo + lane; i < a.S; i += 64) {
+      const uint32_t key = keys[i];
+      if (key == 0xFFFFFFFFu || (key >> 15) != (uint32_t)y) break;
+      int64_t pos = key & 0x7FFFu;
+      bool done = false;
+#pragma unroll
+      for (int k = 0; k < PH_MAX_MEM; ++k) {
+        if (k < a.nmem && !done) {
+          if (pos < a.len[k]) {
+            mass[k] += a.copy[k][r * a.len[k] + pos];
+            a.d_copy[k][r * a.len[k] + pos] = c * pm[k + 1];
+            done = true;
+          }
+          pos -= a.len[k];
+        }
+      }
+    }
+    float dpm[1 + PH_MAX_MEM], dot;
+    dpm[0] = c * gen_y;
+    dot = pm[0] * dpm[0];
+#pragma unroll
+    for (int k = 0; k < PH_MAX_MEM; ++k) {
+      dpm[k + 1] = c * wave_sum(mass[k]);
+      dot += pm[k + 1] * dpm[k + 1];
+    }
+    if (lane == 0) {
+#pragma unroll
+      for (int k = 0; k <= PH_MAX_MEM; ++k)
+        if (k <= a.nmem) a.d_mix[r * (a.nmem + 1) + k] = pm[k] * (dpm[k] - dot);
+    }
+  }
+  const float coef = c * pm[0] * gen_y, nscale = -coef / s;
+  for (int64_t i = tid; i < n8; i += PS_THREADS) {
+    const int64_t v0 = 8 * i;
+    const ps_f32x4 x0 = PS_LOAD4(lg + v0), x1 = PS_LOAD4(lg + v0 + 4);
+    float out[8];
+#pragma unroll
+    for (int e = 0; e < 4; ++e) {
+      out[e] = nscale * __expf(x0[e] - m);
+      out[4 + e] = nscale * __expf(x1[e] - m);
+    }
+#pragma unroll
+    for (int e = 0; e < 8; ++e) {
+      if (v0 + e == y) out[e] += coef;
+      if (v0 + e >= V) out[e] = 0.f;
+    }
+    pt_store8<OutT>(g + v0, out);
   }
 }
 
@@ -1533,8 +1666,66 @@
   a.ptr = copy;
   a.rows_per_source = rows_per_source;
   a.pad = pad;
+  a.ld = V;
+  a.row_max = a.row_sum = nullptr;
   hipLaunchKernelGGL(pointer_head_score_kernel, dim3((unsigned)R), dim3(PS_THREADS), 0, (hipStream_t)stream, a);
   return case_check_launch("case_pointer_head_score");
+}
+
+extern "C" int case_pointer_head_train_fwd(const float* logits, int64_t ld, const float* mix_logits, const uint32_t* keys, int64_t rows_per_source,
+                                           const float* const* copies, const int64_t* lens, int32_t nmem, const int64_t* targets, int64_t pad,
+                                           float* prob, float* row_max, float* row_sum, int64_t R, int64_t V, int64_t S, case_stream_t stream) {
+  CASE_REQUIRE(targets && prob && row_max && row_sum, "case_pointer_head_train_fwd: bad argument");
+  CASE_REQUIRE(ld >= V, "case_pointer_head_train_fwd: row stride %lld below V = %lld", (long long)ld, (long long)V);
+  CASE_REQUIRE(rows_per_source >= 1 && R % rows_per_source == 0, "case_pointer_head_train_fwd: %lld rows are no multiple of rows_per_source %lld",
+               (long long)R, (long long)rows_per_source);
+  ScoreArgs a;
+  const int rc = pointer_head_fill(a, "case_pointer_head_train_fwd", logits, mix_logits, keys, copies, lens, nmem, R, V, S, PS_MAX_V, "");
+  if (rc != CASE_OK) return rc;
+  a.targets = targets;
+  a.prob = prob;
+  a.ptr = nullptr;
+  a.rows_per_source = rows_per_source;
+  a.pad = pad;
+  a.ld = ld;
+  a.row_max = row_max;
+  a.row_sum = row_sum;
+  hipLaunchKernelGGL(pointer_head_score_kernel, dim3((unsigned)R), dim3(PS_THREADS), 0, (hipStream_t)stream, a);
+  return case_check_launch("case_pointer_head_train_fwd");
+}
+
+extern "C" int case_pointer_head_train_bwd(const float* c, const float* logits, int64_t ld, const float* row_max, const float* row_sum,
+                                           const float* mix_logits, const uint32_t* keys, int64_t rows_per_source, const float* const* copies,
+                                           const int64_t* lens, int32_t nmem, const int64_t* targets, int64_t pad, void* g, int32_t g_dtype,
+                                           float* const* d_copies, float* d_mix, int64_t R, int64_t V, int64_t S, case_stream_t stream) {
+  CASE_REQUIRE(c && row_max && row_sum && targets && g && d_copies && d_mix, "case_pointer_head_train_bwd: bad argument");
+  CASE_REQUIRE(g_dtype == CASE_F32 || g_dtype == CASE_BF16, "case_pointer_head_train_bwd: g_dtype %d", g_dtype);
+  CASE_REQUIRE(ld >= V && ld % 8 == 0 && (uintptr_t)logits % 16 == 0 && (uintptr_t)g % 16 == 0,
+               "case_pointer_head_train_bwd: the logits and g rows must be 16-byte aligned with a stride (%lld) that is a multiple of 8 and >= V",
+               (long long)ld);
+  CASE_REQUIRE(rows_per_source >= 1 && R % rows_per_source == 0, "case_pointer_head_train_bwd: %lld rows are no multiple of rows_per_source %lld",
+               (long long)R, (long long)rows_per_source);
+  TrainBwdArgs a;
+  const int rc = pointer_head_fill(a, "case_pointer_head_train_bwd", logits, mix_logits, keys, copies, lens, nmem, R, V, S, PS_MAX_V, "");
+  if (rc != CASE_OK) return rc;
+  for (int k = 0; k < PH_MAX_MEM; ++k) {
+    a.d_copy[k] = k < nmem ? d_copies[k] : nullptr;
+    CASE_REQUIRE(k >= nmem || d_copies[k], "case_pointer_head_train_bwd: null d_copies");
+  }
+  a.c = c;
+  a.row_max = row_max;
+  a.row_sum = row_sum;
+  a.targets = targets;
+  a.g = g;
+  a.d_mix = d_mix;
+  a.rows_per_source = rows_per_source;
+  a.pad = pad;
+  a.ld = ld;
+  if (g_dtype == CASE_BF16)
+    hipLaunchKernelGGL(pointer_head_train_bwd_kernel<bf16_t>, dim3((unsigned)R), dim3(PS_THREADS), 0, (hipStream_t)stream, a);
+  else
+    hipLaunchKernelGGL(pointer_head_train_bwd_kernel<float>, dim3((unsigned)R), dim3(PS_THREADS), 0, (hipStream_t)stream, a);
+  return case_check_launch("case_pointer_head_train_bwd");
 }
 
 extern "C" int case_copy_scatter_fwd(const int64_t* src, const float* w, float* dist, int64_t B, int64_t T, int64_t S,
diff --git a/case_rg_amd/ops.py b/case_rg_amd/ops.py
--- a/case_rg_amd/ops.py
+++ b/case_rg_amd/ops.py
@@ -68,6 +68,39 @@
         if whole is not None:
             return whole.as_strided(p.shape, p.stride(), p.storage_offset() - owner.storage_offset())
     return paramcache.derived(owners, tag, lambda: cast(p.detach(), dtype))
+
+
+VOCAB_ROW_PAD = 256
+
+
+def cast_param_padded(p, dtype, multiple=VOCAB_ROW_PAD):
+    rows = p.shape[0]
+    rows_p = paramcache.padded_rows(rows, multiple)
+    if p.dim() != 2:
+        raise ValueError("cast_param_padded: a [rows, cols] weight, got %s" % (tuple(p.shape),))
+    if rows_p == rows:
+        return cast_param(p, dtype)
+
+    def build():
+        full = torch.zeros(rows_p, p.shape[1], dtype=dtype, device=p.device)
+        src = p.detach()
+        src = src if src.is_contiguous() else src.contiguous()
+        if src.dtype == dtype:
+            full[:rows].copy_(src)
+        else:
+            A.call("case_cast", _ptr(src), _ptr(full), src.numel(), _code(src), _DT[dtype], _stream())
+        return full
+
+    if not isinstance(p, torch.nn.Parameter) or not p.is_contiguous():
+        return build()
+    p.case_row_pad = multiple
+    tag = paramcache.cast_tag(p, dtype)
+    low = paramcache.peek((p,), tag)
+    full = None if low is None else paramcache.padded_base(low, rows_p)
+    if full is None:
+        full = build()
+        paramcache.install((p,), tag, full[:rows])
+    return full
 
 
 def cast(x, dtype):
@@ -1815,6 +1848,79 @@
     return prob, copy
 
 
+TRAIN_HEAD = os.environ.get("CASE_TRAIN_HEAD", "fused")
+
+
+def pointer_train_supported(source_map, nmem, V):
+    return (TRAIN_HEAD != "off" and isinstance(source_map, SortedSource) and 1 <= nmem <= 4 and V <= SortedSource.MAX_V
+            and bool(A.lib.case_abi_features() & A.FEAT_POINTER_TRAIN))
+
+
+class PointerHeadTrainFn(Function):
+
+    @staticmethod
+    def forward(ctx, h, w, mix_logits, keys, rows_per_source, targets, pad, *copies):
+        H, V = h.shape[-1], w.shape[0]
+        h2 = h.reshape(-1, H)
+        h2 = h2 if h2.is_contiguous() else h2.contiguous()
+        R = h2.shape[0]
+        wp = cast_param_padded(w, h2.dtype)
+        Vp = wp.shape[0]
+        logits = torch.empty(R, Vp, dtype=torch.float32, device=h2.device)
+        gemm(h2, wp, logits, R, Vp, H, H, H, Vp)
+        mix2 = mix_logits.reshape(R, -1)
+        _, mix2, cs, ptrs, lens, n, S = _head_operands(logits, mix2, _Keys(keys), [c.reshape(R, -1) for c in copies])
+        tg = targets.reshape(R).contiguous()
+        out = torch.empty(3, R, dtype=torch.float32, device=h2.device)
+        A.call("case_pointer_head_train_fwd", _ptr(logits), Vp, _ptr(mix2), _ptr(keys), rows_per_source, ptrs, lens, n, _ptr(tg), int(pad),
+               _ptr(out[0]), _ptr(out[1]), _ptr(out[2]), R, V, S, _stream())
+        ctx.save_for_backward(h2, wp, logits, mix2, out, tg, keys, *cs)
+        ctx.meta = (h.shape, V, mix_logits.shape, mix_logits.dtype, [(c.shape, c.dtype) for c in copies], rows_per_source, int(pad))
+        return out[0]
+
+    @staticmethod
+    def backward(ctx, c):
+        h2, wp, logits, mix2, out, tg, keys = ctx.saved_tensors[:7]
+        cs = list(ctx.saved_tensors[7:])
+        hshape, V, mix_shape, mix_dtype, copy_meta, rows_per_source, pad = ctx.meta
+        (R, H), Vp, n, S = h2.shape, wp.shape[0], len(cs), keys.shape[1]
+        c = c.reshape(R).float().contiguous()
+        g = torch.empty(R, Vp, dtype=h2.dtype, device=h2.device)
+        d_cs = [torch.empty_like(x) for x in cs]
+        d_mix = torch.empty_like(mix2)
+        ptrs = (C.c_void_p * n)(*[x.data_ptr() for x in cs])
+        d_ptrs = (C.c_void_p * n)(*[x.data_ptr() for x in d_cs])
+        lens = (C.c_int64 * n)(*[x.shape[-1] for x in cs])
+        A.call("case_pointer_head_train_bwd", _ptr(c), _ptr(logits), Vp, _ptr(out[1]), _ptr(out[2]), _ptr(mix2), _ptr(keys), rows_per_source,
+               C.cast(ptrs, C.c_void_p), C.cast(lens, C.c_void_p), n, _ptr(tg), pad, _ptr(g), _code(g), C.cast(d_ptrs, C.c_void_p), _ptr(d_mix),
+               R, V, S, _stream())
+        dh = _input_grad(g, wp, R, H, Vp).view(hshape) if ctx.needs_input_grad[0] else None
+        dw = _weight_grad(g, h2, Vp, H)[:V] if ctx.needs_input_grad[1] else None
+        d_mix = d_mix.view(mix_shape).to(mix_dtype) if ctx.needs_input_grad[2] else None
+        d_copies = [d.view(shape).to(dtype) if need else None for d, (shape, dtype), need in zip(d_cs, copy_meta, ctx.needs_input_grad[7:])]
+        return (dh, dw, d_mix, None, None, None, None) + tuple(d_copies)
+
+
+class _Keys(object):
+
+    def __init__(self, keys):
+        self.keys = keys
+
+
+def pointer_head_train(h, w, mix_logits, copies, source_map, targets, pad=0):
+    if not isinstance(source_map, SortedSource):
+        raise TypeError("pointer_head_train: the source map must be a SortedSource")
+    R, keys = targets.numel(), source_map.keys
+    if keys.shape[0] < 1 or R % keys.shape[0]:
+        raise ValueError("pointer_head_train: %d rows over %d key rows" % (R, keys.shape[0]))
+    if mix_logits.shape[-1] != len(copies) + 1 or mix_logits.numel() != R * (len(copies) + 1):
+        raise ValueError("pointer_head_train: mix_logits must be [..., 1 + nmem]")
+    if h.numel() != R * h.shape[-1] or any(c.numel() != R * c.shape[-1] for c in copies):
+        raise ValueError("pointer_head_train: h and every copies[k] must have one row per target")
+    prob = PointerHeadTrainFn.apply(h, w, mix_logits, keys, R // keys.shape[0], targets, pad, *copies)
+    return prob.view(targets.shape)
+
+
 NGRAM_MAX_T = 256
 
 
diff --git a/case_rg_amd/optim.py b/case_rg_amd/optim.py
--- a/case_rg_amd/optim.py
+++ b/case_rg_amd/optim.py
@@ -127,8 +127,13 @@
                 lp = None
                 if self.low_precision is not None and p.dim() > 1:
                     lp = self._low.get(id(p))
-                    if lp is None or lp.shape != p.shape or lp.device != dev:
-                        lp = self._low[id(p)] = torch.empty(p.shape, dtype=self.low_precision, device=dev)
+                    rows_p = paramcache.padded_rows(p.shape[0], getattr(p, "case_row_pad", 0) if p.dim() == 2 else 0)
+                    if lp is None or lp.shape != p.shape or lp.device != dev or (rows_p != p.shape[0] and paramcache.padded_base(lp, rows_p) is None):
+                        if rows_p != p.shape[0]:
+                            lp = torch.zeros(rows_p, p.shape[1], dtype=self.low_precision, device=dev)[:p.shape[0]]
+                        else:
+                            lp = torch.empty(p.shape, dtype=self.low_precision, device=dev)
+                        self._low[id(p)] = lp
                     fresh.append((p, lp))
                 rows.append((_Entry(p.data_ptr(), g.data_ptr(), st["exp_avg"].data_ptr(), st["exp_avg_sq"].data_ptr(),
                                            0 if sh is None else sh.data_ptr(), 0 if lp is None else lp.data_ptr(), p.numel(),
diff --git a/case_rg_amd/paramcache.py b/case_rg_amd/paramcache.py
--- a/case_rg_amd/paramcache.py
+++ b/case_rg_amd/paramcache.py
@@ -7,6 +7,18 @@
 
 def cast_tag(t, dtype):
     return ("cast", t.storage_offset(), t.shape, t.stride(), dtype)
+
+
+def padded_rows(rows, multiple):
+    return rows if not multiple else (rows + multiple - 1) // multiple * multiple
+
+
+def padded_base(low, rows_p):
+    base = getattr(low, "_base", None)
+    if (base is not None and base.dim() == 2 and low.dim() == 2 and tuple(base.shape) == (rows_p, low.shape[1]) and base.dtype == low.dtype
+            and base.is_contiguous() and low.is_contiguous() and base.data_ptr() == low.data_ptr()):
+        return base
+    return None
 
 
 def peek(owners, tag):
diff --git a/include/case_hip.h b/include/case_hip.h
--- a/include/case_hip.h
+++ b/include/case_hip.h
@@ -44,7 +44,8 @@
   CASE_FEAT_SAMPLE_DECODE = 1u << 19,
   CASE_FEAT_POINTER_SCORE = 1u << 20,
   CASE_FEAT_CONSENSUS = 1u << 21,
-  CASE_FEAT_NGRAM_BAN = 1u << 22
+  CASE_FEAT_NGRAM_BAN = 1u << 22,
+  CASE_FEAT_POINTER_TRAIN = 1u << 23
 };
 uint32_t case_abi_features(void);
 const char* case_last_error(void);
@@ -278,6 +279,13 @@
 int case_pointer_head_score(const float* logits, const float* mix_logits, const uint32_t* keys, int64_t rows_per_source,
                             const float* const* copies, const int64_t* lens, int32_t nmem, const int64_t* targets, int64_t pad, float* prob,
                             float* copy, int64_t R, int64_t V, int64_t S, case_stream_t stream);
+int case_pointer_head_train_fwd(const float* logits, int64_t ld, const float* mix_logits, const uint32_t* keys, int64_t rows_per_source,
+                                const float* const* copies, const int64_t* lens, int32_t nmem, const int64_t* targets, int64_t pad, float* prob,
+                                float* row_max, float* row_sum, int64_t R, int64_t V, int64_t S, case_stream_t stream);
+int case_pointer_head_train_bwd(const float* c, const float* logits, int64_t ld, const float* row_max, const float* row_sum,
+                                const float* mix_logits, const uint32_t* keys, int64_t rows_per_source, const float* const* copies,
+                                const int64_t* lens, int32_t nmem, const int64_t* targets, int64_t pad, void* g, int32_t g_dtype,
+                                float* const* d_copies, float* d_mix, int64_t R, int64_t V, int64_t S, case_stream_t stream);
 int case_pointer_attend_decode(const float* wq, const float* wq_add, const void* eu, const float* v, const void* value, const uint8_t* col_valid,
                                const uint8_t* row_valid, const float* prior, void* ctx, float* p, float* copy, int64_t B, int64_t S, int64_t H,
                                case_stream_t stream);
```

Measured after the change: 1.358 million tokens/s, median of 6. 1.7% higher.
